# w-k-jones/tobac-flow

Measured on AMD Instinct MI355X. Metric: Mpix/s end-to-end flow+sobel+watershed, 5424^2 frames, higher is better.
Workload: dtype f32

## Files before the change

tobac_flow_amd/csrc/capi.hip:

```cpp
#include "tf_common.h"
#include <stdarg.h>
#include <algorithm>

static thread_local char g_err[512] = "";

void tf_set_error(const char *fmt, ...) {
    va_list ap;
    va_start(ap, fmt);
    vsnprintf(g_err, sizeof(g_err), fmt, ap);
    va_end(ap);
}

extern "C" int tf_version(void) { return 100; }
extern "C" const char *tf_last_error(void) { return g_err; }
extern "C" int tf_device_count(void) {
    int n = 0;
    hipError_t e = hipGetDeviceCount(&n);
    if (e != hipSuccess) { tf_set_error("hipGetDeviceCount: %s", hipGetErrorString(e)); return 0; }
    return n;
}

#include <vector>
#include <mutex>
bool g_tf_prof_on = false;
namespace {
struct Rec { int id; double bytes; hipEvent_t a, b; };
std::vector<Rec> g_recs;
std::vector<hipEvent_t> g_free;
std::mutex g_mu;
const char *g_names[TFK_COUNT] = {"to8bit_pair", "fb_gaussian_blur", "fb_resize", "fb_polyexp", "fb_update_matrices",
    "fb_blur_solve", "fb_iteration_fused", "smooth_flow", "convolve", "sobel", "ws_setup", "ws_relax_sweep", "ws_labels", "vr_prepare", "vr_system", "vr_sor", "binary_morph"};
hipEvent_t get_event() {
    if (!g_free.empty()) { hipEvent_t e = g_free.back(); g_free.pop_back(); return e; }
    hipEvent_t e; (void)hipEventCreate(&e); return e;
}
}
void tf_prof_record(int id, double bytes, hipStream_t s, bool start) {
    std::lock_guard<std::mutex> lk(g_mu);
    if (start) { Rec r{id, bytes, get_event(), get_event()}; (void)hipEventRecord(r.a, s); g_recs.push_back(r); }
    else {
        for (size_t i = g_recs.size(); i-- > 0;) if (g_recs[i].id == id) { (void)hipEventRecord(g_recs[i].b, s); break; }
    }
}
extern "C" int tf_profile_enable(int on) { g_tf_prof_on = on != 0; return TF_OK; }
extern "C" int tf_profile_kernel_count(void) { return TFK_COUNT; }
extern "C" const char *tf_profile_kernel_name(int id) { return (id >= 0 && id < TFK_COUNT) ? g_names[id] : ""; }
extern "C" int tf_profile_collect(int64_t *calls, double *ms, double *bytes) {
    std::lock_guard<std::mutex> lk(g_mu);
    for (int i = 0; i < TFK_COUNT; i++) { calls[i] = 0; ms[i] = 0; bytes[i] = 0; }
    for (auto &r : g_recs) {
        float t = 0;
        if (hipEventSynchronize(r.b) == hipSuccess && hipEventElapsedTime(&t, r.a, r.b) == hipSuccess) {
            calls[r.id]++; ms[r.id] += t; bytes[r.id] += r.bytes;
        }
        g_free.push_back(r.a); g_free.push_back(r.b);
    }
    g_recs.clear();
    return TF_OK;
}

void tf_ws_host_pool_release();
extern "C" int tf_shutdown(void) {
    tf_ws_host_pool_release();
    std::lock_guard<std::mutex> lk(g_mu);
    g_tf_prof_on = false;
    for (auto &r : g_recs) { (void)hipEventDestroy(r.a); (void)hipEventDestroy(r.b); }
    for (auto e : g_free) (void)hipEventDestroy(e);
    g_recs.clear(); g_free.clear();
    return TF_OK;
}

template <int UNROLL, bool NT>
__global__ void __launch_bounds__(256)
k_copy16(const uint4 *__restrict__ src, uint4 *__restrict__ dst, size_t n16)
{
    const size_t tile = (size_t)UNROLL * 256, n_tiles = n16 / tile;
    for (size_t t = blockIdx.x; t < n_tiles; t += gridDim.x) {
        const size_t base = t * tile + threadIdx.x;
        uint4 v[UNROLL];
#pragma unroll
        for (int k = 0; k < UNROLL; k++) {
            if (NT) { typedef unsigned int u4 __attribute__((ext_vector_type(4))); const u4 r = __builtin_nontemporal_load((const u4 *)(src + base + k * 256)); v[k] = make_uint4(r.x, r.y, r.z, r.w); }
            else v[k] = src[base + k * 256];
        }
#pragma unroll
        for (int k = 0; k < UNROLL; k++) {
            if (NT) { typedef unsigned int u4 __attribute__((ext_vector_type(4))); u4 r; r.x = v[k].x; r.y = v[k].y; r.z = v[k].z; r.w = v[k].w; __builtin_nontemporal_store(r, (u4 *)(dst + base + k * 256)); }
            else dst[base + k * 256] = v[k];
        }
    }
    for (size_t i = n_tiles * tile + (size_t)blockIdx.x * 256 + threadIdx.x; i < n16; i += (size_t)gridDim.x * 256) dst[i] = src[i];
}
extern "C" int tf_copy16_variant(const void *src, void *dst, size_t bytes, void *stream, int variant)
{
    TF_REQUIRE(src && dst && bytes >= 16 && bytes % 16 == 0 && ((uintptr_t)src & 15) == 0 && ((uintptr_t)dst & 15) == 0, "tf_copy16: 16-byte aligned buffers of a multiple of 16 bytes");
    const size_t n16 = bytes / 16;
    hipStream_t s = (hipStream_t)stream;
    const uint4 *a = (const uint4 *)src; uint4 *b = (uint4 *)dst;
    const unsigned g8 = (unsigned)std::min<size_t>((n16 + 255) / 256, 256 * 8), g16 = (unsigned)std::min<size_t>((n16 + 255) / 256, 256 * 16);
    switch (variant) {
    case 1: hipLaunchKernelGGL((k_copy16<4, false>), dim3(g16), dim3(256), 0, s, a, b, n16); break;
    case 2: hipLaunchKernelGGL((k_copy16<8, false>), dim3(g8), dim3(256), 0, s, a, b, n16); break;
    case 3: hipLaunchKernelGGL((k_copy16<4, true>), dim3(g8), dim3(256), 0, s, a, b, n16); break;
    case 4: hipLaunchKernelGGL((k_copy16<8, true>), dim3(g8), dim3(256), 0, s, a, b, n16); break;
    case 5: hipLaunchKernelGGL((k_copy16<2, false>), dim3(g8), dim3(256), 0, s, a, b, n16); break;
    case 6: hipLaunchKernelGGL((k_copy16<1, false>), dim3(g16), dim3(256), 0, s, a, b, n16); break;
    case 7: hipLaunchKernelGGL((k_copy16<4, false>), dim3(g8), dim3(256), 0, s, a, b, n16); break;
    default: hipLaunchKernelGGL((k_copy16<4, true>), dim3(g8), dim3(256), 0, s, a, b, n16); break;
    }
    TF_CHECK_LAUNCH();
    return TF_OK;
}
extern "C" int tf_copy16(const void *src, void *dst, size_t bytes, void *stream) { return tf_copy16_variant(src, dst, bytes, stream, 0); }
```

tobac_flow_amd/csrc/morph.hip:

```cpp
#include "tf_common.h"
#include <initializer_list>
#include <string.h>
#include <stdlib.h>

struct MorphTaps { int n; int8_t dt[27], dy[27], dx[27]; };

__global__ void __launch_bounds__(256)
k_binary_morph(const uint8_t *__restrict__ in, int64_t T, int H, int W, MorphTaps tp, int op, int border,
               uint8_t *__restrict__ out)
{
    const int x = blockIdx.x * 64 + threadIdx.x, y = blockIdx.y * 4 + threadIdx.y;
    const int64_t t = blockIdx.z;
    if (x >= W || y >= H) return;
    const int64_t plane = (int64_t)H * W;
    bool r = op == 0;
    for (int i = 0; i < tp.n; i++) {
        const int s = op == 0 ? 1 : -1;
        const int64_t tt = t + s * tp.dt[i];
        const int yy = y + s * tp.dy[i], xx = x + s * tp.dx[i];
        bool v;
        if (tt < 0 || tt >= T || yy < 0 || yy >= H || xx < 0 || xx >= W) v = border != 0;
        else v = in[tt * plane + (int64_t)yy * W + xx] != 0;
        if (op == 0) { if (!v) { r = false; break; } }
        else if (v) { r = true; break; }
    }
    out[t * plane + (int64_t)y * W + x] = r ? 1 : 0;
}

struct MorphRows { int n; int8_t dt[9], dy[9]; uint8_t dxmask[9]; };

__device__ __forceinline__ uint32_t morph_norm(uint32_t w) {
    w |= w >> 4; w |= w >> 2; w |= w >> 1;
    return w & 0x01010101u;
}

__global__ void __launch_bounds__(256)
k_binary_morph4(const uint32_t *__restrict__ in, int64_t T, int H, int W4, MorphRows rw, int op, int border,
                uint32_t *__restrict__ out)
{
    const int x4 = blockIdx.x * 64 + threadIdx.x, y = blockIdx.y * 4 + threadIdx.y;
    const int64_t t = blockIdx.z;
    if (x4 >= W4 || y >= H) return;
    const int64_t plane4 = (int64_t)H * W4;
    const uint32_t bw = border ? 0x01010101u : 0u, bb = border ? 1u : 0u;
    uint32_t r = op == 0 ? 0x01010101u : 0u;
    const int s = op == 0 ? 1 : -1;
    for (int i = 0; i < rw.n; i++) {
        const int64_t tt = t + s * rw.dt[i];
        const int yy = y + s * rw.dy[i];
        uint32_t c = bw, l = bb, rt = bb;
        if (tt >= 0 && tt < T && yy >= 0 && yy < H) {
            const uint32_t *row = in + tt * plane4 + (int64_t)yy * W4;
            c = morph_norm(row[x4]);
            if (rw.dxmask[i] & 5) {
                if (x4 > 0) l = morph_norm(row[x4 - 1]) >> 24;
                if (x4 + 1 < W4) rt = morph_norm(row[x4 + 1]) & 1u;
            }
        }
        const uint32_t m = rw.dxmask[i];
        const uint32_t left = (c << 8) | l, right = (c >> 8) | (rt << 24);
        const uint32_t lo = s == 1 ? left : right, hi = s == 1 ? right : left;
        if (op == 0) {
            if (m & 1) r &= lo;
            if (m & 2) r &= c;
            if (m & 4) r &= hi;
        } else {
            if (m & 1) r |= lo;
            if (m & 2) r |= c;
            if (m & 4) r |= hi;
        }
    }
    out[t * plane4 + (int64_t)y * W4 + x4] = r;
}

__global__ void __launch_bounds__(256)
k_binary_morph16(const uint4 *__restrict__ in, int64_t T, int H, int W16, MorphRows rw, int op, int border,
                 uint4 *__restrict__ out)
{
    const int tiles_x = (W16 + 63) / 64, tiles_y = (H + 7) / 8;
    const int64_t n_tiles = (int64_t)tiles_x * tiles_y, L = blockIdx.x;
    int64_t slot = L >> 3, tile = (slot / T) * 8 + (L & 7), t = slot % T;
    if (border & 2) {
        const int64_t padded = (n_tiles + 7) / 8 * 8;
        tile = L % padded; t = L / padded;
        border &= 1;
    }
    if (tile >= n_tiles) return;
    const int x16 = (int)(tile % tiles_x) * 64 + threadIdx.x;
    if (x16 >= W16) return;
    const int64_t plane16 = (int64_t)H * W16;
    const uint32_t bw = border ? 0x01010101u : 0u, bb = border ? 1u : 0u;
    const uint32_t init = op == 0 ? 0x01010101u : 0u;
    const int s = op == 0 ? 1 : -1;
    for (int half = 0; half < 2; half++) {
    const int y = (int)(tile / tiles_x) * 8 + threadIdx.y + 4 * half;
    if (y >= H) break;
    uint32_t r[4] = {init, init, init, init};
    for (int i = 0; i < rw.n; i++) {
        const int64_t tt = t + s * rw.dt[i];
        const int yy = y + s * rw.dy[i];
        uint32_t c[4] = {bw, bw, bw, bw}, l = bb, rt = bb;
        if (tt >= 0 && tt < T && yy >= 0 && yy < H) {
            const uint4 *row = in + tt * plane16 + (int64_t)yy * W16;
            const uint4 v = row[x16];
            c[0] = morph_norm(v.x); c[1] = morph_norm(v.y); c[2] = morph_norm(v.z); c[3] = morph_norm(v.w);
            if (rw.dxmask[i] & 5) {
                const uint32_t *words = (const uint32_t *)row;
                if (x16 > 0) l = morph_norm(words[4 * x16 - 1]) >> 24;
                if (x16 + 1 < W16) rt = morph_norm(words[4 * x16 + 4]) & 1u;
            }
        }
        const uint32_t m = rw.dxmask[i];
#pragma unroll
        for (int k = 0; k < 4; k++) {
            const uint32_t lb = k == 0 ? l : c[k - 1] >> 24, rb = k == 3 ? rt : c[k + 1] & 1u;
            const uint32_t left = (c[k] << 8) | lb, right = (c[k] >> 8) | (rb << 24);
            const uint32_t lo = s == 1 ? left : right, hi = s == 1 ? right : left;
            if (op == 0) {
                if (m & 1) r[k] &= lo;
                if (m & 2) r[k] &= c[k];
                if (m & 4) r[k] &= hi;
            } else {
                if (m & 1) r[k] |= lo;
                if (m & 2) r[k] |= c[k];
                if (m & 4) r[k] |= hi;
            }
        }
    }
    out[t * plane16 + (int64_t)y * W16 + x16] = make_uint4(r[0], r[1], r[2], r[3]);
    }
}

extern "C" int tf_binary_morph(const uint8_t *in, int64_t T, int64_t H, int64_t W, const uint8_t *structure_host,
                               int op, int iterations, int border_value, uint8_t *out, uint8_t *tmp, void *stream)
{
    TF_REQUIRE(in && out && structure_host, "tf_binary_morph: null pointer");
    TF_REQUIRE(T > 0 && H > 0 && W > 0 && T < 65536 && H < (1 << 15) && W < (1 << 15), "tf_binary_morph: bad shape");
    TF_REQUIRE(op == 0 || op == 1, "tf_binary_morph: op must be 0 (erosion) or 1 (dilation)");
    TF_REQUIRE(iterations >= 1, "tf_binary_morph: iterations must be >= 1");
    TF_REQUIRE(iterations == 1 || tmp, "tf_binary_morph: iterations > 1 needs a tmp buffer");
    TF_REQUIRE(out != in && tmp != in && (tmp != out || iterations == 1), "tf_binary_morph: buffers alias");
    MorphTaps tp; tp.n = 0;
    for (int p = 0; p < 3; p++) for (int r = 0; r < 3; r++) for (int c = 0; c < 3; c++)
        if (structure_host[p * 9 + r * 3 + c]) { tp.dt[tp.n] = (int8_t)(p - 1); tp.dy[tp.n] = (int8_t)(r - 1); tp.dx[tp.n] = (int8_t)(c - 1); tp.n++; }
    TF_REQUIRE(tp.n > 0, "tf_binary_morph: empty structure");
    hipStream_t s = (hipStream_t)stream;
    dim3 block(64, 4), grid((unsigned)((W + 63) / 64), (unsigned)((H + 3) / 4), (unsigned)T);
    MorphRows rw; rw.n = 0;
    for (int p = 0; p < 3; p++) for (int r = 0; r < 3; r++) {
        uint8_t m = 0;
        for (int c = 0; c < 3; c++) if (structure_host[p * 9 + r * 3 + c]) m |= (uint8_t)(1 << c);
        if (m) { rw.dt[rw.n] = (int8_t)(p - 1); rw.dy[rw.n] = (int8_t)(r - 1); rw.dxmask[rw.n] = m; rw.n++; }
    }
    const bool words = W % 4 == 0 && ((uintptr_t)in % 4 == 0) && ((uintptr_t)out % 4 == 0) && (!tmp || (uintptr_t)tmp % 4 == 0);
    const dim3 grid4((unsigned)((W / 4 + 63) / 64), (unsigned)((H + 3) / 4), (unsigned)T);
    const bool quads = W % 16 == 0 && ((uintptr_t)in % 16 == 0) && ((uintptr_t)out % 16 == 0) && (!tmp || (uintptr_t)tmp % 16 == 0);
    const int64_t tiles16 = (int64_t)((W / 16 + 63) / 64) * ((H + 7) / 8);
    TF_REQUIRE(!quads || ((tiles16 + 7) / 8) * 8 * T < (1ll << 31), "tf_binary_morph: volume too large for the 1-D grid");
    const dim3 grid16((unsigned)(((tiles16 + 7) / 8) * 8 * T), 1, 1);
    const uint8_t *src = in;
    for (int it = 0; it < iterations; it++) {
        uint8_t *dst = ((iterations - 1 - it) % 2 == 0) ? out : tmp;
        TfProfScope ps(TFK_MORPH, 2.0 * (double)T * H * W, s);
        static const bool plane_grid = getenv("TF_MORPH_GRID") && !strcmp(getenv("TF_MORPH_GRID"), "plane");
        if (quads) hipLaunchKernelGGL(k_binary_morph16, grid16, block, 0, s, (const uint4 *)src, T, (int)H, (int)(W / 16), rw, op, (border_value ? 1 : 0) | (plane_grid ? 2 : 0), (uint4 *)dst);
        else if (words) hipLaunchKernelGGL(k_binary_morph4, grid4, block, 0, s, (const uint32_t *)src, T, (int)H, (int)(W / 4), rw, op, border_value, (uint32_t *)dst);
        else hipLaunchKernelGGL(k_binary_morph, grid, block, 0, s, src, T, (int)H, (int)W, tp, op, border_value, dst);
        src = dst;
    }
    TF_CHECK_LAUNCH();
    return TF_OK;
}

__global__ void __launch_bounds__(256)
k_linearise(const float *__restrict__ f, int64_t n, float lo, float hi, int flip, float *__restrict__ out)
{
    const int64_t i = (int64_t)blockIdx.x * blockDim.x + threadIdx.x;
    if (i >= n) return;
    float v = (f[i] - lo) / (hi - lo);
    v = (v != v) ? v : fminf(v, 1.f);
    v = (v != v) ? v : fmaxf(v, 0.f);
    out[i] = flip ? 1.f - v : v;
}

static bool tf_vec4_ok(std::initializer_list<const void *> words, std::initializer_list<const void *> bytes)
{
    for (const void *p : words) if ((uintptr_t)p % 16) return false;
    for (const void *p : bytes) if ((uintptr_t)p % 4) return false;
    return true;
}

__global__ void __launch_bounds__(256)
k_linearise4(const float *__restrict__ f, int64_t n, float lo, float hi, int flip, float *__restrict__ out)
{
    const int64_t i = ((int64_t)blockIdx.x * blockDim.x + threadIdx.x) * 4;
    if (i >= n) return;
    auto one = [&](float x) {
        float v = (x - lo) / (hi - lo);
        v = (v != v) ? v : fminf(v, 1.f);
        v = (v != v) ? v : fmaxf(v, 0.f);
        return flip ? 1.f - v : v;
    };
    if (i + 3 < n) {
        const float4 x = *(const float4 *)(f + i);
        *(float4 *)(out + i) = make_float4(one(x.x), one(x.y), one(x.z), one(x.w));
    } else {
        for (int64_t j = i; j < n; j++) out[j] = one(f[j]);
    }
}

extern "C" int tf_linearise(const float *field, int64_t n, double lower, double upper, float *out, void *stream)
{
    TF_REQUIRE(field && out && n > 0, "tf_linearise: bad arguments");
    TF_REQUIRE(lower != upper, "tf_linearise: lower and upper thresholds must have different values");
    int flip = 0;
    if (lower > upper) { const double t = lower; lower = upper; upper = t; flip = 1; }
    if (tf_vec4_ok({field, out}, {}))
        hipLaunchKernelGGL(k_linearise4, dim3((unsigned)(((n + 3) / 4 + 255) / 256)), dim3(256), 0, (hipStream_t)stream, field, n,
                           (float)lower, (float)upper, flip, out);
    else
    hipLaunchKernelGGL(k_linearise, dim3((unsigned)((n + 255) / 256)), dim3(256), 0, (hipStream_t)stream, field, n,
                       (float)lower, (float)upper, flip, out);
    TF_CHECK_LAUNCH();
    return TF_OK;
}

__global__ void __launch_bounds__(256)
k_label_extent(const int32_t *__restrict__ labels, const uint8_t *__restrict__ mask, int64_t plane, int n_labels,
               int *__restrict__ tmin, int *__restrict__ tmax, uint8_t *__restrict__ hit)
{
    const int64_t i = (int64_t)blockIdx.x * blockDim.x + threadIdx.x;
    const int t = blockIdx.y;
    if (i >= plane) return;
    const int64_t p = (int64_t)t * plane + i;
    const int32_t l = labels[p];
    if (l <= 0 || l > n_labels) return;
    if (tmin[l] > t) atomicMin(&tmin[l], t);
    if (tmax[l] < t) atomicMax(&tmax[l], t);
    if (mask && mask[p] && !hit[l]) hit[l] = 1;
}

extern "C" int tf_label_extent(const int32_t *labels, const uint8_t *mask, int64_t T, int64_t H, int64_t W, int n_labels,
                               int *tmin, int *tmax, uint8_t *hit, void *stream)
{
    TF_REQUIRE(labels && tmin && tmax && hit && n_labels >= 0, "tf_label_extent: bad arguments");
    TF_REQUIRE(T > 0 && T < 65536 && H > 0 && W > 0, "tf_label_extent: bad shape");
    hipStream_t s = (hipStream_t)stream;
    TF_CHECK_HIP(hipMemsetAsync(tmin, 0x7f, (size_t)(n_labels + 1) * sizeof(int), s));
    TF_CHECK_HIP(hipMemsetAsync(tmax, 0xff, (size_t)(n_labels + 1) * sizeof(int), s));
    TF_CHECK_HIP(hipMemsetAsync(hit, 0, (size_t)(n_labels + 1), s));
    const int64_t plane = H * W;
    hipLaunchKernelGGL(k_label_extent, dim3((unsigned)((plane + 255) / 256), (unsigned)T), dim3(256), 0, s,
                       labels, mask, plane, n_labels, tmin, tmax, hit);
    TF_CHECK_LAUNCH();
    return TF_OK;
}

__global__ void __launch_bounds__(256)
k_apply_lut(const int32_t *__restrict__ labels, int64_t n, const int32_t *__restrict__ lut, int n_lut, int32_t *__restrict__ out)
{
    const int64_t i = (int64_t)blockIdx.x * blockDim.x + threadIdx.x;
    if (i >= n) return;
    const int32_t l = labels[i];
    out[i] = (l >= 0 && l < n_lut) ? lut[l] : 0;
}

extern "C" int tf_apply_lut(const int32_t *labels, int64_t n, const int32_t *lut, int n_lut, int32_t *out, void *stream)
{
    TF_REQUIRE(labels && lut && out && n > 0 && n_lut > 0, "tf_apply_lut: bad arguments");
    hipLaunchKernelGGL(k_apply_lut, dim3((unsigned)((n + 255) / 256)), dim3(256), 0, (hipStream_t)stream, labels, n, lut, n_lut, out);
    TF_CHECK_LAUNCH();
    return TF_OK;
}

__global__ void __launch_bounds__(256)
k_apply_lut_keep(const int32_t *__restrict__ labels, int64_t n, const int32_t *__restrict__ lut, int n_lut, int32_t *__restrict__ out)
{
    const int64_t i = (int64_t)blockIdx.x * blockDim.x + threadIdx.x;
    if (i >= n) return;
    const int32_t l = labels[i];
    out[i] = l <= 0 ? l : (l < n_lut ? lut[l] : 0);
}

__global__ void __launch_bounds__(256)
k_apply_lut_keep4(const int32_t *__restrict__ labels, int64_t n, const int32_t *__restrict__ lut, int n_lut, int32_t *__restrict__ out)
{
    const int64_t i = ((int64_t)blockIdx.x * blockDim.x + threadIdx.x) * 4;
    if (i >= n) return;
    auto one = [&](int32_t l) { return l <= 0 ? l : (l < n_lut ? lut[l] : 0); };
    if (i + 3 < n) {
        const int4 l = *(const int4 *)(labels + i);
        *(int4 *)(out + i) = make_int4(one(l.x), one(l.y), one(l.z), one(l.w));
    } else {
        for (int64_t j = i; j < n; j++) out[j] = one(labels[j]);
    }
}

extern "C" int tf_apply_lut_keep_nonpositive(const int32_t *labels, int64_t n, const int32_t *lut, int n_lut, int32_t *out, void *stream)
{
    TF_REQUIRE(labels && lut && out && n > 0 && n_lut > 0, "tf_apply_lut_keep_nonpositive: bad arguments");
    if (tf_vec4_ok({labels, out}, {}))
        hipLaunchKernelGGL(k_apply_lut_keep4, dim3((unsigned)(((n + 3) / 4 + 255) / 256)), dim3(256), 0, (hipStream_t)stream, labels, n, lut, n_lut, out);
    else
    hipLaunchKernelGGL(k_apply_lut_keep, dim3((unsigned)((n + 255) / 256)), dim3(256), 0, (hipStream_t)stream, labels, n, lut, n_lut, out);
    TF_CHECK_LAUNCH();
    return TF_OK;
}

__global__ void __launch_bounds__(256)
k_field_masks(const float *__restrict__ f, int64_t n, uint8_t *__restrict__ ge1, uint8_t *__restrict__ le0, uint8_t *__restrict__ isn)
{
    const int64_t i = (int64_t)blockIdx.x * blockDim.x + threadIdx.x;
    if (i >= n) return;
    const float v = f[i];
    const bool nan = v != v;
    ge1[i] = v >= 1.f; le0[i] = (v <= 0.f) || nan; isn[i] = nan;
}
__global__ void __launch_bounds__(256)
k_merge_seeds(const int32_t *__restrict__ comp, const uint8_t *__restrict__ bg, const uint8_t *__restrict__ isn, int64_t n,
              int32_t *__restrict__ seeds)
{
    const int64_t i = (int64_t)blockIdx.x * blockDim.x + threadIdx.x;
    if (i >= n) return;
    seeds[i] = (bg[i] | isn[i]) ? -1 : comp[i];
}
__global__ void __launch_bounds__(256)
k_field_masks4(const float *__restrict__ f, int64_t n, uint8_t *__restrict__ ge1, uint8_t *__restrict__ le0, uint8_t *__restrict__ isn)
{
    const int64_t i = ((int64_t)blockIdx.x * blockDim.x + threadIdx.x) * 4;
    if (i >= n) return;
    if (i + 3 < n) {
        const float4 x = *(const float4 *)(f + i);
        const float v[4] = {x.x, x.y, x.z, x.w};
        uint32_t a = 0, b = 0, c = 0;
#pragma unroll
        for (int k = 0; k < 4; k++) {
            const bool nan = v[k] != v[k];
            a |= (uint32_t)(v[k] >= 1.f) << (8 * k); b |= (uint32_t)((v[k] <= 0.f) || nan) << (8 * k); c |= (uint32_t)nan << (8 * k);
        }
        *(uint32_t *)(ge1 + i) = a; *(uint32_t *)(le0 + i) = b; *(uint32_t *)(isn + i) = c;
    } else {
        for (int64_t j = i; j < n; j++) {
            const float v = f[j];
            const bool nan = v != v;
            ge1[j] = v >= 1.f; le0[j] = (v <= 0.f) || nan; isn[j] = nan;
        }
    }
}
__global__ void __launch_bounds__(256)
k_merge_seeds4(const int32_t *__restrict__ comp, const uint8_t *__restrict__ bg, const uint8_t *__restrict__ isn, int64_t n,
               int32_t *__restrict__ seeds)
{
    const int64_t i = ((int64_t)blockIdx.x * blockDim.x + threadIdx.x) * 4;
    if (i >= n) return;
    if (i + 3 < n) {
        const int4 c = *(const int4 *)(comp + i);
        const uint32_t m = *(const uint32_t *)(bg + i) | *(const uint32_t *)(isn + i);
        *(int4 *)(seeds + i) = make_int4((m & 0xffu) ? -1 : c.x, (m & 0xff00u) ? -1 : c.y, (m & 0xff0000u) ? -1 : c.z, (m & 0xff000000u) ? -1 : c.w);
    } else {
        for (int64_t j = i; j < n; j++) seeds[j] = (bg[j] | isn[j]) ? -1 : comp[j];
    }
}
extern "C" int tf_field_masks(const float *field, int64_t n, uint8_t *ge1, uint8_t *le0_or_nan, uint8_t *isnan_out, void *stream)
{
    TF_REQUIRE(field && ge1 && le0_or_nan && isnan_out && n > 0, "tf_field_masks: bad arguments");
    if (tf_vec4_ok({field}, {ge1, le0_or_nan, isnan_out}))
        hipLaunchKernelGGL(k_field_masks4, dim3((unsigned)(((n + 3) / 4 + 255) / 256)), dim3(256), 0, (hipStream_t)stream, field, n, ge1, le0_or_nan, isnan_out);
    else
    hipLaunchKernelGGL(k_field_masks, dim3((unsigned)((n + 255) / 256)), dim3(256), 0, (hipStream_t)stream, field, n, ge1, le0_or_nan, isnan_out);
    TF_CHECK_LAUNCH();
    return TF_OK;
}
extern "C" int tf_merge_seeds(const int32_t *comp, const uint8_t *bg, const uint8_t *isnan_in, int64_t n, int32_t *seeds, void *stream)
{
    TF_REQUIRE(comp && bg && isnan_in && seeds && n > 0, "tf_merge_seeds: bad arguments");
    if (tf_vec4_ok({comp, seeds}, {bg, isnan_in}))
        hipLaunchKernelGGL(k_merge_seeds4, dim3((unsigned)(((n + 3) / 4 + 255) / 256)), dim3(256), 0, (hipStream_t)stream, comp, bg, isnan_in, n, seeds);
    else
    hipLaunchKernelGGL(k_merge_seeds, dim3((unsigned)((n + 255) / 256)), dim3(256), 0, (hipStream_t)stream, comp, bg, isnan_in, n, seeds);
    TF_CHECK_LAUNCH();
    return TF_OK;
}

#include "tf_prim.h"

__device__ __forceinline__ int ccl_find(int *__restrict__ parent, int p) {
    int q = parent[p];
    while (q != p) { p = q; q = parent[p]; }
    return p;
}

__device__ __forceinline__ void ccl_union(int *__restrict__ parent, int a, int b) {
    for (;;) {
        a = ccl_find(parent, a); b = ccl_find(parent, b);
        if (a == b) return;
        if (a < b) { const int t = a; a = b; b = t; }
        const int old = atomicMin(&parent[a], b);
        if (old == a) return;
        a = old;
    }
}

__global__ void __launch_bounds__(256)
k_ccl_init(const uint8_t *__restrict__ in, int64_t n, int *__restrict__ parent) {
    const int64_t i = (int64_t)blockIdx.x * blockDim.x + threadIdx.x;
    if (i < n) parent[i] = in[i] ? (int)i : -1;
}
__global__ void __launch_bounds__(256)
k_ccl_init4(const uint8_t *__restrict__ in, int64_t n, int *__restrict__ parent) {
    const int64_t i = ((int64_t)blockIdx.x * blockDim.x + threadIdx.x) * 4;
    if (i >= n) return;
    if (i + 3 < n) {
        const uint32_t m = *(const uint32_t *)(in + i);
        const int b = (int)i;
        *(int4 *)(parent + i) = make_int4((m & 0xffu) ? b : -1, (m & 0xff00u) ? b + 1 : -1, (m & 0xff0000u) ? b + 2 : -1, (m & 0xff000000u) ? b + 3 : -1);
    } else {
        for (int64_t j = i; j < n; j++) parent[j] = in[j] ? (int)j : -1;
    }
}

__global__ void __launch_bounds__(256)
k_ccl_init_runs(const uint8_t *__restrict__ in, int64_t T, int H, int W, int *__restrict__ parent)
{
    const int x = blockIdx.x * 64 + threadIdx.x, y = blockIdx.y * 4 + threadIdx.y;
    const int64_t t = blockIdx.z;
    const bool inside = x < W && y < H;
    const int64_t plane = (int64_t)H * W, p = t * plane + (int64_t)y * W + x;
    const bool on = inside && in[p] != 0;
    const unsigned long long m = __ballot(on);
    if (!inside) return;
    if (!on) { parent[p] = -1; return; }
    const int lane = threadIdx.x;
    const unsigned long long zeros_below = ~m & ((1ull << lane) - 1ull);
    const int head = zeros_below ? 64 - __clzll((long long)zeros_below) : 0;
    parent[p] = (int)(p - (lane - head));
}

template <bool RUNS>
__global__ void __launch_bounds__(256)
k_ccl_union(const uint8_t *__restrict__ in, int64_t T, int H, int W, MorphTaps tp, unsigned sibling, int *__restrict__ parent)
{
    const int x = blockIdx.x * 64 + threadIdx.x, y = blockIdx.y * 4 + threadIdx.y;
    const int64_t t = blockIdx.z;
    if (x >= W || y >= H) return;
    const int64_t plane = (int64_t)H * W, p = t * plane + (int64_t)y * W + x;
    if (!in[p]) return;
    const bool left = RUNS && x > 0 && in[p - 1] != 0;
    if (RUNS && left && threadIdx.x == 0) ccl_union(parent, (int)p, (int)(p - 1));
    for (int i = 0; i < tp.n; i++) {
        if (RUNS && tp.dt[i] == 0 && tp.dy[i] == 0) continue;
        const int64_t tt = t + tp.dt[i];
        const int yy = y + tp.dy[i], xx = x + tp.dx[i];
        if (tt < 0 || tt >= T || yy < 0 || yy >= H || xx < 0 || xx >= W) continue;
        const int64_t q = tt * plane + (int64_t)yy * W + xx;
        if (!in[q]) continue;
        if (RUNS && tp.dx[i] == 0 && left && in[q - 1]) continue;
        if (RUNS && tp.dx[i] != 0 && ((sibling >> i) & 1u) && in[q - tp.dx[i]]) continue;
        ccl_union(parent, (int)p, (int)q);
    }
}

__global__ void __launch_bounds__(256)
k_ccl_flatten(int64_t n, int *__restrict__ parent, uint8_t *__restrict__ isroot) {
    const int64_t i = (int64_t)blockIdx.x * blockDim.x + threadIdx.x;
    if (i >= n) return;
    const int p = parent[i];
    if (p < 0) { isroot[i] = 0; return; }
    const int r = ccl_find(parent, (int)i);
    parent[i] = r;
    isroot[i] = r == (int)i;
}

__global__ void __launch_bounds__(256)
k_ccl_count_roots(int64_t n, const uint8_t *__restrict__ isroot, int *__restrict__ block_count) {
    const int64_t b = (int64_t)blockIdx.x * 4 + (threadIdx.x >> 6), i0 = b * 256 + (threadIdx.x & 63) * 4;
    if (b * 256 >= n) return;
    const uint32_t w = i0 < n ? *(const uint32_t *)(isroot + i0) : 0u;
    int c = 0;
#pragma unroll
    for (int j = 0; j < 4; j++) c += __popcll(__ballot(i0 + j < n && ((w >> (8 * j)) & 0xffu) != 0));
    if ((threadIdx.x & 63) == 0) block_count[b] = c;
}
__global__ void __launch_bounds__(256)
k_ccl_rank_roots(int64_t n, const uint8_t *__restrict__ isroot, const int *__restrict__ block_base, int *__restrict__ rank) {
    const int lane = threadIdx.x & 63;
    const int64_t b = (int64_t)blockIdx.x * 4 + (threadIdx.x >> 6), i0 = b * 256 + lane * 4;
    if (b * 256 >= n) return;
    const uint32_t w = i0 < n ? *(const uint32_t *)(isroot + i0) : 0u;
    const unsigned long long below = (1ull << lane) - 1ull;
    bool f[4];
    int before = 0;
#pragma unroll
    for (int j = 0; j < 4; j++) { f[j] = i0 + j < n && ((w >> (8 * j)) & 0xffu) != 0; before += __popcll(__ballot(f[j]) & below); }
    if (!(f[0] || f[1] || f[2] || f[3])) return;
    int r = block_base[b] + before;
#pragma unroll
    for (int j = 0; j < 4; j++) if (f[j]) rank[i0 + j] = r++;
}

__global__ void __launch_bounds__(256)
k_ccl_number(int64_t n, const int *__restrict__ parent, const int *__restrict__ rank, int32_t *__restrict__ labels) {
    const int64_t i = (int64_t)blockIdx.x * blockDim.x + threadIdx.x;
    if (i >= n) return;
    const int r = parent[i];
    labels[i] = r < 0 ? 0 : rank[r] + 1;
}
__global__ void __launch_bounds__(256)
k_ccl_number4(int64_t n, const int *__restrict__ parent, const int *__restrict__ rank, int32_t *__restrict__ labels) {
    const int64_t i = ((int64_t)blockIdx.x * blockDim.x + threadIdx.x) * 4;
    if (i >= n) return;
    if (i + 3 < n) {
        const int4 r = *(const int4 *)(parent + i);
        const int a = rank[r.x < 0 ? 0 : r.x], b = rank[r.y < 0 ? 0 : r.y], c = rank[r.z < 0 ? 0 : r.z], d = rank[r.w < 0 ? 0 : r.w];
        *(int4 *)(labels + i) = make_int4(r.x < 0 ? 0 : a + 1, r.y < 0 ? 0 : b + 1, r.z < 0 ? 0 : c + 1, r.w < 0 ? 0 : d + 1);
    } else {
        for (int64_t j = i; j < n; j++) { const int r = parent[j]; labels[j] = r < 0 ? 0 : rank[r] + 1; }
    }
}

extern "C" size_t tf_label_workspace_bytes(int64_t T, int64_t H, int64_t W)
{
    if (T <= 0 || H <= 0 || W <= 0) return 0;
    const int64_t n = T * H * W;
    size_t scan = 0;
    const int64_t nblk = (n + 255) / 256;
    (void)tf_exclusive_sum(nullptr, scan, (const int *)nullptr, (int *)nullptr, (size_t)(nblk > 0x7fffffff ? 0x7fffffff : nblk));
    return tf_align_up((size_t)n * 4, 256) * 2 + tf_align_up((size_t)n, 256) + 2 * tf_align_up((size_t)nblk * 4, 256) + tf_align_up(scan, 256) + 4096;
}

extern "C" int tf_label(const uint8_t *in, int64_t T, int64_t H, int64_t W, const uint8_t *structure_host,
                        int32_t *labels, int *n_labels_host, void *ws, size_t ws_bytes, void *stream)
{
    TF_REQUIRE(in && labels && structure_host && ws, "tf_label: null pointer");
    TF_REQUIRE(T > 0 && H > 0 && W > 0 && T < 65536 && H < (1 << 15) && W < (1 << 15), "tf_label: bad shape");
    const int64_t n = T * H * W;
    TF_REQUIRE(n < 0x7fffffffll, "tf_label: volume too large for 32-bit parents (use time windows)");
    if (ws_bytes < tf_label_workspace_bytes(T, H, W)) { tf_set_error("tf_label: workspace too small"); return TF_ENOMEM; }
    MorphTaps tp; tp.n = 0;
    for (int p = 0; p < 3; p++) for (int r = 0; r < 3; r++) for (int c = 0; c < 3; c++) {
        const int i = p * 9 + r * 3 + c;
        TF_REQUIRE((structure_host[i] != 0) == (structure_host[26 - i] != 0), "tf_label: structuring element must be symmetric");
        if (structure_host[i] && i > 13) { tp.dt[tp.n] = (int8_t)(p - 1); tp.dy[tp.n] = (int8_t)(r - 1); tp.dx[tp.n] = (int8_t)(c - 1); tp.n++; }
    }
    hipStream_t s = (hipStream_t)stream;
    TfArena ar(ws, ws_bytes);
    int *parent = ar.take<int>(n), *rank = ar.take<int>(n);
    uint8_t *isroot = ar.take<uint8_t>(n);
    const int64_t nblk = (n + 255) / 256;
    int *block_count = ar.take<int>(nblk), *block_base = ar.take<int>(nblk);
    size_t scan_bytes = 0;
    (void)tf_exclusive_sum(nullptr, scan_bytes, (const int *)nullptr, (int *)nullptr, (size_t)nblk);
    char *scan_tmp = ar.take<char>(scan_bytes ? scan_bytes : 1);
    if (!ar.ok()) { tf_set_error("tf_label: workspace too small"); return TF_ENOMEM; }
    const unsigned nb = (unsigned)((n + 255) / 256);
    dim3 block(64, 4), grid((unsigned)((W + 63) / 64), (unsigned)((H + 3) / 4), (unsigned)T);
    bool runs = false;
    for (int i = 0; i < tp.n; i++) runs = runs || (tp.dt[i] == 0 && tp.dy[i] == 0 && tp.dx[i] == 1);
    static const bool no_runs_env = getenv("TF_CCL_NO_RUNS") != nullptr;
    if (no_runs_env) runs = false;
    if (runs) hipLaunchKernelGGL(k_ccl_init_runs, grid, block, 0, s, in, T, (int)H, (int)W, parent);
    else if (tf_vec4_ok({parent}, {in})) hipLaunchKernelGGL(k_ccl_init4, dim3((unsigned)(((n + 3) / 4 + 255) / 256)), dim3(256), 0, s, in, n, parent);
    else hipLaunchKernelGGL(k_ccl_init, dim3(nb), dim3(256), 0, s, in, n, parent);
    unsigned sibling = 0;
    for (int i = 0; i < tp.n; i++)
        for (int j = 0; j < tp.n && tp.dx[i] != 0; j++)
            if (tp.dx[j] == 0 && tp.dt[j] == tp.dt[i] && tp.dy[j] == tp.dy[i]) sibling |= 1u << i;
    if (tp.n && runs) hipLaunchKernelGGL(k_ccl_union<true>, grid, block, 0, s, in, T, (int)H, (int)W, tp, sibling, parent);
    else if (tp.n) hipLaunchKernelGGL(k_ccl_union<false>, grid, block, 0, s, in, T, (int)H, (int)W, tp, sibling, parent);
    hipLaunchKernelGGL(k_ccl_flatten, dim3(nb), dim3(256), 0, s, n, parent, isroot);
    TF_CHECK_LAUNCH();
    const unsigned nb4 = (unsigned)((nblk + 3) / 4);
    hipLaunchKernelGGL(k_ccl_count_roots, dim3(nb4), dim3(256), 0, s, n, (const uint8_t *)isroot, block_count);
    TF_CHECK_HIP(tf_exclusive_sum(scan_tmp, scan_bytes, (const int *)block_count, block_base, (size_t)nblk, s));
    hipLaunchKernelGGL(k_ccl_rank_roots, dim3(nb4), dim3(256), 0, s, n, (const uint8_t *)isroot, (const int *)block_base, rank);
    if (tf_vec4_ok({parent, labels}, {})) hipLaunchKernelGGL(k_ccl_number4, dim3((unsigned)(((n + 3) / 4 + 255) / 256)), dim3(256), 0, s, n, parent, rank, labels);
    else hipLaunchKernelGGL(k_ccl_number, dim3(nb), dim3(256), 0, s, n, parent, rank, labels);
    TF_CHECK_LAUNCH();
    int last_base = 0, last_count = 0;
    TF_CHECK_HIP(hipMemcpyAsync(&last_base, block_base + nblk - 1, sizeof(int), hipMemcpyDeviceToHost, s));
    TF_CHECK_HIP(hipMemcpyAsync(&last_count, block_count + nblk - 1, sizeof(int), hipMemcpyDeviceToHost, s));
    TF_CHECK_HIP(hipStreamSynchronize(s));
    if (n_labels_host) *n_labels_host = last_base + last_count;
    return TF_OK;
}

#define TF_C1D_MAX_RADIUS 64
struct Corr1dW { double w[TF_C1D_MAX_RADIUS + 1]; int r; };

__device__ __forceinline__ int64_t tf_reflect_index(int64_t i, int64_t n)
{
    if (n == 1) return 0;
    const int64_t p = 2 * n;
    i %= p;
    if (i < 0) i += p;
    return i < n ? i : p - 1 - i;
}

template <typename TS>
__global__ void __launch_bounds__(256)
k_correlate1d_sym(const TS *__restrict__ in, int64_t T, int H, int W, int axis, Corr1dW kw, TS *__restrict__ out)
{
    const int x = blockIdx.x * 64 + threadIdx.x, y = blockIdx.y * 4 + threadIdx.y;
    const int64_t t = blockIdx.z;
    if (x >= W || y >= H) return;
    const int64_t plane = (int64_t)H * W;
    const int64_t o = t * plane + (int64_t)y * W + x;
    const int64_t n = axis == 0 ? T : (axis == 1 ? H : W);
    const int64_t c = axis == 0 ? t : (axis == 1 ? y : x);
    const int64_t stride = axis == 0 ? plane : (axis == 1 ? W : 1);
    const TS *line = in + (o - c * stride);
    double tmp = (double)line[c * stride] * kw.w[0];
    for (int j = kw.r; j >= 1; j--) {
        const double a = (double)line[tf_reflect_index(c - j, n) * stride];
        const double b = (double)line[tf_reflect_index(c + j, n) * stride];
        tmp += (a + b) * kw.w[j];
    }
    out[o] = (TS)tmp;
}

extern "C" int tf_correlate1d_sym(const void *in, int type, int64_t T, int64_t H, int64_t W, int axis,
                                  const double *weights_host, int radius, void *out, void *stream)
{
    TF_REQUIRE(in && out && weights_host, "tf_correlate1d_sym: null pointer");
    TF_REQUIRE(in != out, "tf_correlate1d_sym: in-place operation is not supported");
    TF_REQUIRE(T > 0 && H > 0 && W > 0 && H < (1 << 30) && W < (1 << 30) && T < 65536, "tf_correlate1d_sym: bad shape");
    TF_REQUIRE(axis >= 0 && axis <= 2, "tf_correlate1d_sym: axis must be 0, 1 or 2");
    TF_REQUIRE(radius >= 0 && radius <= TF_C1D_MAX_RADIUS, "tf_correlate1d_sym: radius out of range");
    TF_REQUIRE(type == TF_F32 || type == TF_F64, "tf_correlate1d_sym: type must be TF_F32 or TF_F64");
    Corr1dW kw; kw.r = radius;
    for (int j = 0; j <= radius; j++) {
        TF_REQUIRE(weights_host[radius - j] == weights_host[radius + j], "tf_correlate1d_sym: kernel is not symmetric");
        kw.w[j] = weights_host[radius + j];
    }
    hipStream_t s = (hipStream_t)stream;
    const dim3 block(64, 4, 1), grid((unsigned)((W + 63) / 64), (unsigned)((H + 3) / 4), (unsigned)T);
    if (type == TF_F32) hipLaunchKernelGGL(k_correlate1d_sym<float>, grid, block, 0, s, (const float *)in, T, (int)H, (int)W, axis, kw, (float *)out);
    else hipLaunchKernelGGL(k_correlate1d_sym<double>, grid, block, 0, s, (const double *)in, T, (int)H, (int)W, axis, kw, (double *)out);
    TF_CHECK_LAUNCH();
    return TF_OK;
}

template <typename TS>
__global__ void __launch_bounds__(256)
k_grey_morph(const TS *__restrict__ in, int64_t T, int H, int W, MorphTaps tp, int op, TS *__restrict__ out)
{
    const int x = blockIdx.x * 64 + threadIdx.x, y = blockIdx.y * 4 + threadIdx.y;
    const int64_t t = blockIdx.z;
    if (x >= W || y >= H) return;
    const int64_t plane = (int64_t)H * W;
    TS tmp = 0;
    for (int i = 0; i < tp.n; i++) {
        const int64_t tt = tf_reflect_index(t + tp.dt[i], T);
        const int64_t yy = tf_reflect_index(y + tp.dy[i], H), xx = tf_reflect_index(x + tp.dx[i], W);
        const TS v = in[tt * plane + yy * W + xx];
        if (i == 0) tmp = v;
        else if (op == 0) { if (v < tmp) tmp = v; }
        else { if (v > tmp) tmp = v; }
    }
    out[t * plane + (int64_t)y * W + x] = tmp;
}

extern "C" int tf_grey_morph(const void *in, int type, int64_t T, int64_t H, int64_t W, const uint8_t *footprint_host,
                             int op, void *out, void *stream)
{
    TF_REQUIRE(in && out && footprint_host, "tf_grey_morph: null pointer");
    TF_REQUIRE(in != out, "tf_grey_morph: in-place operation is not supported");
    TF_REQUIRE(T > 0 && H > 0 && W > 0 && H < (1 << 30) && W < (1 << 30) && T < 65536, "tf_grey_morph: bad shape");
    TF_REQUIRE(op == 0 || op == 1, "tf_grey_morph: op must be 0 (erosion) or 1 (dilation)");
    TF_REQUIRE(type == TF_F32 || type == TF_F64, "tf_grey_morph: type must be TF_F32 or TF_F64");
    MorphTaps tp; tp.n = 0;
    for (int i = 0; i < 27; i++) {
        TF_REQUIRE((footprint_host[i] != 0) == (footprint_host[26 - i] != 0), "tf_grey_morph: footprint must be point-symmetric");
        if (footprint_host[i]) { tp.dt[tp.n] = (int8_t)(i / 9 - 1); tp.dy[tp.n] = (int8_t)((i / 3) % 3 - 1); tp.dx[tp.n] = (int8_t)(i % 3 - 1); tp.n++; }
    }
    TF_REQUIRE(tp.n > 0, "tf_grey_morph: empty footprint");
    hipStream_t s = (hipStream_t)stream;
    const dim3 block(64, 4, 1), grid((unsigned)((W + 63) / 64), (unsigned)((H + 3) / 4), (unsigned)T);
    if (type == TF_F32) hipLaunchKernelGGL(k_grey_morph<float>, grid, block, 0, s, (const float *)in, T, (int)H, (int)W, tp, op, (float *)out);
    else hipLaunchKernelGGL(k_grey_morph<double>, grid, block, 0, s, (const double *)in, T, (int)H, (int)W, tp, op, (double *)out);
    TF_CHECK_LAUNCH();
    return TF_OK;
}
```

tobac_flow_amd/csrc/tf_common.h:

```cpp
#pragma once
#include <hip/hip_runtime.h>
#include <stdint.h>
#include <stdio.h>
#include "../../include/tobac_flow_hip.h"

void tf_set_error(const char *fmt, ...);

#define TF_CHECK_HIP(expr)                                                              \
    do {                                                                                \
        hipError_t _e = (expr);                                                         \
        if (_e != hipSuccess) {                                                         \
            tf_set_error("%s failed: %s (%s:%d)", #expr, hipGetErrorString(_e), __FILE__, __LINE__); \
            return TF_EHIP;                                                             \
        }                                                                               \
    } while (0)

#define TF_CHECK_LAUNCH()                                                               \
    do {                                                                                \
        hipError_t _e = hipGetLastError();                                              \
        if (_e != hipSuccess) {                                                         \
            tf_set_error("kernel launch failed: %s (%s:%d)", hipGetErrorString(_e), __FILE__, __LINE__); \
            return TF_EHIP;                                                             \
        }                                                                               \
    } while (0)

#define TF_REQUIRE(cond, msg)                                                           \
    do {                                                                                \
        if (!(cond)) { tf_set_error("%s", msg); return TF_EINVAL; }                     \
    } while (0)

static inline size_t tf_align_up(size_t v, size_t a) { return (v + a - 1) / a * a; }

struct TfArena {
    char *base; size_t size, used;
    TfArena(void *p, size_t n) : base((char *)p), size(n), used(0) {}
    template <typename T> T *take(size_t count) {
        size_t off = tf_align_up(used, 256);
        size_t end = off + count * sizeof(T);
        if (end > size || base == nullptr) { used = size + 1; return nullptr; }
        used = end;
        return (T *)(base + off);
    }
    bool ok() const { return used <= size; }
};

#include <mutex>
#define TF_MAX_DEVICES 64
struct TfDeviceOnce {
    std::mutex mu; bool done_[TF_MAX_DEVICES] = {};
    struct Guard {
        TfDeviceOnce &o; std::unique_lock<std::mutex> lk; int dev; bool first;
        explicit Guard(TfDeviceOnce &o_) : o(o_), lk(o_.mu), dev(0), first(false) {
            if (hipGetDevice(&dev) != hipSuccess || dev < 0 || dev >= TF_MAX_DEVICES) dev = 0;
            first = !o.done_[dev];
        }
        void done() { o.done_[dev] = true; }
    };
};

__device__ __forceinline__ int tf_cvround(float v) { return __float2int_rn(v); }
__device__ __forceinline__ int tf_cvfloor(float v) { return __float2int_rd(v); }
__device__ __forceinline__ int tf_sat_short(int v) { return v < -32768 ? -32768 : (v > 32767 ? 32767 : v); }
__device__ __forceinline__ int tf_clampi(int v, int lo, int hi) { return v < lo ? lo : (v > hi ? hi : v); }

enum TfKernelId {
    TFK_TO8BIT = 0, TFK_FB_BLUR, TFK_FB_RESIZE, TFK_FB_POLYEXP, TFK_FB_MATRICES, TFK_FB_BLUR_SOLVE, TFK_FB_ITER,
    TFK_SMOOTH, TFK_CONVOLVE, TFK_SOBEL, TFK_WS_SETUP, TFK_WS_RELAX, TFK_WS_LABELS, TFK_VR_PREPARE, TFK_VR_SYSTEM, TFK_VR_SOR,
    TFK_MORPH,
    TFK_COUNT
};
extern bool g_tf_prof_on;
void tf_prof_record(int id, double bytes, hipStream_t s, bool start);
struct TfProfScope {
    int id; double bytes; hipStream_t s; bool on;
    TfProfScope(int id_, double bytes_, hipStream_t s_) : id(id_), bytes(bytes_), s(s_), on(g_tf_prof_on) { if (on) tf_prof_record(id, bytes, s, true); }
    ~TfProfScope() { if (on) tf_prof_record(id, bytes, s, false); }
};
```

tobac_flow_amd/csrc/watershed.hip:

```cpp
#include "tf_common.h"
#include <string.h>
#include <time.h>
#include <stdio.h>
#include <stdlib.h>
#include "tf_prim.h"
#include <new>

typedef unsigned long long u64;
#define WS_INF 0xFFFFFFFFFFFFFFFFull
#define WS_MARKER_BIT 0x8000000000000000ull
#define WS_MAX_NBR 26
#define WS_MAX_DEPTH TF_WS_MAX_DEPTH
#define WS_BATCH 32
#define WS_K2(c, i) ((c).KM[2 * (int64_t)(i)])
#define WS_M1(c, i) ((c).KM[2 * (int64_t)(i) + 1])

struct WsGeom {
    int64_t T; int H, W; int64_t plane;
    int n_nbr;
    int8_t dt[WS_MAX_NBR], dy[WS_MAX_NBR], dx[WS_MAX_NBR];
    int n_tx;
};

#ifndef WS_TILE
#define WS_TILE 16
#endif
__device__ __forceinline__ int64_t ws_vpos(const WsGeom &g, int64_t t, int y, int x) {
    const int64_t tile = (int64_t)(y / WS_TILE) * g.n_tx + x / WS_TILE;
    return ((tile * g.T + t) * WS_TILE + (y % WS_TILE)) * WS_TILE + (x % WS_TILE);
}
static int64_t ws_virtual_voxels(int64_t T, int64_t H, int64_t W) {
    return T * ((H + WS_TILE - 1) / WS_TILE * WS_TILE) * ((W + WS_TILE - 1) / WS_TILE * WS_TILE);
}

struct WsC {
    int64_t R; int n_nbr;
    const u64 *pix; const unsigned *val; const int *nbr;
    u64 *KM;
    u64 *C[WS_MAX_DEPTH], *Rt;
    int *Llo, *Lhi;
    const u64 *emask;
};

__device__ __forceinline__ unsigned ws_ordkey(float v) {
    v = v + 0.0f;
    unsigned u = __float_as_uint(v);
    return (u & 0x80000000u) ? ~u : (u | 0x80000000u);
}
__device__ __forceinline__ u64 ws_load(const u64 *p) {
    return __hip_atomic_load(p, __ATOMIC_RELAXED, __HIP_MEMORY_SCOPE_AGENT);
}
__device__ __forceinline__ int ws_after(int was) { asm volatile("" : "+v"(was)); return was >> 2; }
__device__ __forceinline__ int ws_round_flow(float f) {
    return (f == f) ? __float2int_rn(f) : 0;
}

__device__ __forceinline__ int64_t ws_neighbour(const WsGeom &g, int64_t t, int y, int x, int fx, int fy, int bx, int by, int i) {
    const int dt = g.dt[i];
    int yy = y + g.dy[i], xx = x + g.dx[i];
    if (dt == 1) { xx += fx; yy += fy; }
    else if (dt == -1) { xx += bx; yy += by; }
    const int64_t tt = t + dt;
    if (tt < 0 || tt >= g.T || (unsigned)yy >= (unsigned)g.H || (unsigned)xx >= (unsigned)g.W) return -1;
    return tt * g.plane + (int64_t)yy * g.W + xx;
}

__global__ void __launch_bounds__(256)
k_ws_classify(const int32_t *__restrict__ markers, const int8_t *__restrict__ mask, int64_t n, uint8_t *__restrict__ cls)
{
    const int64_t i = (int64_t)blockIdx.x * blockDim.x + threadIdx.x;
    if (i >= n) return;
    const int32_t m = markers[i];
    cls[i] = m != 0 ? 2 : ((mask ? mask[i] != 0 : true) ? 1 : 0);
}
__global__ void __launch_bounds__(256)
k_ws_classify4(const int32_t *__restrict__ markers, const int8_t *__restrict__ mask, int64_t n, uint8_t *__restrict__ cls)
{
    const int64_t i = ((int64_t)blockIdx.x * blockDim.x + threadIdx.x) * 4;
    if (i >= n) return;
    if (i + 3 < n) {
        const int4 m = *(const int4 *)(markers + i);
        const uint32_t k = mask ? *(const uint32_t *)(mask + i) : 0xffffffffu;
        const int mm[4] = {m.x, m.y, m.z, m.w};
        uint32_t out = 0;
#pragma unroll
        for (int j = 0; j < 4; j++) out |= (uint32_t)(mm[j] != 0 ? 2 : (((k >> (8 * j)) & 0xffu) ? 1 : 0)) << (8 * j);
        *(uint32_t *)(cls + i) = out;
    } else {
        for (int64_t j = i; j < n; j++) cls[j] = markers[j] != 0 ? 2 : ((mask ? mask[j] != 0 : true) ? 1 : 0);
    }
}

template <int NN>
__global__ void __launch_bounds__(256)
k_ws_relevant(const uint8_t *__restrict__ cls, const float *__restrict__ fwd, const float *__restrict__ bwd, WsGeom g,
              uint8_t *__restrict__ flag)
{
    const int x = blockIdx.x * 64 + threadIdx.x, y = blockIdx.y * 4 + threadIdx.y;
    const int64_t t = blockIdx.z;
    if (x >= g.W || y >= g.H) return;
    const int64_t p = t * g.plane + (int64_t)y * g.W + x;
    const uint8_t c = cls[p];
    uint8_t f = c == 1;
    if (c == 2) {
        const float2 fw = ((const float2 *)fwd)[p], bw = ((const float2 *)bwd)[p];
        const int fx = ws_round_flow(fw.x), fy = ws_round_flow(fw.y), bx = ws_round_flow(bw.x), by = ws_round_flow(bw.y);
        if (NN > 0) {
            uint8_t v[NN > 0 ? NN : 1];
#pragma unroll
            for (int j = 0; j < NN; j++) {
                const int64_t n = ws_neighbour(g, t, y, x, fx, fy, bx, by, j);
                const uint8_t vn = cls[n >= 0 ? n : p];
                v[j] = n >= 0 ? vn : 0;
            }
#pragma unroll
            for (int j = 0; j < NN; j++) f |= v[j] == 1;
        } else {
            for (int i0 = 0; i0 < g.n_nbr && !f; i0 += 8) {
                uint8_t v[8];
#pragma unroll
                for (int j = 0; j < 8; j++) {
                    const int64_t n = i0 + j < g.n_nbr ? ws_neighbour(g, t, y, x, fx, fy, bx, by, i0 + j) : -1;
                    v[j] = n >= 0 ? cls[n] : 0;
                }
#pragma unroll
                for (int j = 0; j < 8; j++) f |= v[j] == 1;
            }
        }
    }
    flag[ws_vpos(g, t, y, x)] = f;
}

__global__ void __launch_bounds__(256)
k_ws_relevant6x4(const uint8_t *__restrict__ cls, const float *__restrict__ fwd, const float *__restrict__ bwd, WsGeom g,
                 uint8_t *__restrict__ flag)
{
    const int x0 = (blockIdx.x * 64 + threadIdx.x) * 4, y = blockIdx.y * 4 + threadIdx.y;
    const int64_t t = blockIdx.z;
    if (x0 >= g.W || y >= g.H) return;
    const int64_t p0 = t * g.plane + (int64_t)y * g.W + x0;
    const uint32_t c = *(const uint32_t *)(cls + p0);
    const uint32_t is1 = c & 0x01010101u & ~((c >> 1) & 0x01010101u);
    const uint32_t is2 = (c >> 1) & 0x01010101u;
    uint32_t rel = is1;
    if (is2) {
        const uint32_t up = y > 0 ? *(const uint32_t *)(cls + p0 - g.W) : 0u, dn = y + 1 < g.H ? *(const uint32_t *)(cls + p0 + g.W) : 0u;
        const uint32_t lb = x0 > 0 ? cls[p0 - 1] : 0u, rb = x0 + 4 < g.W ? cls[p0 + 4] : 0u;
        const uint32_t one = 0x01010101u;
        auto ones = [&](uint32_t w) { return w & one & ~((w >> 1) & one); };
        uint32_t hit = ones(up) | ones(dn) | ones((c << 8) | lb) | ones((c >> 8) | (rb << 24));
        uint32_t need = is2 & ~hit;
        rel |= is2 & hit;
        if (need) {
            const float4 fa = *(const float4 *)(fwd + 2 * p0), fb = *(const float4 *)(fwd + 2 * p0 + 4);
            const float4 ba = *(const float4 *)(bwd + 2 * p0), bb = *(const float4 *)(bwd + 2 * p0 + 4);
            const float fx[4] = {fa.x, fa.z, fb.x, fb.z}, fy[4] = {fa.y, fa.w, fb.y, fb.w};
            const float bx[4] = {ba.x, ba.z, bb.x, bb.z}, by[4] = {ba.y, ba.w, bb.y, bb.w};
            uint8_t vn[4], vp[4];
#pragma unroll
            for (int j = 0; j < 4; j++) {
                const bool want = (need >> (8 * j)) & 1u;
                const int xn = x0 + j + ws_round_flow(fx[j]), yn = y + ws_round_flow(fy[j]);
                const int xp = x0 + j + ws_round_flow(bx[j]), yp = y + ws_round_flow(by[j]);
                const bool okn = want && t + 1 < g.T && (unsigned)xn < (unsigned)g.W && (unsigned)yn < (unsigned)g.H;
                const bool okp = want && t > 0 && (unsigned)xp < (unsigned)g.W && (unsigned)yp < (unsigned)g.H;
                const uint8_t a = cls[okn ? (t + 1) * g.plane + (int64_t)yn * g.W + xn : p0 + j];
                const uint8_t b = cls[okp ? (t - 1) * g.plane + (int64_t)yp * g.W + xp : p0 + j];
                vn[j] = okn ? a : 0; vp[j] = okp ? b : 0;
            }
#pragma unroll
            for (int j = 0; j < 4; j++) rel |= (uint32_t)(vn[j] == 1 || vp[j] == 1) << (8 * j);
        }
    }
    *(uint32_t *)(flag + ws_vpos(g, t, y, x0)) = rel;
}

__global__ void __launch_bounds__(256)
k_ws_cid_tiled(const uint8_t *__restrict__ cls, const uint8_t *__restrict__ flag, const int *__restrict__ scan, WsGeom g,
               int *__restrict__ cid)
{
    const int x = blockIdx.x * 64 + threadIdx.x, y = blockIdx.y * 4 + threadIdx.y;
    const int64_t t = blockIdx.z;
    if (x >= g.W || y >= g.H) return;
    const int64_t p = t * g.plane + (int64_t)y * g.W + x, k = ws_vpos(g, t, y, x);
    int c = -1;
    if (flag[k]) c = cls[p] == 1 ? scan[k] : -2 - scan[k];
    cid[p] = c;
}

__global__ void __launch_bounds__(256)
k_ws_count_tiles(const uint8_t *__restrict__ flag, int64_t n_tiles, long long *__restrict__ count)
{
    const int64_t b = (int64_t)blockIdx.x * 4 + (threadIdx.x >> 6);
    if (b >= n_tiles) return;
    const int lane = threadIdx.x & 63;
    const uint32_t w = *(const uint32_t *)(flag + b * 256 + lane * 4);
    int c = 0;
#pragma unroll
    for (int j = 0; j < 4; j++) c += __popcll(__ballot(((w >> (8 * j)) & 0xffu) != 0));
    if (lane == 0) count[b] = c;
}
__global__ void __launch_bounds__(256)
k_ws_cid_tiles(const uint8_t *__restrict__ cls, const uint8_t *__restrict__ flag, const long long *__restrict__ base, int64_t n_tiles,
               WsGeom g, int *__restrict__ cid)
{
    const int64_t b = (int64_t)blockIdx.x * 4 + (threadIdx.x >> 6);
    if (b >= n_tiles) return;
    const int lane = threadIdx.x & 63;
    const int64_t tile = b / g.T, t = b - tile * g.T;
    const int ty = (int)(tile / g.n_tx), tx = (int)(tile - (int64_t)ty * g.n_tx);
    const int y = ty * WS_TILE + lane / 4, x0 = tx * WS_TILE + (lane & 3) * 4;
    const uint32_t w = *(const uint32_t *)(flag + b * 256 + lane * 4);
    const unsigned long long below = (1ull << lane) - 1ull;
    bool f[4]; unsigned long long m[4];
    int before = 0;
#pragma unroll
    for (int j = 0; j < 4; j++) { f[j] = ((w >> (8 * j)) & 0xffu) != 0; m[j] = __ballot(f[j]); before += __popcll(m[j] & below); }
    if (y >= g.H || x0 >= g.W) return;
    const int64_t p0 = t * g.plane + (int64_t)y * g.W + x0;
    const int id0 = (int)base[b] + before;
    int c[4], run = 0;
#pragma unroll
    for (int j = 0; j < 4; j++) {
        c[j] = -1;
        if (f[j]) { const int id = id0 + run; c[j] = cls[p0 + j] == 1 ? id : -2 - id; run++; }
    }
    if (x0 + 3 < g.W && (((uintptr_t)(cid + p0)) & 15) == 0) *(int4 *)(cid + p0) = make_int4(c[0], c[1], c[2], c[3]);
    else {
#pragma unroll
        for (int j = 0; j < 4; j++) if (x0 + j < g.W) cid[p0 + j] = c[j];
    }
}
static_assert(WS_TILE * WS_TILE == 256, "one scan block = one tile of one frame");

__global__ void __launch_bounds__(256)
k_ws_cid(const uint8_t *__restrict__ cls, const uint8_t *__restrict__ flag, const int *__restrict__ scan, int64_t n,
         int *__restrict__ cid)
{
    const int64_t i = (int64_t)blockIdx.x * blockDim.x + threadIdx.x;
    if (i >= n) return;
    int c = -1;
    if (flag[i]) c = cls[i] == 1 ? scan[i] : -2 - scan[i];
    cid[i] = c;
}

template <int NN>
__global__ void __launch_bounds__(256)
k_ws_compact(const float *__restrict__ field, const float *__restrict__ fwd, const float *__restrict__ bwd,
             const int *__restrict__ cid, WsGeom g, u64 *__restrict__ pix, unsigned *__restrict__ val,
             int *__restrict__ nbr, u64 *__restrict__ KM, int *__restrict__ nan_flag)
{
    const int x = blockIdx.x * 64 + threadIdx.x, y = blockIdx.y * 4 + threadIdx.y;
    const int64_t t = blockIdx.z;
    if (x >= g.W || y >= g.H) return;
    const int64_t p = t * g.plane + (int64_t)y * g.W + x;
    const int c = cid[p];
    if (c == -1) return;
    const bool marker = c < 0;
    const int64_t id = marker ? -2 - c : c;
    const float2 fw = ((const float2 *)fwd)[p], bw = ((const float2 *)bwd)[p];
    const int fx = ws_round_flow(fw.x), fy = ws_round_flow(fw.y), bx = ws_round_flow(bw.x), by = ws_round_flow(bw.y);
    const float fv = field[p];
    if (fv != fv) *nan_flag = 1;
    const unsigned v = ws_ordkey(fv);
    pix[id] = (u64)p | (marker ? WS_MARKER_BIT : 0ull);
    val[id] = v;
    if (NN > 0) {
        int cn[NN > 0 ? NN : 1];
#pragma unroll
        for (int i = 0; i < NN; i++) {
            const int64_t n = ws_neighbour(g, t, y, x, fx, fy, bx, by, i);
            const int cv = cid[n >= 0 ? n : p];
            cn[i] = n >= 0 ? cv : -1;
        }
#pragma unroll
        for (int i = 0; i < NN; i++) nbr[id * NN + i] = cn[i] < 0 ? -1 : cn[i];
    } else {
        for (int i = 0; i < g.n_nbr; i++) {
            const int64_t n = ws_neighbour(g, t, y, x, fx, fy, bx, by, i);
            int cn = -1;
            if (n >= 0) { cn = cid[n]; if (cn < 0) cn = -1; }
            nbr[id * g.n_nbr + i] = cn;
        }
    }
    *(ulonglong2 *)&KM[2 * id] = make_ulonglong2(marker ? ((u64)v << 32) : WS_INF, WS_INF);
}

struct WsRavel {
    int64_t n; int n_nbr;
    int64_t structure[WS_MAX_NBR]; int32_t floc[WS_MAX_NBR], bloc[WS_MAX_NBR];
    const int32_t *foff, *boff;
};
__device__ __forceinline__ int64_t wsr_neighbour(const WsRavel &g, int64_t p, int fo, int bo, int i) {
    const int64_t n = p + g.structure[i] + (int64_t)g.floc[i] * fo + (int64_t)g.bloc[i] * bo;
    return (n >= 0 && n < g.n) ? n : -1;
}

__global__ void __launch_bounds__(256)
k_wsr_seeds(const int64_t *__restrict__ locs, int64_t n_locs, int64_t n, uint8_t *__restrict__ seed, int *__restrict__ bad)
{
    const int64_t i = (int64_t)blockIdx.x * blockDim.x + threadIdx.x;
    if (i >= n_locs) return;
    const int64_t p = locs[i];
    if (p < 0 || p >= n || (i > 0 && locs[i - 1] >= p)) { *bad = 1; return; }
    seed[p] = 1;
}

__global__ void __launch_bounds__(256)
k_wsr_classify(const uint8_t *__restrict__ seed, const int32_t *__restrict__ output, const int8_t *__restrict__ mask, int64_t n,
               uint8_t *__restrict__ cls, int *__restrict__ bad)
{
    const int64_t i = (int64_t)blockIdx.x * blockDim.x + threadIdx.x;
    if (i >= n) return;
    const bool sd = seed[i] != 0;
    if (sd && output[i] == 0) *bad = 2;
    cls[i] = sd ? 2 : ((mask[i] != 0 && output[i] == 0) ? 1 : 0);
}

__global__ void __launch_bounds__(256)
k_wsr_relevant(const uint8_t *__restrict__ cls, WsRavel g, uint8_t *__restrict__ flag)
{
    const int64_t p = (int64_t)blockIdx.x * blockDim.x + threadIdx.x;
    if (p >= g.n) return;
    const uint8_t c = cls[p];
    uint8_t f = c == 1;
    if (c == 2) {
        const int fo = g.foff[p], bo = g.boff[p];
        for (int i = 0; i < g.n_nbr && !f; i++) { const int64_t n = wsr_neighbour(g, p, fo, bo, i); f |= n >= 0 && cls[n] == 1; }
    }
    flag[p] = f;
}

__global__ void __launch_bounds__(256)
k_wsr_compact(const float *__restrict__ image, const int *__restrict__ cid, WsRavel g, u64 *__restrict__ pix,
              unsigned *__restrict__ val, int *__restrict__ nbr, u64 *__restrict__ KM, int *__restrict__ nan_flag)
{
    const int64_t p = (int64_t)blockIdx.x * blockDim.x + threadIdx.x;
    if (p >= g.n) return;
    const int c = cid[p];
    if (c == -1) return;
    const bool marker = c < 0;
    const int64_t id = marker ? -2 - c : c;
    const int fo = g.foff[p], bo = g.boff[p];
    const float fv = image[p];
    if (fv != fv) *nan_flag = 1;
    const unsigned v = ws_ordkey(fv);
    pix[id] = (u64)p | (marker ? WS_MARKER_BIT : 0ull);
    val[id] = v;
    for (int i = 0; i < g.n_nbr; i++) {
        const int64_t n = wsr_neighbour(g, p, fo, bo, i);
        int cn = -1;
        if (n >= 0) { cn = cid[n]; if (cn < 0) cn = -1; }
        nbr[id * g.n_nbr + i] = cn;
    }
    *(ulonglong2 *)&KM[2 * id] = make_ulonglong2(marker ? ((u64)v << 32) : WS_INF, WS_INF);
}

__global__ void __launch_bounds__(256)
k_wsr_labels(const int *__restrict__ cid, const u64 *__restrict__ Rt, const u64 *__restrict__ pix, int ranked, int32_t *output, int64_t n)
{
    const int64_t i = (int64_t)blockIdx.x * blockDim.x + threadIdx.x;
    if (i >= n) return;
    const int c = cid[i];
    if (c >= 0 && output[i] == 0) { const u64 r = Rt[c]; if (r != WS_INF) output[i] = output[ranked ? (pix[r & 0xFFFFFFFFull] & ~WS_MARKER_BIT) : r]; }
}

__global__ void __launch_bounds__(256)
k_ws_init_level(const u64 *__restrict__ pix, u64 *__restrict__ dst, int64_t R, int is_root, const int *__restrict__ rank)
{
    const int64_t i = (int64_t)blockIdx.x * blockDim.x + threadIdx.x;
    if (i >= R) return;
    const u64 px = pix[i];
    const bool marker = (px & WS_MARKER_BIT) != 0ull;
    const u64 root = rank ? (((u64)(unsigned)rank[i] << 32) | (u64)(unsigned)i) : (px & ~WS_MARKER_BIT);
    dst[i] = marker ? (is_root ? root : 0ull) : WS_INF;
}

__global__ void __launch_bounds__(256)
k_ws_init_labelset(const u64 *__restrict__ pix, const int32_t *__restrict__ markers, int *__restrict__ lo,
                   int *__restrict__ hi, int64_t R)
{
    const int64_t i = (int64_t)blockIdx.x * blockDim.x + threadIdx.x;
    if (i >= R) return;
    const u64 px = pix[i];
    const bool marker = (px & WS_MARKER_BIT) != 0ull;
    const int32_t l = marker ? markers[px & ~WS_MARKER_BIT] : 0;
    lo[i] = marker ? l : 0x7fffffff;
    hi[i] = marker ? l : (int)0x80000000;
}

#ifndef WS_LDS_CAP
#define WS_LDS_CAP 4096
#endif
struct WsStage { int cnt[2]; int base; int buf[2][WS_LDS_CAP]; };

__device__ __forceinline__ void ws_stage(WsStage &st, int w, bool enq, int n, int *__restrict__ qout, int *__restrict__ cnt_out, int qcap) {
    if (enq) {
        const int pos = atomicAdd(&st.cnt[w], 1);
        if (pos < WS_LDS_CAP) st.buf[w][pos] = n;
        else { const int g = atomicAdd(cnt_out, 1); if (g < qcap) qout[g] = n; }
    }
}
__device__ __forceinline__ void ws_flush(WsStage &st, int w, int *__restrict__ qout, int *__restrict__ cnt_out, int qcap) {
    __syncthreads();
    const int n = min(st.cnt[w], WS_LDS_CAP);
    if (n > 0) {
        if (threadIdx.x == 0) st.base = atomicAdd(cnt_out, n);
        __syncthreads();
        const int base = st.base;
        for (int i = threadIdx.x; i < n; i += blockDim.x) { const int pos = base + i; if (pos < qcap) qout[pos] = st.buf[w][i]; }
        __syncthreads();
        if (threadIdx.x == 0) st.cnt[w] = 0;
    }
    __syncthreads();
}

#define WS_NB 8

template <int NN>
__device__ __forceinline__ void ws_entry_a(const WsC &c, WsStage &st, int w, bool act, int p, int *__restrict__ inq,
                                           int *__restrict__ qout, int *__restrict__ cnt_out, int qcap)
{
    constexpr int NB = NN ? NN : WS_NB;
    const int n_nbr = NN ? NN : c.n_nbr;
    const int *np = c.nbr + (int64_t)p * n_nbr;
    u64 kp = WS_INF;
    for (int s0 = 0; s0 < n_nbr; s0 += NB) {
        int n[NB];
#pragma unroll
        for (int j = 0; j < NB; j++) n[j] = (act && s0 + j < n_nbr) ? np[s0 + j] : -1;
        if (s0 == 0 && act) {
            const int dep = inq ? ws_after(atomicExch(&inq[p], 0)) : 0;
            kp = ws_load(&WS_K2(c, p) + 2 * dep);
        }
        const u64 lp = kp >> 32;
        u64 vn[NB], m1[NB], k2[NB];
#pragma unroll
        for (int j = 0; j < NB; j++) {
            const int q = n[j] >= 0 ? n[j] : 0;
            vn[j] = c.val[q];
            const ulonglong2 km = *(const ulonglong2 *)&WS_K2(c, q);
            k2[j] = km.x; m1[j] = km.y;
        }
        u64 cand[NB], old[NB];
#pragma unroll
        for (int j = 0; j < NB; j++) {
            cand[j] = vn[j] > lp ? ((vn[j] << 32) | 1ull) : (vn[j] == lp ? kp + 1ull : kp);
            old[j] = 0ull;
            if (n[j] >= 0) {
                if (kp < m1[j]) atomicMin(&WS_M1(c, n[j]), kp);
                if (cand[j] < k2[j]) old[j] = atomicMin(&WS_K2(c, n[j]), cand[j]);
            }
        }
        int was_q[NB];
#pragma unroll
        for (int j = 0; j < NB; j++) {
            was_q[j] = 1;
            if (n[j] >= 0 && cand[j] < old[j]) was_q[j] = inq ? atomicExch(&inq[n[j]], 1) : 0;
        }
#pragma unroll
        for (int j = 0; j < NB; j++) ws_stage(st, w, was_q[j] == 0, n[j], qout, cnt_out, qcap);
    }
}

template <int NN>
__global__ void __launch_bounds__(256)
k_ws_sweep_a(WsC c, const int *__restrict__ qin, const int *__restrict__ cnt_in, int *__restrict__ qout,
             int *__restrict__ cnt_out, int *__restrict__ inq, int qcap, int rounds)
{
    __shared__ WsStage st;
    if (threadIdx.x == 0) { st.cnt[0] = 0; st.cnt[1] = 0; }
    __syncthreads();
    const int64_t n_in = qin ? (int64_t)min(*cnt_in, qcap) : c.R;
    const int64_t n_pad = (n_in + 255) & ~255ll;
    for (int64_t i0 = (int64_t)blockIdx.x * 256; i0 < n_pad; i0 += (int64_t)gridDim.x * 256) {
        const int64_t i = i0 + threadIdx.x;
        const bool act = i < n_in;
        const int p = act ? (qin ? qin[i] : (int)i) : 0;
        int w = 0;
        ws_entry_a<NN>(c, st, w, act, p, inq, qout, cnt_out, qcap);
        for (int r = 0; r < rounds; r++) {
            __syncthreads();
            const int n = min(st.cnt[w], WS_LDS_CAP);
            if (n == 0) break;
            for (int j0 = 0; j0 < n; j0 += 256) {
                const int j = j0 + threadIdx.x;
                const bool a2 = j < n;
                ws_entry_a<NN>(c, st, w ^ 1, a2, a2 ? st.buf[w][j] : 0, inq, qout, cnt_out, qcap);
            }
            __syncthreads();
            if (threadIdx.x == 0) st.cnt[w] = 0;
            w ^= 1;
        }
        ws_flush(st, w, qout, cnt_out, qcap);
    }
}

__global__ void __launch_bounds__(256)
k_ws_edge_masks(WsC c, u64 *__restrict__ emask)
{
    const int64_t p = (int64_t)blockIdx.x * blockDim.x + threadIdx.x;
    if (p >= c.R) return;
    const u64 kp = WS_K2(c, p);
    u64 m = 0ull;
    if (kp != WS_INF) {
        const int *np = c.nbr + p * c.n_nbr;
        for (int i0 = 0; i0 < c.n_nbr; i0 += WS_NB) {
            int n[WS_NB]; u64 m1[WS_NB], kn[WS_NB]; unsigned vn[WS_NB];
#pragma unroll
            for (int j = 0; j < WS_NB; j++) n[j] = i0 + j < c.n_nbr ? np[i0 + j] : -1;
#pragma unroll
            for (int j = 0; j < WS_NB; j++) {
                const int q = n[j] >= 0 ? n[j] : 0;
                const ulonglong2 km = *(const ulonglong2 *)&WS_K2(c, q);
                kn[j] = km.x; m1[j] = km.y; vn[j] = c.val[q];
            }
#pragma unroll
            for (int j = 0; j < WS_NB; j++)
                if (n[j] >= 0 && m1[j] == kp) {
                    m |= 1ull << (i0 + j);
                    if ((kn[j] >> 32) == (u64)vn[j] && (kn[j] & 0xFFFFFFFFull) == 1ull) m |= 1ull << (32 + i0 + j);
                }
        }
    }
    emask[p] = m;
}

__device__ __forceinline__ int ws_load_i(const int *p) {
    return __hip_atomic_load(p, __ATOMIC_RELAXED, __HIP_MEMORY_SCOPE_AGENT);
}

template <int NN>
__device__ __forceinline__ void ws_entry_chain(const WsC &c, int k, int depth, u64 *__restrict__ dst, WsStage &st, int w,
                                               bool act0, int p, int *__restrict__ inq,
                                               int *__restrict__ qout, int *__restrict__ cnt_out, int qcap)
{
    constexpr int NB = NN ? NN : WS_NB;
    const int n_nbr = NN ? NN : c.n_nbr;
    const int *np = c.nbr + (int64_t)p * n_nbr;
    const bool root = k == depth;
    u64 kp = WS_INF, own = WS_INF, em = 0ull;
    int own_lo = 0x7fffffff, own_hi = (int)0x80000000;
    u64 cp[WS_MAX_DEPTH];
    for (int s0 = 0; s0 < n_nbr; s0 += NB) {
        if (s0 == 0 && act0) {
            const int dep = inq ? ws_after(atomicExch(&inq[p], 0)) : 0;
            em = c.emask[p];
            kp = WS_K2(c, p);
            own = ws_load(&dst[p] + dep);
            if (root) { own_lo = ws_load_i(&c.Llo[p] + dep); own_hi = ws_load_i(&c.Lhi[p] + dep); }
            for (int j = 1; j < k; j++) cp[j] = c.C[j][p];
        }
        int n[NB];
#pragma unroll
        for (int j = 0; j < NB; j++) n[j] = (s0 + j < n_nbr && ((em >> (s0 + j)) & 1ull)) ? np[s0 + j] : -1;
        u64 dn[NB];
        int lon[NB], hin[NB];
#pragma unroll
        for (int j = 0; j < NB; j++) {
            dn[j] = WS_INF; lon[j] = 0; hin[j] = 0;
            if (n[j] >= 0) { dn[j] = dst[n[j]]; if (root) { lon[j] = c.Llo[n[j]]; hin[j] = c.Lhi[n[j]]; } }
        }
        u64 offered[NB], old[NB];
        int olo[NB], ohi[NB];
#pragma unroll
        for (int j = 0; j < NB; j++) {
            offered[j] = WS_INF; old[j] = 0ull; olo[j] = (int)0x80000000; ohi[j] = 0x7fffffff;
            if (n[j] >= 0) {
                const bool entry = ((em >> (32 + s0 + j)) & 1ull) != 0ull;
                bool match = true;
                for (int l = 1; l < k && match; l++) {
                    const u64 offered_l = entry ? (l == 1 ? kp : cp[l - 1]) : cp[l];
                    match = offered_l == c.C[l][n[j]];
                }
                if (match) {
                    if (root) offered[j] = own;
                    else offered[j] = entry ? (k == 1 ? kp : cp[k - 1]) : own;
                    if (offered[j] != WS_INF && offered[j] < dn[j]) old[j] = atomicMin(&dst[n[j]], offered[j]);
                    if (root) {
                        if (own_lo < lon[j]) olo[j] = atomicMin(&c.Llo[n[j]], own_lo);
                        if (own_hi > hin[j]) ohi[j] = atomicMax(&c.Lhi[n[j]], own_hi);
                    }
                }
            }
        }
        int was_q[NB];
#pragma unroll
        for (int j = 0; j < NB; j++) {
            was_q[j] = 1;
            const bool improved = offered[j] < old[j] || (root && (own_lo < olo[j] || own_hi > ohi[j]));
            if (improved) was_q[j] = inq ? atomicExch(&inq[n[j]], 1) : 0;
        }
#pragma unroll
        for (int j = 0; j < NB; j++) ws_stage(st, w, was_q[j] == 0, n[j], qout, cnt_out, qcap);
    }
}

template <int NN>
__global__ void __launch_bounds__(256)
k_ws_sweep_chain(WsC c, int k, int depth, const int *__restrict__ qin, const int *__restrict__ cnt_in,
                 int *__restrict__ qout, int *__restrict__ cnt_out, int *__restrict__ inq, int qcap, int rounds)
{
    __shared__ WsStage st;
    if (threadIdx.x == 0) { st.cnt[0] = 0; st.cnt[1] = 0; }
    __syncthreads();
    const int64_t n_in = qin ? (int64_t)min(*cnt_in, qcap) : c.R;
    const int64_t n_pad = (n_in + 255) & ~255ll;
    u64 *dst = k == depth ? c.Rt : c.C[k];
    for (int64_t i0 = (int64_t)blockIdx.x * 256; i0 < n_pad; i0 += (int64_t)gridDim.x * 256) {
        const int64_t i = i0 + threadIdx.x;
        const bool act0 = i < n_in;
        const int p = act0 ? (qin ? qin[i] : (int)i) : 0;
        int w = 0;
        ws_entry_chain<NN>(c, k, depth, dst, st, w, act0, p, inq, qout, cnt_out, qcap);
        for (int r = 0; r < rounds; r++) {
            __syncthreads();
            const int n = min(st.cnt[w], WS_LDS_CAP);
            if (n == 0) break;
            for (int j0 = 0; j0 < n; j0 += 256) {
                const int j = j0 + threadIdx.x;
                const bool a2 = j < n;
                ws_entry_chain<NN>(c, k, depth, dst, st, w ^ 1, a2, a2 ? st.buf[w][j] : 0, inq, qout, cnt_out, qcap);
            }
            __syncthreads();
            if (threadIdx.x == 0) st.cnt[w] = 0;
            w ^= 1;
        }
        ws_flush(st, w, qout, cnt_out, qcap);
    }
}

__global__ void __launch_bounds__(256)
k_ws_origins(WsC c, int depth, int *__restrict__ org)
{
    const int64_t p = (int64_t)blockIdx.x * blockDim.x + threadIdx.x;
    if (p >= c.R) return;
    const u64 kp = WS_K2(c, p);
    if (kp == WS_INF || c.Rt[p] == WS_INF) return;
    const int lo = c.Llo[p], hi = c.Lhi[p];
    u64 cp[WS_MAX_DEPTH];
    for (int j = 1; j < depth; j++) cp[j] = c.C[j][p];
    const u64 em = c.emask[p];
    for (int i = 0; i < c.n_nbr; i++) {
        if (!((em >> i) & 1ull)) continue;
        const int n = c.nbr[p * c.n_nbr + i];
        const bool entry = ((em >> (32 + i)) & 1ull) != 0ull;
        bool match = true;
        for (int l = 1; l < depth && match; l++) {
            const u64 offered_l = entry ? (l == 1 ? kp : cp[l - 1]) : cp[l];
            match = offered_l == c.C[l][n];
        }
        if (!match) continue;
        if (c.Llo[n] != lo || c.Lhi[n] != hi) {
            const bool complete = depth >= 2 && (c.C[depth - 1][n] & 0xFFFFFFFFull) == 0ull;
            atomicOr(&org[n], complete ? 1 : 2);
        }
    }
}

__global__ void __launch_bounds__(256)
k_ws_count_ambiguous(WsC c, const int *__restrict__ org, unsigned long long *__restrict__ cnt)
{
    const int64_t i = (int64_t)blockIdx.x * blockDim.x + threadIdx.x;
    int a = 0, t = 0, e = 0;
    if (i < c.R && c.Rt[i] != WS_INF && !(c.pix[i] & WS_MARKER_BIT)) {
        a = c.Llo[i] != c.Lhi[i];
        const int o = org[i];
        t = o & 1; e = (o >> 1) & 1;
    }
    const unsigned long long ma = __ballot(a), mt = __ballot(t), me = __ballot(e);
    if ((threadIdx.x & 63) == 0) {
        if (ma) atomicAdd(&cnt[0], (unsigned long long)__popcll(ma));
        if (mt) atomicAdd(&cnt[1], (unsigned long long)__popcll(mt));
        if (me) atomicAdd(&cnt[2], (unsigned long long)__popcll(me));
    }
}

__global__ void __launch_bounds__(256)
k_ws_labels(const int32_t *__restrict__ markers, const int *__restrict__ cid, const u64 *__restrict__ Rt,
            const u64 *__restrict__ pix, int ranked, const int *__restrict__ lo, const int *__restrict__ hi, const int *__restrict__ org,
            int32_t *__restrict__ labels, uint8_t *__restrict__ amb, int64_t n)
{
    const int64_t i = (int64_t)blockIdx.x * blockDim.x + threadIdx.x;
    if (i >= n) return;
    int32_t l = markers[i];
    const int c = cid[i];
    uint8_t a = 0;
    if (l == 0 && c >= 0) {
        const u64 r = Rt[c];
        if (r != WS_INF) {
            l = markers[ranked ? (pix[r & 0xFFFFFFFFull] & ~WS_MARKER_BIT) : r];
            if (amb) a = (uint8_t)((lo[c] != hi[c] ? 1 : 0) | ((org[c] & 3) << 1));
        }
    }
    labels[i] = l;
    if (amb) amb[i] = a;
}

__global__ void __launch_bounds__(256)
k_ws_seed_counts(const uint8_t *__restrict__ cls, const float *__restrict__ field, int64_t n, unsigned vmax,
                 int *__restrict__ n_seed, int *__restrict__ n_small, int *__restrict__ any_below)
{
    __shared__ int part[2][4];
    const int64_t i = (int64_t)blockIdx.x * 256 + threadIdx.x;
    const bool sd = i < n && cls[i] == 2;
    const unsigned key = sd ? ws_ordkey(field[i]) : 0u;
    const bool sm = sd && key <= vmax;
    if (sm && key < vmax) *any_below = 1;
    const unsigned long long ms = __ballot(sd), mm = __ballot(sm);
    if ((threadIdx.x & 63) == 0) { part[0][threadIdx.x >> 6] = __popcll(ms); part[1][threadIdx.x >> 6] = __popcll(mm); }
    __syncthreads();
    if (threadIdx.x == 0) {
        n_seed[blockIdx.x] = part[0][0] + part[0][1] + part[0][2] + part[0][3];
        n_small[blockIdx.x] = part[1][0] + part[1][1] + part[1][2] + part[1][3];
    }
}
__global__ void __launch_bounds__(256)
k_ws_small_list(const uint8_t *__restrict__ cls, const int *__restrict__ cid, const float *__restrict__ field, int64_t n, unsigned vmax,
                const long long *__restrict__ base_seed, const long long *__restrict__ base_small, const int *__restrict__ subid,
                long long *__restrict__ out_k, unsigned *__restrict__ out_val, int *__restrict__ out_id)
{
    __shared__ int part[2][4];
    const int64_t i = (int64_t)blockIdx.x * 256 + threadIdx.x;
    unsigned key = 0;
    const bool sd = i < n && cls[i] == 2;
    bool sm = false;
    if (sd) { key = ws_ordkey(field[i]); sm = key <= vmax; }
    const unsigned long long ms = __ballot(sd), mm = __ballot(sm);
    const int lane = threadIdx.x & 63, wave = threadIdx.x >> 6;
    if (lane == 0) { part[0][wave] = __popcll(ms); part[1][wave] = __popcll(mm); }
    __syncthreads();
    if (!sm) return;
    const unsigned long long below = (1ull << lane) - 1ull;
    long long k = base_seed[blockIdx.x] + __popcll(ms & below), slot = base_small[blockIdx.x] + __popcll(mm & below);
    for (int w = 0; w < wave; w++) { k += part[0][w]; slot += part[1][w]; }
    const int c = cid[i];
    const int id = c <= -2 ? -2 - c : -1;
    out_k[slot] = k; out_val[slot] = key; out_id[slot] = (id >= 0 && subid) ? subid[id] : id;
}
__global__ void __launch_bounds__(256)
k_ws_seed_list(const uint8_t *__restrict__ cls, const int *__restrict__ cid, const float *__restrict__ field, int64_t n,
               const long long *__restrict__ base_seed, int64_t c0, int64_t cap, const int *__restrict__ subid, unsigned vmax,
               u64 *__restrict__ out_entry)
{
    __shared__ int part[4];
    const long long b0 = base_seed[blockIdx.x];
    if (b0 >= c0 + cap || b0 + 256 <= c0) return;
    const int64_t i = (int64_t)blockIdx.x * 256 + threadIdx.x;
    const bool sd = i < n && cls[i] == 2;
    const unsigned long long ms = __ballot(sd);
    const int lane = threadIdx.x & 63, wave = threadIdx.x >> 6;
    if (lane == 0) part[wave] = __popcll(ms);
    __syncthreads();
    if (!sd) return;
    long long k = b0 + __popcll(ms & ((1ull << lane) - 1ull));
    for (int w = 0; w < wave; w++) k += part[w];
    k -= c0;
    if (k < 0 || k >= cap) return;
    const int c = cid[i];
    int id = c <= -2 ? -2 - c : -1;
    const unsigned v = ws_ordkey(field[i]);
    if (id >= 0 && subid && v <= vmax) id = subid[id];
    out_entry[k] = v > vmax ? WS_INF : (((u64)v << 32) | 0x80000000ull | (u64)(unsigned)(id + 1));
}
__global__ void __launch_bounds__(256)
k_ws_entry_sample(const uint8_t *__restrict__ cls, const int *__restrict__ cid, const float *__restrict__ field, int64_t n, unsigned vmax,
                  u64 *__restrict__ out)
{
    const int64_t step = n / 256 > 0 ? n / 256 : 1;
    int64_t i = (int64_t)threadIdx.x * step;
    u64 e = 0ull;
    for (int j = 0; j < 512 && i < n; j++, i++) {
        if (cls[i] != 2 || cid[i] != -1) continue;
        const unsigned v = ws_ordkey(field[i]);
        if (v <= vmax) { e = ((u64)v << 32) | 0x80000000ull; break; }
    }
    out[threadIdx.x] = e;
}
struct WsSeedCode { bool seed, d, l, x; unsigned key; int id; };
__device__ __forceinline__ WsSeedCode ws_seed_code(const uint8_t *cls, const int *cid, const float *field, int64_t i, int64_t n, unsigned vmax, u64 D) {
    WsSeedCode r; r.seed = i < n && cls[i] == 2; r.d = r.l = r.x = false; r.key = 0; r.id = -1;
    if (r.seed) {
        r.key = ws_ordkey(field[i]);
        const int c = cid[i];
        r.id = c <= -2 ? -2 - c : -1;
        r.l = r.key > vmax;
        r.d = !r.l && r.id < 0 && D != 0ull && r.key == (unsigned)(D >> 32);
        r.x = !r.l && !r.d;
    }
    return r;
}
__global__ void __launch_bounds__(256)
k_ws_code_counts(const uint8_t *__restrict__ cls, const int *__restrict__ cid, const float *__restrict__ field, int64_t n, unsigned vmax, u64 D,
                 int *__restrict__ n_exc)
{
    __shared__ int part[4];
    const WsSeedCode r = ws_seed_code(cls, cid, field, (int64_t)blockIdx.x * 256 + threadIdx.x, n, vmax, D);
    const unsigned long long m = __ballot(r.x);
    if ((threadIdx.x & 63) == 0) part[threadIdx.x >> 6] = __popcll(m);
    __syncthreads();
    if (threadIdx.x == 0) n_exc[blockIdx.x] = part[0] + part[1] + part[2] + part[3];
}
__global__ void __launch_bounds__(256)
k_ws_seed_codes(const uint8_t *__restrict__ cls, const int *__restrict__ cid, const float *__restrict__ field, int64_t n, unsigned vmax, u64 D,
                const long long *__restrict__ base_seed, const long long *__restrict__ base_exc, const int *__restrict__ subid,
                int write_bits, unsigned *__restrict__ bits_d, unsigned *__restrict__ bits_l, int64_t c0, int64_t cap, u64 *__restrict__ exc)
{
    __shared__ int part_s[4], part_x[4];
    __shared__ unsigned lb_d[9], lb_l[9];
    if (!write_bits) { const long long b0 = base_exc[blockIdx.x]; if (b0 >= c0 + cap || b0 + 256 <= c0) return; }
    if (threadIdx.x < 9) { lb_d[threadIdx.x] = 0u; lb_l[threadIdx.x] = 0u; }
    const WsSeedCode r = ws_seed_code(cls, cid, field, (int64_t)blockIdx.x * 256 + threadIdx.x, n, vmax, D);
    const unsigned long long ms = __ballot(r.seed), mx = __ballot(r.x);
    const int lane = threadIdx.x & 63, wave = threadIdx.x >> 6;
    if (lane == 0) { part_s[wave] = __popcll(ms); part_x[wave] = __popcll(mx); }
    __syncthreads();
    const unsigned long long below = (1ull << lane) - 1ull;
    int sl = __popcll(ms & below), xl = __popcll(mx & below);
    for (int w = 0; w < wave; w++) { sl += part_s[w]; xl += part_x[w]; }
    if (write_bits) {
        if (r.d) atomicOr(&lb_d[sl >> 5], 1u << (sl & 31));
        if (r.l) atomicOr(&lb_l[sl >> 5], 1u << (sl & 31));
        __syncthreads();
        if (threadIdx.x < 18) {
            const int t = threadIdx.x % 9;
            const unsigned *lb = threadIdx.x < 9 ? lb_d : lb_l;
            unsigned *bits = threadIdx.x < 9 ? bits_d : bits_l;
            const long long kb = base_seed[blockIdx.x];
            const int sh = (int)(kb & 31);
            const unsigned lo = t < 8 ? lb[t] : 0u, hi = t > 0 ? lb[t - 1] : 0u;
            const unsigned word = sh ? ((lo << sh) | (hi >> (32 - sh))) : lo;
            if (word) atomicOr(&bits[(kb >> 5) + t], word);
        }
    }
    if (r.x) {
        const long long slot = base_exc[blockIdx.x] + xl - c0;
        if (slot >= 0 && slot < cap) {
            int id = r.id;
            if (id >= 0 && subid) id = subid[id];
            exc[slot] = ((u64)r.key << 32) | 0x80000000ull | (u64)(unsigned)(id + 1);
        }
    }
}
__device__ __forceinline__ bool ws_poppable(const WsC &c, int64_t i, unsigned vmax) {
    const unsigned v = c.val[i];
    return (c.pix[i] & WS_MARKER_BIT) ? v <= vmax : v < vmax;
}
__global__ void __launch_bounds__(256)
k_ws_sub_mark(WsC c, unsigned vmax, uint8_t *__restrict__ in_q, int *__restrict__ any_flooded_small)
{
    const int64_t i = (int64_t)blockIdx.x * blockDim.x + threadIdx.x;
    if (i >= c.R || !ws_poppable(c, i, vmax)) return;
    in_q[i] = 1;
    if (!(c.pix[i] & WS_MARKER_BIT)) *any_flooded_small = 1;
    const int *np = c.nbr + i * c.n_nbr;
    for (int j = 0; j < c.n_nbr; j++) { const int n = np[j]; if (n >= 0) in_q[n] = 1; }
}
__global__ void __launch_bounds__(256)
k_ws_sub_export(WsC c, unsigned vmax, const uint8_t *__restrict__ in_q, const int *__restrict__ subid,
                unsigned *__restrict__ out_val, int *__restrict__ out_nbr)
{
    const int64_t i = (int64_t)blockIdx.x * blockDim.x + threadIdx.x;
    if (i >= c.R || !in_q[i]) return;
    const int64_t q = subid[i];
    out_val[q] = c.val[i];
    const bool pop = ws_poppable(c, i, vmax);
    const int *np = c.nbr + i * c.n_nbr;
    for (int j = 0; j < c.n_nbr; j++) { const int n = pop ? np[j] : -1; out_nbr[q * c.n_nbr + j] = n >= 0 ? subid[n] : -1; }
}
struct WsTie { const long long *k; const int *sid; int S; long long M; long long *pos; int *tj, *c0, *c1, *size, *pre; int *n_nodes; };
__device__ __forceinline__ int ws_tie_lower_bound(const long long *k, int lo, int hi, long long a) {
    while (lo < hi) { const int mid = lo + ((hi - lo) >> 1); if (k[mid] < a) lo = mid + 1; else hi = mid; }
    return lo;
}
__global__ void __launch_bounds__(256)
k_ws_tie_level(WsTie t, int lo, int hi)
{
    const int n = lo + (int)(blockIdx.x * blockDim.x + threadIdx.x);
    if (n >= hi) return;
    const long long p = t.pos[n];
    const int j = t.tj[n];
    const long long kprev = t.k[j];
#pragma unroll
    for (int side = 0; side < 2; side++) {
        const long long v = 2 * p + 1 + side;
        int jj = -1;
        for (int sh = 0; sh < 62; sh++) {
            const long long lo_l = ((v + 1) << sh) - 1;
            if (lo_l >= t.M) break;
            const long long hi_l = lo_l + (1ll << sh) - 1;
            if (hi_l <= kprev) continue;
            const long long a = lo_l > kprev + 1 ? lo_l : kprev + 1;
            const int idx = ws_tie_lower_bound(t.k, j + 1, t.S, a);
            if (idx < t.S && t.k[idx] <= hi_l) { jj = idx; break; }
        }
        int m = -1;
        if (jj >= 0) { m = atomicAdd(t.n_nodes, 1); if (m < t.S) { t.pos[m] = v; t.tj[m] = jj; } else m = -1; }
        if (side == 0) t.c0[n] = m; else t.c1[n] = m;
    }
}
__global__ void __launch_bounds__(256)
k_ws_tie_sizes(WsTie t, int lo, int hi)
{
    const int n = lo + (int)(blockIdx.x * blockDim.x + threadIdx.x);
    if (n >= hi) return;
    const int a = t.c0[n], b = t.c1[n];
    t.size[n] = 1 + (a >= 0 ? t.size[a] : 0) + (b >= 0 ? t.size[b] : 0);
}
__global__ void __launch_bounds__(256)
k_ws_tie_pre(WsTie t, int lo, int hi)
{
    const int n = lo + (int)(blockIdx.x * blockDim.x + threadIdx.x);
    if (n >= hi) return;
    const int a = t.c0[n], b = t.c1[n], p = t.pre[n];
    if (a >= 0) t.pre[a] = p + 1;
    if (b >= 0) t.pre[b] = p + 1 + (a >= 0 ? t.size[a] : 0);
}
__global__ void __launch_bounds__(256)
k_ws_tie_default_ranks(int64_t R, int S, int *__restrict__ rank)
{
    const int64_t i = (int64_t)blockIdx.x * blockDim.x + threadIdx.x;
    if (i < R) rank[i] = (int)(S + i);
}
__global__ void __launch_bounds__(256)
k_ws_tie_scatter(WsTie t, int *__restrict__ rank)
{
    const int n = (int)(blockIdx.x * blockDim.x + threadIdx.x);
    if (n >= t.S) return;
    const int id = t.sid[t.tj[n]];
    if (id >= 0) rank[id] = t.pre[n];
}

__global__ void __launch_bounds__(256)
k_ws_scatter_ranks(const uint8_t *__restrict__ in_q, const int *__restrict__ subid, const int *__restrict__ rank_q, int n_ranked,
                   int64_t R, int *__restrict__ rank)
{
    const int64_t i = (int64_t)blockIdx.x * blockDim.x + threadIdx.x;
    if (i >= R) return;
    int r = -1;
    if (!in_q) r = rank_q[i];
    else if (in_q[i]) r = rank_q[subid[i]];
    rank[i] = r >= 0 ? r : (int)(n_ranked + i);
}
__global__ void __launch_bounds__(256)
k_ws_tie_value_max(WsC c, const int *__restrict__ org, const float *__restrict__ field, int ranked, unsigned *__restrict__ vmax)
{
    const int64_t i = (int64_t)blockIdx.x * blockDim.x + threadIdx.x;
    if (i >= c.R || !(org[i] & 1)) return;
    const u64 r = c.Rt[i];
    if (r != WS_INF) atomicMax(vmax, ws_ordkey(field[ranked ? (c.pix[r & 0xFFFFFFFFull] & ~WS_MARKER_BIT) : r]));
}

struct WsU8ToInt { __host__ __device__ __forceinline__ int operator()(uint8_t v) const { return (int)v; } };
typedef rocprim::transform_iterator<const uint8_t *, WsU8ToInt, int> WsFlagIter;

#define WS_SCAN_CHUNK (1ll << 30)
struct WsIntToLL { __host__ __device__ __forceinline__ long long operator()(int v) const { return (long long)v; } };
typedef rocprim::transform_iterator<const int *, WsIntToLL, long long> WsCountIter;
static size_t ws_scan_temp_bytes(int64_t n) {
    size_t bytes = 0, b2 = 0, b3 = 0;
    WsFlagIter it((const uint8_t *)nullptr, WsU8ToInt());
    (void)tf_exclusive_sum_from(nullptr, bytes, it, (int *)nullptr, 0, (size_t)(n > WS_SCAN_CHUNK ? WS_SCAN_CHUNK : n));
    const int64_t nb = (n + 255) / 256 < 0x7fffffffll ? (n + 255) / 256 : 0x7ffffffell;
    (void)tf_exclusive_sum(nullptr, b2, (const long long *)nullptr, (long long *)nullptr, (size_t)nb);
    (void)tf_exclusive_sum(nullptr, b3, WsCountIter((const int *)nullptr, WsIntToLL()), (long long *)nullptr, (size_t)nb);
    if (b2 > bytes) bytes = b2;
    if (b3 > bytes) bytes = b3;
    return bytes;
}

static int ws_scan_flags(const uint8_t *flag, int *scan, int64_t N, void *tmp, size_t tmp_bytes, hipStream_t s, int64_t *total)
{
    int64_t carry = 0;
    for (int64_t off = 0; off < N; off += WS_SCAN_CHUNK) {
        const int64_t n = N - off < WS_SCAN_CHUNK ? N - off : WS_SCAN_CHUNK;
        size_t tb = tmp_bytes;
        WsFlagIter it(flag + off, WsU8ToInt());
        TF_CHECK_HIP(tf_exclusive_sum_from(tmp, tb, it, scan + off, (int)carry, (size_t)n, s));
        int last_scan = 0; uint8_t last_flag = 0;
        TF_CHECK_HIP(hipMemcpyAsync(&last_scan, scan + off + n - 1, sizeof(int), hipMemcpyDeviceToHost, s));
        TF_CHECK_HIP(hipMemcpyAsync(&last_flag, flag + off + n - 1, 1, hipMemcpyDeviceToHost, s));
        TF_CHECK_HIP(hipStreamSynchronize(s));
        carry = (int64_t)last_scan + last_flag;
        TF_REQUIRE(carry <= 0x3fffff00ll, "tf_watershed: more than 2^30 relevant pixels in one call (use time windows)");
    }
    *total = carry;
    return TF_OK;
}

static size_t ws_full_bytes(int64_t N, int64_t NV) {
    return tf_align_up((size_t)N, 256) + tf_align_up((size_t)NV, 256) + tf_align_up((size_t)N * 4, 256) + tf_align_up((size_t)NV * 4, 256)
         + tf_align_up(ws_scan_temp_bytes(NV), 256) + tf_align_up((size_t)((N + 255) / 256) * 24 + 64, 256) + 4096;
}
static size_t ws_compact_bytes(int64_t R, int n_nbr, int depth) {
    return tf_align_up((size_t)R * 8, 256) + tf_align_up((size_t)R * 4, 256) + tf_align_up((size_t)R * 4 * n_nbr, 256)
         + (size_t)(depth + 2) * tf_align_up((size_t)R * 8, 256)
         + 2 * tf_align_up((size_t)R * 8 + 256, 256) + tf_align_up((size_t)R * 4, 256)
         + 5 * tf_align_up((size_t)R * 4, 256) + tf_align_up((size_t)R * 8, 256) + 4096;
}

extern "C" size_t tf_watershed_workspace_bytes(int64_t T, int64_t H, int64_t W, int n_nbr, int chain_depth, int64_t max_relevant)
{
    if (T <= 0 || H <= 0 || W <= 0 || chain_depth < 1 || chain_depth > WS_MAX_DEPTH || n_nbr < 1 || n_nbr > WS_MAX_NBR) return 0;
    const int64_t N = T * H * W;
    if (max_relevant <= 0 || max_relevant > N) max_relevant = N;
    return ws_full_bytes(N, ws_virtual_voxels(T, H, W)) + ws_compact_bytes(max_relevant, n_nbr, chain_depth);
}

struct WsQueues { int *q[2]; int *cnt; int *inq; int qcap; int *h_cnt; int64_t *processed; };

static int ws_run_phase(const WsC &c, int phase_k, int depth, const WsQueues &Q, hipStream_t s, int64_t max_sweeps,
                        int64_t *sweeps_out, double alg_bytes = 0.0)
{
    const unsigned nbR = (unsigned)((c.R + 255) / 256);
    const unsigned nb = nbR < 2048u ? nbR : 2048u;
    static const int rounds = getenv("TF_WS_LOCAL_ROUNDS") ? atoi(getenv("TF_WS_LOCAL_ROUNDS")) : 4;
    static const bool dedupe = getenv("TF_WS_DEDUPE") != nullptr;
    int *inq = dedupe ? Q.inq : nullptr;
    TF_CHECK_HIP(hipMemsetAsync(Q.cnt, 0, (WS_BATCH + 1) * sizeof(int), s));
    if (dedupe) TF_CHECK_HIP(hipMemsetAsync(Q.inq, 0, (size_t)c.R * sizeof(int), s));
    int64_t sweeps = 0;
    int parity = 0;
    bool first = true;
    unsigned grid_hint = nb;
    for (;;) {
        const bool scan_batch = first;
        {
            TfProfScope ps(TFK_WS_RELAX, alg_bytes, s);
            alg_bytes = 0.0;
            for (int b = 0; b < WS_BATCH; b++) {
                const int *qin = first ? nullptr : Q.q[parity];
                const unsigned blocks = first ? nbR : grid_hint;
                if (phase_k == 0) {
                    if (c.n_nbr == 6) hipLaunchKernelGGL(k_ws_sweep_a<6>, dim3(blocks), dim3(256), 0, s, c, qin, Q.cnt + b, Q.q[parity ^ 1], Q.cnt + b + 1, inq, Q.qcap, rounds);
                    else hipLaunchKernelGGL(k_ws_sweep_a<0>, dim3(blocks), dim3(256), 0, s, c, qin, Q.cnt + b, Q.q[parity ^ 1], Q.cnt + b + 1, inq, Q.qcap, rounds);
                } else {
                    if (c.n_nbr == 6) hipLaunchKernelGGL(k_ws_sweep_chain<6>, dim3(blocks), dim3(256), 0, s, c, phase_k, depth, qin, Q.cnt + b, Q.q[parity ^ 1], Q.cnt + b + 1, inq, Q.qcap, rounds);
                    else hipLaunchKernelGGL(k_ws_sweep_chain<0>, dim3(blocks), dim3(256), 0, s, c, phase_k, depth, qin, Q.cnt + b, Q.q[parity ^ 1], Q.cnt + b + 1, inq, Q.qcap, rounds);
                }
                parity ^= 1;
                first = false;
            }
        }
        TF_CHECK_LAUNCH();
        TF_CHECK_HIP(hipMemcpyAsync(Q.h_cnt, Q.cnt, (WS_BATCH + 1) * sizeof(int), hipMemcpyDeviceToHost, s));
        TF_CHECK_HIP(hipStreamSynchronize(s));
        bool done = false, overflow = false;
        static const bool trace = getenv("TF_WS_TRACE") != nullptr;
        if (trace) {
            fprintf(stderr, "ws_trace phase %d sweeps %lld:", phase_k, (long long)sweeps);
            for (int b = 0; b <= WS_BATCH; b++) fprintf(stderr, " %d", Q.h_cnt[b]);
            fprintf(stderr, "\n");
        }
        for (int b = (scan_batch ? 1 : 0); b <= WS_BATCH; b++) overflow = overflow || Q.h_cnt[b] > Q.qcap;
        if (overflow && dedupe) { tf_set_error("tf_watershed: frontier queue overflow"); return TF_EHIP; }
        for (int b = (scan_batch ? 1 : 0); b <= WS_BATCH && !overflow; b++) {
            if (Q.h_cnt[b] == 0) { done = true; break; }
            if (b < WS_BATCH) *Q.processed += Q.h_cnt[b];
        }
        sweeps += WS_BATCH;
        {
            const int64_t last = Q.h_cnt[WS_BATCH];
            int64_t gb = (last * 4 + 255) / 256;
            if (gb < 64) gb = 64;
            if (gb > (int64_t)nb) gb = nb;
            grid_hint = (unsigned)gb;
        }
        if (done) break;
        if (sweeps > max_sweeps) { tf_set_error("tf_watershed: phase %d did not converge in %lld sweeps", phase_k, (long long)sweeps); return TF_ENOCONV; }
        if (overflow) {
            first = true;
            TF_CHECK_HIP(hipMemsetAsync(Q.cnt, 0, (WS_BATCH + 1) * sizeof(int), s));
            continue;
        }
        TF_CHECK_HIP(hipMemcpyAsync(Q.cnt, Q.cnt + WS_BATCH, sizeof(int), hipMemcpyDeviceToDevice, s));
        TF_CHECK_HIP(hipMemsetAsync(Q.cnt + 1, 0, WS_BATCH * sizeof(int), s));
    }
    *sweeps_out = sweeps;
    return TF_OK;
}

#include <vector>
namespace {
struct WsHostBuf { void *p; size_t bytes; bool pinned; };
std::mutex g_ws_host_mu;
std::vector<WsHostBuf> g_ws_host_free, g_ws_host_lent;
}
static WsHostBuf ws_host_take(size_t bytes, bool pinned)
{
    if (bytes == 0) bytes = 64;
    {
        std::lock_guard<std::mutex> lk(g_ws_host_mu);
        int best = -1;
        for (size_t i = 0; i < g_ws_host_free.size(); i++) {
            const WsHostBuf &b = g_ws_host_free[i];
            if (b.pinned == pinned && b.bytes >= bytes && (best < 0 || b.bytes < g_ws_host_free[best].bytes)) best = (int)i;
        }
        if (best >= 0) { WsHostBuf b = g_ws_host_free[best]; g_ws_host_free.erase(g_ws_host_free.begin() + best); return b; }
    }
    WsHostBuf b{nullptr, bytes + bytes / 8, pinned};
    if (pinned) { if (hipHostMalloc(&b.p, b.bytes, hipHostMallocDefault) != hipSuccess) { (void)hipGetLastError(); b.p = nullptr; } }
    else b.p = malloc(b.bytes);
    if (!b.p) b.bytes = 0;
    return b;
}
static void ws_host_give(WsHostBuf &b)
{
    if (!b.p) return;
    std::lock_guard<std::mutex> lk(g_ws_host_mu);
    g_ws_host_free.push_back(b);
    b.p = nullptr; b.bytes = 0;
}
static void *ws_pool_alloc(size_t bytes)
{
    WsHostBuf b = ws_host_take(bytes, false);
    if (!b.p) return nullptr;
    std::lock_guard<std::mutex> lk(g_ws_host_mu);
    g_ws_host_lent.push_back(b);
    return b.p;
}
static void ws_pool_free(void *p)
{
    if (!p) return;
    std::lock_guard<std::mutex> lk(g_ws_host_mu);
    for (size_t i = 0; i < g_ws_host_lent.size(); i++)
        if (g_ws_host_lent[i].p == p) { g_ws_host_free.push_back(g_ws_host_lent[i]); g_ws_host_lent.erase(g_ws_host_lent.begin() + i); return; }
}
void tf_ws_host_pool_release()
{
    std::lock_guard<std::mutex> lk(g_ws_host_mu);
    for (auto &b : g_ws_host_free) { if (b.pinned) (void)hipHostFree(b.p); else free(b.p); }
    g_ws_host_free.clear();
}
#define WSR_ALLOC(bytes) ws_pool_alloc(bytes)
#define WSR_FREE(p) ws_pool_free(p)
#include "ws_replay.h"

struct tf_ws_job {
    const float *field; const int32_t *markers; const int8_t *mask;
    int64_t T, H, W, N, NV, R;
    int n_nbr, depth0, depth_max, flags;
    hipStream_t s;
    bool raveled;
    WsGeom g;
    uint8_t *cls, *flag; int *scan, *cid; char *scan_tmp; size_t scan_bytes;
    int *d_flags; unsigned long long *d_cnt; char *seed_blocks;
    WsC c; WsQueues Q; int *org, *rank_dev;
    int h_cnt[WS_BATCH + 8];
    int depth; int64_t max_sweeps;
    unsigned long long h_amb[4];
    int64_t st[TF_WS_NSTATS];
    bool need_replay, replay_done, applied, sparse, plain, identity, coded;
    bool speculative;
    bool root_pending;
    bool sweeps_pending;
    bool speculate_fast; int levels_done;
    unsigned true_vmax; bool has_tie, spec_hit; int *subid;
    bool ranked, late_export; double ms_detour;
    bool device_ranks;
    u64 code_d; int64_t code_words, n_exc;
    int64_t M, S, nQ; unsigned vmax;
    WsHostBuf hb_val, hb_nbr, hb_rank, hb_sk, hb_sval, hb_sid;
    int64_t popped; int n_ranked; int replay_rc;
    double ms_export, ms_replay;
};

static double ws_now_ms() { timespec ts; clock_gettime(CLOCK_MONOTONIC, &ts); return ts.tv_sec * 1e3 + ts.tv_nsec * 1e-6; }
static bool ws_env(const char *name) { return getenv(name) != nullptr; }

static void ws_job_free(tf_ws_job *j)
{
    if (!j) return;
    ws_host_give(j->hb_val); ws_host_give(j->hb_nbr); ws_host_give(j->hb_rank);
    ws_host_give(j->hb_sk); ws_host_give(j->hb_sval); ws_host_give(j->hb_sid);
    delete j;
}

static int ws_to_host(void *dst, const void *src, size_t bytes, hipStream_t s)
{
    if (bytes == 0) return TF_OK;
    TF_CHECK_HIP(hipMemcpyAsync(dst, src, bytes, hipMemcpyDeviceToHost, s));
    return TF_OK;
}

static int ws_job_export(tf_ws_job *j)
{
    const double t_enter = ws_now_ms();
    j->device_ranks = false;
    hipStream_t s = j->s;
    const WsC &c = j->c;
    const int64_t R = j->R, N = j->N;
    const int nn = j->n_nbr;
    const unsigned nbr_blocks = (unsigned)((R + 255) / 256);
    static const bool ref_debug = ws_env("TF_WS_REF_DEBUG");
    const char *dense_env = getenv("TF_WS_REFERENCE_DENSE");
    const bool force_dense = dense_env != nullptr;
    j->plain = dense_env && atoi(dense_env) == 2;
    const unsigned h_vmax = j->vmax;
    const int64_t nb256 = (N + 255) / 256;
    TF_REQUIRE(nb256 < 0x7fffffffll, "tf_watershed: too many voxels for the seed numbering");
    int *n_seed = (int *)j->seed_blocks, *n_small = n_seed + nb256;
    long long *base_seed = (long long *)(((uintptr_t)(n_small + nb256) + 15) & ~(uintptr_t)15), *base_small = base_seed + nb256;
    size_t need = 0;
    (void)tf_exclusive_sum(nullptr, need, WsCountIter((const int *)nullptr, WsIntToLL()), (long long *)nullptr, (size_t)nb256);
    TF_REQUIRE(need <= j->scan_bytes, "tf_watershed: scan scratch too small for the seed numbering");
    int *d_any = j->d_flags + WS_BATCH + 6;
    TF_CHECK_HIP(hipMemsetAsync(d_any, 0, 2 * sizeof(int), s));
    hipLaunchKernelGGL(k_ws_seed_counts, dim3((unsigned)nb256), dim3(256), 0, s, (const uint8_t *)j->cls, j->field, N, h_vmax, n_seed, n_small, d_any);
    TF_CHECK_LAUNCH();
    size_t tb = j->scan_bytes;
    TF_CHECK_HIP(tf_exclusive_sum(j->scan_tmp, tb, WsCountIter(n_seed, WsIntToLL()), base_seed, (size_t)nb256, s));
    tb = j->scan_bytes;
    TF_CHECK_HIP(tf_exclusive_sum(j->scan_tmp, tb, WsCountIter(n_small, WsIntToLL()), base_small, (size_t)nb256, s));
    long long h_last[4] = {0, 0, 0, 0}; int h_lastc[2] = {0, 0};
    TF_CHECK_HIP(hipMemcpyAsync(&h_last[0], base_seed + nb256 - 1, sizeof(long long), hipMemcpyDeviceToHost, s));
    TF_CHECK_HIP(hipMemcpyAsync(&h_last[1], base_small + nb256 - 1, sizeof(long long), hipMemcpyDeviceToHost, s));
    TF_CHECK_HIP(hipMemcpyAsync(&h_lastc[0], n_seed + nb256 - 1, sizeof(int), hipMemcpyDeviceToHost, s));
    TF_CHECK_HIP(hipMemcpyAsync(&h_lastc[1], n_small + nb256 - 1, sizeof(int), hipMemcpyDeviceToHost, s));
    uint8_t *in_q = (uint8_t *)j->scan;
    int *subid = j->subid;
    TF_CHECK_HIP(hipMemsetAsync(in_q, 0, (size_t)R, s));
    hipLaunchKernelGGL(k_ws_sub_mark, dim3(nbr_blocks), dim3(256), 0, s, c, h_vmax, in_q, d_any + 1);
    TF_CHECK_LAUNCH();
    int h_any[2] = {0, 0};
    TF_CHECK_HIP(hipMemcpyAsync(h_any, d_any, 2 * sizeof(int), hipMemcpyDeviceToHost, s));
    int64_t nQ = 0;
    {
        const int rc = ws_scan_flags(in_q, subid, R, j->scan_tmp, j->scan_bytes, s, &nQ);
        if (rc) return rc;
    }
    j->M = h_last[0] + h_lastc[0]; j->S = h_last[1] + h_lastc[1];
    {
        const bool force_host = ws_env("TF_WS_REFERENCE_HOST");
        const int64_t S = j->S;
        char *tie_base = (char *)j->scan + tf_align_up((size_t)R, 256);
        const size_t tie_room = (size_t)j->NV * 4 > tf_align_up((size_t)R, 256) ? (size_t)j->NV * 4 - tf_align_up((size_t)R, 256) : 0;
        const size_t tie_need = tf_align_up((size_t)S * 8, 256) + 5 * tf_align_up((size_t)S * 4, 256) + 256;
        if (ref_debug)
            fprintf(stderr, "reference order: closed form? seed below the tie value %d, floodable pixel below it %d, S %lld, R %lld, room %zu of %zu\n",
                    h_any[0], h_any[1], (long long)S, (long long)R, tie_room, tie_need);
        if (!force_host && !force_dense && !h_any[0] && !h_any[1] && S > 0 && S <= R && S < 0x3fffffffll && tie_need <= tie_room) {
            long long *stg_k = (long long *)c.Rt; unsigned *stg_val = (unsigned *)c.Llo; int *stg_id = c.Lhi;
            hipLaunchKernelGGL(k_ws_small_list, dim3((unsigned)nb256), dim3(256), 0, s, (const uint8_t *)j->cls, (const int *)j->cid, j->field, N, h_vmax,
                               (const long long *)base_seed, (const long long *)base_small, (const int *)nullptr, stg_k, stg_val, stg_id);
            TF_CHECK_LAUNCH();
            long long k_max = 0;
            TF_CHECK_HIP(hipMemcpyAsync(&k_max, stg_k + S - 1, sizeof(long long), hipMemcpyDeviceToHost, s));
            TF_CHECK_HIP(hipStreamSynchronize(s));
            if (ref_debug && k_max >= j->M - S) fprintf(stderr, "reference order: closed form refused: small seed at heap position %lld of %lld\n", k_max, (long long)j->M);
            if (k_max < j->M - S) {
                TfArena ta(tie_base, tie_room);
                WsTie t;
                t.k = stg_k; t.sid = stg_id; t.S = (int)S; t.M = j->M;
                t.pos = ta.take<long long>(S); t.tj = ta.take<int>(S); t.c0 = ta.take<int>(S); t.c1 = ta.take<int>(S);
                t.size = ta.take<int>(S); t.pre = ta.take<int>(S); t.n_nodes = ta.take<int>(4);
                if (ta.ok()) {
                    const long long h_pos0 = 0; const int h_init[2] = {1, 0};
                    TF_CHECK_HIP(hipMemcpyAsync(t.pos, &h_pos0, sizeof(long long), hipMemcpyHostToDevice, s));
                    TF_CHECK_HIP(hipMemsetAsync(t.tj, 0, sizeof(int), s));
                    TF_CHECK_HIP(hipMemsetAsync(t.pre, 0, sizeof(int), s));
                    TF_CHECK_HIP(hipMemcpyAsync(t.n_nodes, h_init, sizeof(int), hipMemcpyHostToDevice, s));
                    int offs[80]; int n_lev = 0, lo = 0, hi = 1;
                    offs[0] = 0;
                    while (hi > lo && n_lev < 78) {
                        hipLaunchKernelGGL(k_ws_tie_level, dim3((unsigned)((hi - lo + 255) / 256)), dim3(256), 0, s, t, lo, hi);
                        TF_CHECK_LAUNCH();
                        int h_n = 0;
                        TF_CHECK_HIP(hipMemcpyAsync(&h_n, t.n_nodes, sizeof(int), hipMemcpyDeviceToHost, s));
                        TF_CHECK_HIP(hipStreamSynchronize(s));
                        offs[++n_lev] = hi;
                        lo = hi; hi = h_n < (int)S ? h_n : (int)S;
                        if (h_n > (int)S) { lo = hi = -1; break; }
                    }
                    if (hi == (int)S && lo == hi) {
                        for (int l = n_lev - 1; l >= 0; l--)
                            hipLaunchKernelGGL(k_ws_tie_sizes, dim3((unsigned)((offs[l + 1] - offs[l] + 255) / 256)), dim3(256), 0, s, t, offs[l], offs[l + 1]);
                        for (int l = 0; l < n_lev; l++)
                            hipLaunchKernelGGL(k_ws_tie_pre, dim3((unsigned)((offs[l + 1] - offs[l] + 255) / 256)), dim3(256), 0, s, t, offs[l], offs[l + 1]);
                        hipLaunchKernelGGL(k_ws_tie_default_ranks, dim3(nbr_blocks), dim3(256), 0, s, R, (int)S, j->rank_dev);
                        hipLaunchKernelGGL(k_ws_tie_scatter, dim3((unsigned)((S + 255) / 256)), dim3(256), 0, s, t, j->rank_dev);
                        TF_CHECK_LAUNCH();
                        TF_CHECK_HIP(hipStreamSynchronize(s));
                        j->device_ranks = true;
                        j->need_replay = false;
                        j->popped = S; j->n_ranked = (int)S;
                        j->ms_export = ws_now_ms() - t_enter;
                        if (ref_debug)
                            fprintf(stderr, "reference order: %lld seeds, %lld at the tie value (key %u) and nothing below it: pop ranks on the device "
                                    "(tree of %d levels), %.1f ms\n", (long long)j->M, (long long)S, h_vmax, n_lev, j->ms_export);
                        return TF_OK;
                    }
                }
            }
        }
    }
    j->identity = nQ * nn > 2 * R + 64;
    if (j->identity) nQ = R;
    j->nQ = nQ;
    j->sparse = !force_dense && j->S <= R;
    const double t_numbered = ws_now_ms();
    j->hb_val = ws_host_take((size_t)nQ * sizeof(unsigned), true);
    j->hb_nbr = ws_host_take((size_t)nQ * nn * sizeof(int), true);
    j->hb_rank = ws_host_take((size_t)nQ * sizeof(int), true);
    if (j->sparse) {
        j->hb_sk = ws_host_take((size_t)j->S * sizeof(long long), true);
        j->hb_sval = ws_host_take((size_t)j->S * sizeof(unsigned), true); j->hb_sid = ws_host_take((size_t)j->S * sizeof(int), true);
    }
    if (!j->hb_val.p || !j->hb_nbr.p || !j->hb_rank.p || (j->sparse && (!j->hb_sk.p || !j->hb_sval.p || !j->hb_sid.p))) {
        tf_set_error("tf_watershed: out of host memory for the reference-order replay");
        return TF_ENOMEM;
    }
    if (j->identity) {
        if (ws_to_host(j->hb_val.p, c.val, (size_t)R * sizeof(unsigned), s) || ws_to_host(j->hb_nbr.p, c.nbr, (size_t)R * nn * sizeof(int), s)) return TF_EHIP;
    } else {
        unsigned *stg_val = (unsigned *)j->Q.q[0]; int *stg_nbr = j->Q.q[1];
        hipLaunchKernelGGL(k_ws_sub_export, dim3(nbr_blocks), dim3(256), 0, s, c, h_vmax, (const uint8_t *)in_q, (const int *)subid, stg_val, stg_nbr);
        TF_CHECK_LAUNCH();
        if (ws_to_host(j->hb_val.p, stg_val, (size_t)nQ * sizeof(unsigned), s) || ws_to_host(j->hb_nbr.p, stg_nbr, (size_t)nQ * nn * sizeof(int), s)) return TF_EHIP;
    }
    const int *subid_or_null = j->identity ? nullptr : subid;
    if (j->sparse) {
        long long *stg_k = (long long *)c.Rt; unsigned *stg_val = (unsigned *)c.Llo; int *stg_id = c.Lhi;
        hipLaunchKernelGGL(k_ws_small_list, dim3((unsigned)nb256), dim3(256), 0, s, (const uint8_t *)j->cls, (const int *)j->cid, j->field, N, h_vmax,
                           (const long long *)base_seed, (const long long *)base_small, subid_or_null, stg_k, stg_val, stg_id);
        TF_CHECK_LAUNCH();
        if (ws_to_host(j->hb_sk.p, stg_k, (size_t)j->S * sizeof(long long), s) || ws_to_host(j->hb_sval.p, stg_val, (size_t)j->S * sizeof(unsigned), s) ||
            ws_to_host(j->hb_sid.p, stg_id, (size_t)j->S * sizeof(int), s)) return TF_EHIP;
        TF_CHECK_HIP(hipStreamSynchronize(s));
    } else {
        TF_CHECK_HIP(hipStreamSynchronize(s));
        const int64_t W = (j->M + 31) / 32 + 8;
        j->coded = 2 * W <= 2 * R + 64 && !ws_env("TF_WS_REFERENCE_NO_CODES");
        if (j->coded) {
            u64 *d_sample = (u64 *)j->Q.q[1];
            hipLaunchKernelGGL(k_ws_entry_sample, dim3(1), dim3(256), 0, s, (const uint8_t *)j->cls, (const int *)j->cid, j->field, N, h_vmax, d_sample);
            TF_CHECK_LAUNCH();
            u64 h_sample[256];
            TF_CHECK_HIP(hipMemcpyAsync(h_sample, d_sample, sizeof(h_sample), hipMemcpyDeviceToHost, s));
            TF_CHECK_HIP(hipStreamSynchronize(s));
            u64 D = 0ull; int best = 0;
            for (int a = 0; a < 256; a++) {
                if (!h_sample[a]) continue;
                int cnt = 0;
                for (int b = 0; b < 256; b++) cnt += h_sample[b] == h_sample[a];
                if (cnt > best) { best = cnt; D = h_sample[a]; }
            }
            j->code_d = D;
            int *n_exc = n_small; long long *base_exc = base_small;
            hipLaunchKernelGGL(k_ws_code_counts, dim3((unsigned)nb256), dim3(256), 0, s, (const uint8_t *)j->cls, (const int *)j->cid, j->field, N, h_vmax, D, n_exc);
            TF_CHECK_LAUNCH();
            tb = j->scan_bytes;
            TF_CHECK_HIP(tf_exclusive_sum(j->scan_tmp, tb, WsCountIter(n_exc, WsIntToLL()), base_exc, (size_t)nb256, s));
            long long h_e = 0; int h_ec = 0;
            TF_CHECK_HIP(hipMemcpyAsync(&h_e, base_exc + nb256 - 1, sizeof(long long), hipMemcpyDeviceToHost, s));
            TF_CHECK_HIP(hipMemcpyAsync(&h_ec, n_exc + nb256 - 1, sizeof(int), hipMemcpyDeviceToHost, s));
            TF_CHECK_HIP(hipStreamSynchronize(s));
            const int64_t E = h_e + h_ec;
            j->code_words = W; j->n_exc = E;
            j->hb_sval = ws_host_take((size_t)2 * W * sizeof(unsigned), true);
            j->hb_sid = ws_host_take((size_t)(E > 0 ? E : 1) * sizeof(u64), true);
            j->hb_sk = ws_host_take((size_t)(j->M + nQ + 1) * sizeof(u64), false);
            if (!j->hb_sval.p || !j->hb_sid.p || !j->hb_sk.p) { tf_set_error("tf_watershed: out of host memory for the reference-order replay"); return TF_ENOMEM; }
            unsigned *d_bits = (unsigned *)j->Q.q[0];
            TF_CHECK_HIP(hipMemsetAsync(d_bits, 0, (size_t)2 * W * sizeof(unsigned), s));
            const int64_t cap = R + 32;
            bool first = true;
            for (int64_t c0 = 0; first || c0 < E; c0 += cap, first = false) {
                const int64_t cnt = E - c0 < cap ? E - c0 : cap;
                u64 *stg = (u64 *)j->Q.q[1];
                hipLaunchKernelGGL(k_ws_seed_codes, dim3((unsigned)nb256), dim3(256), 0, s, (const uint8_t *)j->cls, (const int *)j->cid, j->field, N, h_vmax, D,
                                   (const long long *)base_seed, (const long long *)base_exc, subid_or_null, first ? 1 : 0, d_bits, d_bits + W, c0, cap, stg);
                TF_CHECK_LAUNCH();
                if (cnt > 0 && ws_to_host((u64 *)j->hb_sid.p + c0, stg, (size_t)cnt * sizeof(u64), s)) return TF_EHIP;
                if (first && ws_to_host(j->hb_sval.p, d_bits, (size_t)2 * W * sizeof(unsigned), s)) return TF_EHIP;
                TF_CHECK_HIP(hipStreamSynchronize(s));
            }
        } else {
            j->hb_sk = ws_host_take((size_t)(j->M + nQ + 1) * sizeof(u64), true);
            if (!j->hb_sk.p) { tf_set_error("tf_watershed: out of host memory for the reference-order replay"); return TF_ENOMEM; }
            const int64_t cap = R + 32;
            int turn = 0;
            for (int64_t c0 = 0; c0 < j->M; c0 += cap, turn ^= 1) {
                const int64_t cnt = j->M - c0 < cap ? j->M - c0 : cap;
                u64 *stg = (u64 *)j->Q.q[turn];
                hipLaunchKernelGGL(k_ws_seed_list, dim3((unsigned)nb256), dim3(256), 0, s, (const uint8_t *)j->cls, (const int *)j->cid, j->field, N,
                                   (const long long *)base_seed, c0, cap, subid_or_null, h_vmax, stg);
                TF_CHECK_LAUNCH();
                if (ws_to_host((u64 *)j->hb_sk.p + c0, stg, (size_t)cnt * sizeof(u64), s)) return TF_EHIP;
                if (turn) TF_CHECK_HIP(hipStreamSynchronize(s));
            }
            TF_CHECK_HIP(hipStreamSynchronize(s));
        }
    }
    j->need_replay = true;
    j->ms_export = ws_now_ms() - t_enter;
    if (ref_debug)
        fprintf(stderr, "reference order: %lld seeds, %lld at or below the tie value (key %u), %lld relevant pixels, sub-graph %lld%s, %s form; "
                "tie value + numbering %.1f ms, export %.1f ms\n", (long long)j->M, (long long)j->S, h_vmax, (long long)R, (long long)nQ,
                j->identity ? " (whole compact set)" : "", j->sparse ? "sparse" : (j->coded ? "dense (2 bits per seed + exceptions)" : "dense"), t_numbered - t_enter, ws_now_ms() - t_numbered);
    if (ref_debug && !j->sparse && j->coded)
        fprintf(stderr, "reference order: modal ballast entry %016llx, %lld exceptions\n", (unsigned long long)j->code_d, (long long)j->n_exc);
    return TF_OK;
}

static int ws_chain_levels(tf_ws_job *j)
{
    const unsigned nbr_blocks = (unsigned)((j->R + 255) / 256);
    for (int k = j->levels_done + 1; k < j->depth; k++) {
        hipLaunchKernelGGL(k_ws_init_level, dim3(nbr_blocks), dim3(256), 0, j->s, j->c.pix, j->c.C[k], j->R, 0, (const int *)nullptr);
        TF_CHECK_LAUNCH();
        int64_t sw = 0;
        const int rc = ws_run_phase(j->c, k, j->depth_max + 1, j->Q, j->s, j->max_sweeps, &sw);
        if (rc) return rc;
        j->st[2 + (k < 3 ? k - 1 : 2)] += sw;
        j->levels_done = k;
    }
    return TF_OK;
}

static int ws_root_and_check(tf_ws_job *j, bool ranked)
{
    hipStream_t s = j->s;
    const WsC &c = j->c;
    const int64_t R = j->R;
    const unsigned nbr_blocks = (unsigned)((R + 255) / 256);
    hipLaunchKernelGGL(k_ws_init_level, dim3(nbr_blocks), dim3(256), 0, s, c.pix, c.Rt, R, 1, ranked ? (const int *)j->rank_dev : (const int *)nullptr);
    hipLaunchKernelGGL(k_ws_init_labelset, dim3(nbr_blocks), dim3(256), 0, s, c.pix, j->markers, c.Llo, c.Lhi, R);
    TF_CHECK_LAUNCH();
    int64_t sw = 0;
    const int rc = ws_run_phase(c, j->depth, j->depth, j->Q, s, j->max_sweeps, &sw);
    if (rc) return rc;
    if (j->speculate_fast && j->depth == 1) j->st[1] = sw; else j->st[2 + (j->depth < 3 ? j->depth - 1 : 2)] += sw;
    j->st[12] += 1;
    TF_CHECK_HIP(hipMemsetAsync(j->org, 0, (size_t)R * sizeof(int), s));
    TF_CHECK_HIP(hipMemsetAsync(j->d_cnt, 0, 4 * sizeof(unsigned long long), s));
    hipLaunchKernelGGL(k_ws_origins, dim3(nbr_blocks), dim3(256), 0, s, c, j->depth, j->org);
    hipLaunchKernelGGL(k_ws_count_ambiguous, dim3(nbr_blocks), dim3(256), 0, s, c, j->org, j->d_cnt);
    TF_CHECK_LAUNCH();
    TF_CHECK_HIP(hipMemcpyAsync(j->h_amb, j->d_cnt, 4 * sizeof(unsigned long long), hipMemcpyDeviceToHost, s));
    TF_CHECK_HIP(hipStreamSynchronize(s));
    return TF_OK;
}

static int ws_job_sweeps(tf_ws_job *j)
{
    if (!j->sweeps_pending) return TF_OK;
    j->sweeps_pending = false;
    int64_t *st = j->st;
    const WsC &c = j->c;
    hipStream_t s = j->s;
    const unsigned nbr_blocks = (unsigned)((j->R + 255) / 256);
    int rc = ws_run_phase(c, 0, j->depth_max, j->Q, s, j->max_sweeps, &st[0], 29.0 * (double)j->N);
    if (rc) return rc;
    {
        TfProfScope ps(TFK_WS_SETUP, 0.0, s);
        hipLaunchKernelGGL(k_ws_edge_masks, dim3(nbr_blocks), dim3(256), 0, s, c, (u64 *)c.emask);
    }
    TF_CHECK_LAUNCH();
    j->speculate_fast = !((j->flags & TF_WS_SKIP_FAST_PATH) && j->depth0 > 1);
    st[5] = j->speculate_fast ? 0 : -1;
    j->depth = j->depth0;
    j->root_pending = true;
    if (j->speculate_fast) {
        j->depth = 1;
        rc = ws_root_and_check(j, false);
        if (rc) return rc;
        st[5] = j->h_amb[2] != 0;
        if (j->h_amb[2] == 0 || j->depth_max <= 1) j->root_pending = false;
        else j->depth = j->depth0;
    }
    if (j->root_pending) {
        rc = ws_chain_levels(j);
        if (rc) return rc;
    }
    st[8] = j->depth; st[9] = (int64_t)j->h_amb[0]; st[10] = (int64_t)j->h_amb[1]; st[11] = (int64_t)j->h_amb[2];
    return TF_OK;
}

static int ws_job_begin(tf_ws_job *j, const float *field, const int32_t *markers, const int8_t *mask,
                        const float *fwd, const float *bwd, int64_t T, int64_t H, int64_t W,
                        const int8_t *nbr_host, int n_nbr, int depth0, int depth_max, int flags,
                        void *ws, size_t ws_bytes, void *stream,
                        const WsRavel *rv = nullptr, const int64_t *rv_locs = nullptr, int64_t rv_n_locs = 0, int64_t spec_key = -1)
{
    int64_t *st = j->st;
    for (int i = 0; i < TF_WS_NSTATS; i++) st[i] = 0;
    TF_REQUIRE((flags & ~(TF_WS_SKIP_FAST_PATH | TF_WS_REFERENCE_ORDER | TF_WS_DEFER_SWEEPS)) == 0, "tf_watershed: unknown flag");
    TF_REQUIRE(field && markers && ws, "tf_watershed: null pointer");
    if (!rv) {
        TF_REQUIRE(fwd && bwd && nbr_host, "tf_watershed: null pointer");
        TF_REQUIRE(T > 0 && H > 0 && W > 0 && H < (1 << 15) && W < (1 << 15) && T < 65536, "tf_watershed: bad shape");
    }
    TF_REQUIRE(n_nbr > 0 && n_nbr <= WS_MAX_NBR, "tf_watershed: bad neighbour count");
    TF_REQUIRE(depth0 >= 1 && depth0 <= depth_max && depth_max <= WS_MAX_DEPTH, "tf_watershed: bad chain_depth");
    const int64_t N = rv ? rv->n : T * H * W;
    TF_REQUIRE(N > 0 && (rv ? N <= 0x7fffffffll : N <= (1ll << 36)), "tf_watershed: too many voxels per call (use time windows)");
    const int64_t NV = rv ? N : ws_virtual_voxels(T, H, W);
    if (ws_bytes < ws_full_bytes(N, NV) + ws_compact_bytes(1, n_nbr, depth_max)) { tf_set_error("tf_watershed: workspace too small"); return TF_ENOMEM; }
    hipStream_t s = (hipStream_t)stream;
    WsGeom &g = j->g;
    g.T = T; g.H = (int)H; g.W = (int)W; g.plane = H * W; g.n_nbr = n_nbr; g.n_tx = (int)((W + WS_TILE - 1) / WS_TILE);
    for (int i = 0; i < n_nbr && !rv; i++) {
        g.dt[i] = nbr_host[i * 3]; g.dy[i] = nbr_host[i * 3 + 1]; g.dx[i] = nbr_host[i * 3 + 2];
        TF_REQUIRE(abs(g.dt[i]) <= 1 && abs(g.dy[i]) <= 1 && abs(g.dx[i]) <= 1, "tf_watershed: neighbour offset out of range");
    }
    j->field = field; j->markers = markers; j->mask = mask; j->T = T; j->H = H; j->W = W; j->N = N; j->NV = NV;
    j->n_nbr = n_nbr; j->depth0 = depth0; j->depth_max = depth_max; j->flags = flags; j->s = s; j->raveled = rv != nullptr;
    TfArena ar(ws, ws_bytes);
    uint8_t *cls = ar.take<uint8_t>(N), *flag = ar.take<uint8_t>(NV);
    int *scan = ar.take<int>(NV), *cid = ar.take<int>(N);
    const size_t scan_bytes = ws_scan_temp_bytes(NV);
    char *scan_tmp = ar.take<char>(scan_bytes ? scan_bytes : 1);
    int *d_flags = ar.take<int>(WS_BATCH + 8);
    unsigned long long *d_cnt = ar.take<unsigned long long>(4);
    j->seed_blocks = ar.take<char>((size_t)((N + 255) / 256) * 24 + 64);
    if (!ar.ok()) { tf_set_error("tf_watershed: workspace too small"); return TF_ENOMEM; }
    j->cls = cls; j->flag = flag; j->scan = scan; j->cid = cid; j->scan_tmp = scan_tmp; j->scan_bytes = scan_bytes;
    j->d_flags = d_flags; j->d_cnt = d_cnt;

    dim3 block(64, 4, 1), grid(rv ? 1 : (g.W + 63) / 64, rv ? 1 : (g.H + 3) / 4, rv ? 1 : (unsigned)T);
    const unsigned nb1 = (unsigned)((N + 255) / 256);
    int64_t R = 0;
    bool tiles = false;
    {
        TfProfScope ps(TFK_WS_SETUP, 29.0 * (double)N, s);
        if (rv) {
            int *d_bad = d_flags + WS_BATCH + 5;
            TF_CHECK_HIP(hipMemsetAsync(d_bad, 0, sizeof(int), s));
            TF_CHECK_HIP(hipMemsetAsync(flag, 0, (size_t)N, s));
            if (rv_n_locs > 0)
                hipLaunchKernelGGL(k_wsr_seeds, dim3((unsigned)((rv_n_locs + 255) / 256)), dim3(256), 0, s, rv_locs, rv_n_locs, N, flag, d_bad);
            hipLaunchKernelGGL(k_wsr_classify, dim3(nb1), dim3(256), 0, s, (const uint8_t *)flag, markers, mask, N, cls, d_bad);
            TF_CHECK_LAUNCH();
            int h_bad = 0;
            TF_CHECK_HIP(hipMemcpyAsync(&h_bad, d_bad, sizeof(int), hipMemcpyDeviceToHost, s));
            TF_CHECK_HIP(hipStreamSynchronize(s));
            TF_REQUIRE(h_bad != 1, "tf_watershed_raveled: marker_locations must be strictly ascending indices into the arrays (np.flatnonzero order)");
            TF_REQUIRE(h_bad != 2, "tf_watershed_raveled: output must be non-zero at every marker location (_watershed.pyx:241-244)");
            hipLaunchKernelGGL(k_wsr_relevant, dim3(nb1), dim3(256), 0, s, (const uint8_t *)cls, *rv, flag);
        } else {
            if ((uintptr_t)markers % 16 == 0 && (uintptr_t)cls % 4 == 0 && (!mask || (uintptr_t)mask % 4 == 0))
                hipLaunchKernelGGL(k_ws_classify4, dim3((unsigned)(((N + 3) / 4 + 255) / 256)), dim3(256), 0, s, markers, mask, N, cls);
            else hipLaunchKernelGGL(k_ws_classify, dim3(nb1), dim3(256), 0, s, markers, mask, N, cls);
            if (NV > N) TF_CHECK_HIP(hipMemsetAsync(flag, 0, (size_t)NV, s));
            bool faces = n_nbr == 6;
            for (int i = 0; faces && i < 6; i++) faces = abs(g.dt[i]) + abs(g.dy[i]) + abs(g.dx[i]) == 1;
            for (int i = 0; faces && i < 6; i++) for (int k = 0; k < i; k++) faces = faces && !(g.dt[i] == g.dt[k] && g.dy[i] == g.dy[k] && g.dx[i] == g.dx[k]);
            if (faces && W % 4 == 0 && (uintptr_t)cls % 4 == 0 && (uintptr_t)flag % 4 == 0 && (uintptr_t)fwd % 16 == 0 && (uintptr_t)bwd % 16 == 0)
                hipLaunchKernelGGL(k_ws_relevant6x4, dim3((unsigned)((W / 4 + 63) / 64), (unsigned)((H + 3) / 4), (unsigned)T), block, 0, s,
                                   (const uint8_t *)cls, fwd, bwd, g, flag);
            else if (n_nbr == 6) hipLaunchKernelGGL(k_ws_relevant<6>, grid, block, 0, s, cls, fwd, bwd, g, flag);
            else if (n_nbr == 18) hipLaunchKernelGGL(k_ws_relevant<18>, grid, block, 0, s, cls, fwd, bwd, g, flag);
            else if (n_nbr == 26) hipLaunchKernelGGL(k_ws_relevant<26>, grid, block, 0, s, cls, fwd, bwd, g, flag);
            else hipLaunchKernelGGL(k_ws_relevant<0>, grid, block, 0, s, cls, fwd, bwd, g, flag);
        }
        TF_CHECK_LAUNCH();
        const int64_t n_tiles = NV / 256;
        size_t tile_scan_bytes = 0;
        if (!rv) (void)tf_exclusive_sum(nullptr, tile_scan_bytes, (const long long *)nullptr, (long long *)nullptr, (size_t)n_tiles);
        tiles = !rv && NV % 256 == 0 && n_tiles > 0 && n_tiles < 0x7fffffffll && tile_scan_bytes <= scan_bytes;
        if (tiles) {
            long long *t_count = (long long *)scan, *t_base = t_count + n_tiles;
            hipLaunchKernelGGL(k_ws_count_tiles, dim3((unsigned)((n_tiles + 3) / 4)), dim3(256), 0, s, (const uint8_t *)flag, n_tiles, t_count);
            size_t tb = scan_bytes;
            TF_CHECK_HIP(tf_exclusive_sum(scan_tmp, tb, (const long long *)t_count, t_base, (size_t)n_tiles, s));
            long long h_last[2] = {0, 0};
            TF_CHECK_HIP(hipMemcpyAsync(&h_last[0], t_base + n_tiles - 1, sizeof(long long), hipMemcpyDeviceToHost, s));
            TF_CHECK_HIP(hipMemcpyAsync(&h_last[1], t_count + n_tiles - 1, sizeof(long long), hipMemcpyDeviceToHost, s));
            TF_CHECK_HIP(hipStreamSynchronize(s));
            R = h_last[0] + h_last[1];
            TF_REQUIRE(R <= 0x3fffff00ll, "tf_watershed: more than 2^30 relevant pixels in one call (use time windows)");
        } else {
            const int rc_scan = ws_scan_flags(flag, scan, NV, scan_tmp, scan_bytes, s, &R);
            if (rc_scan) return rc_scan;
        }
    }
    st[6] = R;
    j->R = R;
    if (ws_bytes < ws_full_bytes(N, NV) + ws_compact_bytes(R > 0 ? R : 1, n_nbr, depth_max)) {
        tf_set_error("tf_watershed: workspace too small for %lld relevant pixels", (long long)R);
        return TF_ENOMEM;
    }
    if (rv) hipLaunchKernelGGL(k_ws_cid, dim3(nb1), dim3(256), 0, s, cls, flag, scan, N, cid);
    else if (tiles) hipLaunchKernelGGL(k_ws_cid_tiles, dim3((unsigned)((NV / 256 + 3) / 4)), dim3(256), 0, s, (const uint8_t *)cls, (const uint8_t *)flag,
                                       (const long long *)((long long *)scan + NV / 256), NV / 256, g, cid);
    else hipLaunchKernelGGL(k_ws_cid_tiled, grid, block, 0, s, (const uint8_t *)cls, (const uint8_t *)flag, (const int *)scan, g, cid);
    TF_CHECK_LAUNCH();
    WsC &c = j->c; memset(&c, 0, sizeof(c));
    c.R = R; c.n_nbr = n_nbr;
    j->org = nullptr; j->rank_dev = nullptr;
    j->depth = 0;
    if (R > 0) {
        u64 *pix = ar.take<u64>(R); unsigned *val = ar.take<unsigned>(R); int *nbr = ar.take<int>(R * n_nbr);
        c.pix = pix; c.val = val; c.nbr = nbr;
        c.KM = ar.take<u64>(2 * R);
        for (int k = 1; k < depth_max; k++) c.C[k] = ar.take<u64>(R);
        c.Rt = ar.take<u64>(R);
        c.Llo = ar.take<int>(R); c.Lhi = ar.take<int>(R); j->org = ar.take<int>(R);
        j->rank_dev = ar.take<int>(R);
        u64 *emask = ar.take<u64>(R);
        c.emask = emask;
        WsQueues &Q = j->Q;
        Q.qcap = (int)(2 * R < 0x7fffff00ll ? 2 * R : 0x7fffff00ll);
        Q.q[0] = ar.take<int>(2 * R + 64); Q.q[1] = ar.take<int>(2 * R + 64); Q.inq = ar.take<int>(R);
        j->subid = ar.take<int>(R);
        Q.cnt = d_flags; Q.h_cnt = j->h_cnt; Q.processed = &st[7];
        if (!ar.ok()) { tf_set_error("tf_watershed: workspace too small"); return TF_ENOMEM; }
        int *d_nan = d_flags + WS_BATCH + 4;
        TF_CHECK_HIP(hipMemsetAsync(d_nan, 0, sizeof(int), s));
        {
            TfProfScope ps(TFK_WS_SETUP, 0.0, s);
            if (rv) hipLaunchKernelGGL(k_wsr_compact, dim3(nb1), dim3(256), 0, s, field, (const int *)cid, *rv, pix, val, nbr, c.KM, d_nan);
            else if (n_nbr == 6) hipLaunchKernelGGL(k_ws_compact<6>, grid, block, 0, s, field, fwd, bwd, cid, g, pix, val, nbr, c.KM, d_nan);
            else if (n_nbr == 18) hipLaunchKernelGGL(k_ws_compact<18>, grid, block, 0, s, field, fwd, bwd, cid, g, pix, val, nbr, c.KM, d_nan);
            else if (n_nbr == 26) hipLaunchKernelGGL(k_ws_compact<26>, grid, block, 0, s, field, fwd, bwd, cid, g, pix, val, nbr, c.KM, d_nan);
            else hipLaunchKernelGGL(k_ws_compact<0>, grid, block, 0, s, field, fwd, bwd, cid, g, pix, val, nbr, c.KM, d_nan);
        }
        TF_CHECK_LAUNCH();
        {
            int h_nan = 0;
            TF_CHECK_HIP(hipMemcpyAsync(&h_nan, d_nan, sizeof(int), hipMemcpyDeviceToHost, s));
            TF_CHECK_HIP(hipStreamSynchronize(s));
            if (h_nan) {
                tf_set_error("tf_watershed: the field is NaN at a floodable pixel or at a seed next to one; the pop order of the "
                             "reference's heap is undefined for NaN keys (detection.get_combined_edge_field maps NaN to +inf)");
                return TF_EINVAL;
            }
        }
        const unsigned nbr_blocks = (unsigned)((R + 255) / 256);
        const int64_t max_sweeps = rv ? 4096 + 2 * R : 4096 + 512 * (T + H + W);
        j->max_sweeps = max_sweeps;
        if ((flags & TF_WS_REFERENCE_ORDER) && spec_key >= 0) {
            j->vmax = (unsigned)spec_key;
            j->speculative = true;
            const int rc_x = ws_job_export(j);
            if (rc_x) return rc_x;
        }
        (void)nbr_blocks;
        j->sweeps_pending = true;
        if (flags & TF_WS_DEFER_SWEEPS) return TF_OK;
        return ws_job_sweeps(j);
    }
    st[8] = j->depth; st[9] = (int64_t)j->h_amb[0]; st[10] = (int64_t)j->h_amb[1]; st[11] = (int64_t)j->h_amb[2];
    return TF_OK;
}

static int ws_job_replay(tf_ws_job *j)
{
    if (!j->need_replay || j->replay_done) return j->replay_rc;
    const double t0 = ws_now_ms();
    int n_ranked = 0;
    double phase[2] = {0.0, 0.0};
    if (j->sparse)
        j->popped = ws_reference_ranks_sparse(j->M, j->S, (const long long *)j->hb_sk.p, (const unsigned *)j->hb_sval.p, (const int *)j->hb_sid.p,
                                              j->nQ, (const unsigned *)j->hb_val.p, (const int *)j->hb_nbr.p, j->n_nbr, j->vmax, (int *)j->hb_rank.p, &n_ranked, phase);
    else {
        const WsSeedCodes codes{(const uint32_t *)j->hb_sval.p, (const uint32_t *)j->hb_sval.p + (j->coded ? j->code_words : 0), j->code_d, (const u64 *)j->hb_sid.p};
        if (j->plain) {
            if (j->coded) wsr_expand(j->M, codes, (u64 *)j->hb_sk.p);
            j->popped = ws_reference_ranks_plain(j->M, (const u64 *)j->hb_sk.p, nullptr, j->nQ, (const unsigned *)j->hb_val.p,
                                                 (const int *)j->hb_nbr.p, j->n_nbr, j->vmax, (int *)j->hb_rank.p, &n_ranked);
        } else
            j->popped = ws_reference_ranks_dense(j->M, (u64 *)j->hb_sk.p, j->nQ, (const unsigned *)j->hb_val.p, (const int *)j->hb_nbr.p,
                                                 j->n_nbr, j->vmax, (int *)j->hb_rank.p, &n_ranked, phase, j->coded ? &codes : nullptr);
    }
    j->n_ranked = n_ranked;
    j->replay_done = true;
    j->ms_replay = ws_now_ms() - t0;
    if (j->popped < 0) { tf_set_error("tf_watershed: out of host memory for the reference-order replay"); j->replay_rc = TF_ENOMEM; }
    static const bool ref_debug = ws_env("TF_WS_REF_DEBUG");
    if (ref_debug) fprintf(stderr, "reference order: %s%s replay %.1f ms (%lld pops, %d markers ranked; heap build %.1f ms, pops %.1f ms)\n", j->speculative ? "speculative " : "",
                           j->sparse ? "sparse" : (j->plain ? "plain" : "dense"), j->ms_replay, (long long)j->popped, n_ranked, phase[0], phase[1]);
    return j->replay_rc;
}

static int ws_upload_ranks(tf_ws_job *j)
{
    hipStream_t s = j->s;
    const unsigned nbr_blocks = (unsigned)((j->R + 255) / 256);
    int *stg_rank = j->Q.q[0];
    TF_CHECK_HIP(hipMemcpyAsync(stg_rank, j->hb_rank.p, (size_t)j->nQ * sizeof(int), hipMemcpyHostToDevice, s));
    hipLaunchKernelGGL(k_ws_scatter_ranks, dim3(nbr_blocks), dim3(256), 0, s, j->identity ? (const uint8_t *)nullptr : (const uint8_t *)j->scan,
                       (const int *)j->subid, (const int *)stg_rank, j->n_ranked, j->R, j->rank_dev);
    TF_CHECK_LAUNCH();
    TF_CHECK_HIP(hipStreamSynchronize(s));
    return TF_OK;
}

static int ws_job_finish(tf_ws_job *j, int32_t *labels, uint8_t *amb_out)
{
    TF_REQUIRE(labels, "tf_watershed: null pointer");
    hipStream_t s = j->s;
    int64_t *st = j->st;
    const WsC &c = j->c;
    const int64_t R = j->R, N = j->N;
    const unsigned nb1 = (unsigned)((N + 255) / 256);
    static const bool ref_debug = ws_env("TF_WS_REF_DEBUG");
    bool ranked = j->ranked;
    if (R > 0 && j->sweeps_pending) {
        const int rc_s = ws_job_sweeps(j);
        if (rc_s) return rc_s;
    }
    if (R > 0 && j->late_export) {
        j->late_export = false;
        int rc = ws_job_replay(j);
        if (rc) return rc;
        const double t0 = ws_now_ms();
        rc = ws_upload_ranks(j);
        if (rc) return rc;
        ranked = j->ranked = true;
        rc = ws_root_and_check(j, true);
        if (rc) return rc;
        j->applied = true;
        j->ms_detour += j->ms_export + j->ms_replay + (ws_now_ms() - t0);
        st[13] = j->popped; st[14] = j->sparse ? j->S : j->M;
        st[15] = (int64_t)(j->ms_detour * 1000.0);
    } else if (R > 0 && j->root_pending) {
        j->root_pending = false;
        const unsigned nbr_blocks = (unsigned)((R + 255) / 256);
        int rc;
        double &ms_detour = j->ms_detour;
        if (j->need_replay) {
            rc = ws_job_replay(j);
            if (rc) return rc;
            const double t0 = ws_now_ms();
            rc = ws_upload_ranks(j);
            if (rc) return rc;
            ranked = j->ranked = true;
            ms_detour = j->ms_export + j->ms_replay + (ws_now_ms() - t0);
        } else if (j->device_ranks) {
            ranked = j->ranked = true;
            ms_detour = j->ms_export;
        }
        for (;;) {
            rc = ws_root_and_check(j, ranked);
            if (rc) return rc;
            if (j->h_amb[2] == 0 || j->depth >= j->depth_max) break;
            j->depth += 1;
            rc = ws_chain_levels(j);
            if (rc) return rc;
        }
        if ((j->flags & TF_WS_REFERENCE_ORDER) && j->h_amb[1] > 0 && j->h_amb[2] == 0) {
            unsigned *d_vmax = (unsigned *)(j->d_cnt + 3);
            TF_CHECK_HIP(hipMemsetAsync(d_vmax, 0, sizeof(unsigned), s));
            hipLaunchKernelGGL(k_ws_tie_value_max, dim3(nbr_blocks), dim3(256), 0, s, c, (const int *)j->org, j->field, ranked ? 1 : 0, d_vmax);
            TF_CHECK_LAUNCH();
            unsigned h_vmax = 0;
            TF_CHECK_HIP(hipMemcpyAsync(&h_vmax, d_vmax, sizeof(unsigned), hipMemcpyDeviceToHost, s));
            TF_CHECK_HIP(hipStreamSynchronize(s));
            j->true_vmax = h_vmax; j->has_tie = true;
            if (ranked && h_vmax <= j->vmax) {
                j->applied = true;
                j->spec_hit = true;
            } else {
                if (ref_debug && ranked) fprintf(stderr, "reference order: the guessed tie value (key %u) was too low (true key %u): export again\n", j->vmax, h_vmax);
                ws_host_give(j->hb_val); ws_host_give(j->hb_nbr); ws_host_give(j->hb_rank);
                ws_host_give(j->hb_sk); ws_host_give(j->hb_sval); ws_host_give(j->hb_sid);
                j->need_replay = false; j->replay_done = false; j->speculative = false; j->replay_rc = TF_OK;
                j->vmax = h_vmax;
                rc = ws_job_export(j);
                if (rc) return rc;
                if (j->device_ranks) {
                    ranked = j->ranked = true;
                    rc = ws_root_and_check(j, true);
                    if (rc) return rc;
                    j->applied = true;
                    ms_detour += j->ms_export;
                    st[13] = j->popped; st[14] = j->S; st[15] = (int64_t)(ms_detour * 1000.0);
                    goto labels_out;
                }
                j->late_export = true;
                st[8] = j->depth; st[9] = (int64_t)j->h_amb[0]; st[10] = (int64_t)j->h_amb[1]; st[11] = (int64_t)j->h_amb[2];
                return TF_WS_REPLAY_PENDING;
            }
        }
        if (j->need_replay && j->replay_done) {
            st[13] = j->popped; st[14] = j->sparse ? j->S : j->M;
            st[15] = (int64_t)(ms_detour * 1000.0);
        } else if (j->device_ranks) {
            st[13] = j->popped; st[14] = j->S; st[15] = (int64_t)(ms_detour * 1000.0);
        }
    }
labels_out:
    st[8] = j->depth; st[9] = (int64_t)j->h_amb[0]; st[10] = (int64_t)j->h_amb[1]; st[11] = (int64_t)j->h_amb[2];
    {
        TfProfScope ps(TFK_WS_LABELS, 12.0 * (double)N, s);
        if (j->raveled) { if (R > 0) hipLaunchKernelGGL(k_wsr_labels, dim3(nb1), dim3(256), 0, s, (const int *)j->cid, (const u64 *)c.Rt, c.pix, ranked ? 1 : 0, labels, N); }
        else hipLaunchKernelGGL(k_ws_labels, dim3(nb1), dim3(256), 0, s, j->markers, j->cid, c.Rt, c.pix, ranked ? 1 : 0, c.Llo, c.Lhi, j->org, labels,
                                R > 0 ? amb_out : nullptr, N);
    }
    TF_CHECK_LAUNCH();
    if (R == 0 && amb_out) TF_CHECK_HIP(hipMemsetAsync(amb_out, 0, (size_t)N, s));
    TF_CHECK_HIP(hipStreamSynchronize(s));
    if (st[11] > 0) {
        tf_set_error("tf_watershed: %lld pixel(s) still tie at chain depth %d (the compared chains are cut off); "
                     "labels written, but they may differ from the reference there: raise max_depth",
                     (long long)st[11], j->depth);
        return TF_EDEPTH;
    }
    return (st[9] > 0 && !j->applied) ? TF_WS_AMBIGUOUS : TF_OK;
}

static tf_ws_job *ws_job_new()
{
    tf_ws_job *j = new (std::nothrow) tf_ws_job;
    if (!j) return nullptr;
    memset((void *)j, 0, sizeof(*j));
    return j;
}

static int ws_run(const float *field, const int32_t *markers, const int8_t *mask,
                  const float *fwd, const float *bwd, int64_t T, int64_t H, int64_t W,
                  const int8_t *nbr_host, int n_nbr, int depth0, int depth_max, int flags, int32_t *labels,
                  uint8_t *amb_out, void *ws, size_t ws_bytes, int64_t *st, void *stream,
                  const WsRavel *rv = nullptr, const int64_t *rv_locs = nullptr, int64_t rv_n_locs = 0)
{
    TF_REQUIRE(!(flags & TF_WS_DEFER_SWEEPS), "tf_watershed: unknown flag (TF_WS_DEFER_SWEEPS is tf_watershed_begin's)");
    for (int i = 0; i < TF_WS_NSTATS; i++) st[i] = 0;
    TF_REQUIRE(labels, "tf_watershed: null pointer");
    tf_ws_job *j = ws_job_new();
    if (!j) { tf_set_error("tf_watershed: out of host memory"); return TF_ENOMEM; }
    int rc = ws_job_begin(j, field, markers, mask, fwd, bwd, T, H, W, nbr_host, n_nbr, depth0, depth_max, flags, ws, ws_bytes, stream, rv, rv_locs, rv_n_locs);
    if (rc == TF_OK) {
        rc = ws_job_finish(j, labels, amb_out);
        if (rc == TF_WS_REPLAY_PENDING) rc = ws_job_finish(j, labels, amb_out);
    }
    for (int i = 0; i < TF_WS_NSTATS; i++) st[i] = j->st[i];
    ws_job_free(j);
    return rc;
}

extern "C" int tf_watershed_begin(const float *field, const int32_t *markers, const int8_t *mask,
                                  const float *fwd, const float *bwd, int64_t T, int64_t H, int64_t W,
                                  const int8_t *nbr_host, int n_nbr, int chain_depth, int max_depth, int flags,
                                  int64_t guessed_tie_key, void *ws, size_t ws_bytes, int64_t *stats_host, void *stream, void **job_out)
{
    TF_REQUIRE(job_out, "tf_watershed_begin: null pointer");
    *job_out = nullptr;
    TF_REQUIRE(guessed_tie_key >= -1 && guessed_tie_key <= 0xFFFFFFFFll, "tf_watershed_begin: guessed_tie_key must be -1 or a 32-bit ordered key");
    tf_ws_job *j = ws_job_new();
    if (!j) { tf_set_error("tf_watershed: out of host memory"); return TF_ENOMEM; }
    const int rc = ws_job_begin(j, field, markers, mask, fwd, bwd, T, H, W, nbr_host, n_nbr, chain_depth, max_depth, flags, ws, ws_bytes, stream,
                                nullptr, nullptr, 0, guessed_tie_key);
    if (stats_host) for (int i = 0; i < TF_WS_NSTATS; i++) stats_host[i] = j->st[i];
    if (rc != TF_OK) { ws_job_free(j); return rc; }
    *job_out = j;
    return TF_OK;
}
extern "C" int tf_watershed_needs_replay(const void *job) { return job && ((const tf_ws_job *)job)->need_replay ? 1 : 0; }
extern "C" int tf_watershed_sweeps(void *job, int64_t *stats_host)
{
    TF_REQUIRE(job, "tf_watershed_sweeps: null job");
    tf_ws_job *j = (tf_ws_job *)job;
    const int rc = j->R > 0 ? ws_job_sweeps(j) : TF_OK;
    if (stats_host) for (int i = 0; i < TF_WS_NSTATS; i++) stats_host[i] = j->st[i];
    return rc;
}
extern "C" int tf_watershed_replay(void *job)
{
    TF_REQUIRE(job, "tf_watershed_replay: null job");
    return ws_job_replay((tf_ws_job *)job);
}
extern "C" int tf_watershed_job_info(const void *job, int64_t *info);
extern "C" int tf_watershed_finish(void *job, int32_t *labels, uint8_t *ambiguous, int64_t *stats_host, int64_t *info_host)
{
    TF_REQUIRE(job, "tf_watershed_finish: null job");
    tf_ws_job *j = (tf_ws_job *)job;
    const int rc = ws_job_finish(j, labels, ambiguous);
    if (stats_host) for (int i = 0; i < TF_WS_NSTATS; i++) stats_host[i] = j->st[i];
    if (info_host) (void)tf_watershed_job_info(j, info_host);
    if (rc == TF_WS_REPLAY_PENDING) return rc;
    ws_job_free(j);
    return rc;
}
extern "C" void tf_watershed_abandon(void *job) { ws_job_free((tf_ws_job *)job); }
extern "C" int tf_watershed_set_stream(void *job, void *stream)
{
    TF_REQUIRE(job, "tf_watershed_set_stream: null job");
    ((tf_ws_job *)job)->s = (hipStream_t)stream;
    return TF_OK;
}
extern "C" int tf_watershed_job_info(const void *job, int64_t *info)
{
    TF_REQUIRE(job && info, "tf_watershed_job_info: null pointer");
    const tf_ws_job *j = (const tf_ws_job *)job;
    info[0] = j->need_replay ? (j->sparse ? 1 : 2) : (j->device_ranks ? 3 : 0);
    info[1] = j->M; info[2] = j->S; info[3] = j->nQ; info[4] = j->R;
    info[5] = (int64_t)(j->ms_export * 1000.0); info[6] = j->replay_done ? (int64_t)(j->ms_replay * 1000.0) : -1;
    info[7] = j->has_tie ? (int64_t)j->true_vmax : -1;
    info[8] = j->speculative ? 1 : 0; info[9] = j->spec_hit ? 1 : 0; info[10] = (j->need_replay || j->device_ranks) ? (int64_t)j->vmax : -1; info[11] = j->device_ranks ? 1 : 0;
    return TF_OK;
}

extern "C" int tf_watershed_ex2(const float *field, const int32_t *markers, const int8_t *mask,
                                const float *fwd, const float *bwd, int64_t T, int64_t H, int64_t W,
                                const int8_t *nbr_host, int n_nbr, int chain_depth, int max_depth, int flags,
                                int32_t *labels, uint8_t *ambiguous, void *ws, size_t ws_bytes,
                                int64_t *stats_host, void *stream)
{
    int64_t st[TF_WS_NSTATS];
    const int rc = ws_run(field, markers, mask, fwd, bwd, T, H, W, nbr_host, n_nbr, chain_depth, max_depth, flags, labels,
                          ambiguous, ws, ws_bytes, st, stream);
    if (stats_host) for (int i = 0; i < TF_WS_NSTATS; i++) stats_host[i] = st[i];
    return rc;
}

extern "C" int tf_watershed_ex(const float *field, const int32_t *markers, const int8_t *mask,
                               const float *fwd, const float *bwd, int64_t T, int64_t H, int64_t W,
                               const int8_t *nbr_host, int n_nbr, int chain_depth, int flags, int32_t *labels,
                               void *ws, size_t ws_bytes, int64_t *stats_host, void *stream)
{
    int64_t st[TF_WS_NSTATS];
    const int rc = ws_run(field, markers, mask, fwd, bwd, T, H, W, nbr_host, n_nbr, chain_depth, chain_depth, flags, labels,
                          nullptr, ws, ws_bytes, st, stream);
    if (stats_host) for (int i = 0; i < 8; i++) stats_host[i] = st[i];
    return rc;
}

extern "C" int tf_watershed(const float *field, const int32_t *markers, const int8_t *mask,
                            const float *fwd, const float *bwd, int64_t T, int64_t H, int64_t W,
                            const int8_t *nbr_host, int n_nbr, int chain_depth, int32_t *labels,
                            void *ws, size_t ws_bytes, int64_t *stats_host, void *stream)
{
    return tf_watershed_ex(field, markers, mask, fwd, bwd, T, H, W, nbr_host, n_nbr, chain_depth, 0, labels,
                           ws, ws_bytes, stats_host, stream);
}

extern "C" size_t tf_watershed_raveled_workspace_bytes(int64_t n, int n_structure, int max_depth, int64_t max_relevant)
{
    if (n <= 0 || n > 0x7fffffffll || max_depth < 1 || max_depth > WS_MAX_DEPTH || n_structure < 1 || n_structure > WS_MAX_NBR) return 0;
    if (max_relevant <= 0 || max_relevant > n) max_relevant = n;
    return ws_full_bytes(n, n) + ws_compact_bytes(max_relevant, n_structure, max_depth);
}

extern "C" int tf_watershed_raveled_ex(const float *image, int64_t n, const int64_t *marker_locations, int64_t n_markers,
                                       const int64_t *structure_host, int n_structure,
                                       const int32_t *forward_offset, const int32_t *backward_offset,
                                       const int32_t *forward_offset_locations_host, const int32_t *backward_offset_locations_host,
                                       const int8_t *mask, const int32_t *strides_host, int n_strides, double compactness,
                                       int32_t *output, int wsl, int max_depth, int flags, void *ws, size_t ws_bytes,
                                       int64_t *stats_host, void *stream)
{
    TF_REQUIRE((flags & ~TF_WS_REFERENCE_ORDER) == 0, "tf_watershed_raveled_ex: unknown flag");
    TF_REQUIRE(image && structure_host && forward_offset && backward_offset && forward_offset_locations_host &&
               backward_offset_locations_host && mask && output && ws && (marker_locations || n_markers == 0),
               "tf_watershed_raveled: null pointer");
    (void)strides_host; (void)n_strides;
    TF_REQUIRE(compactness == 0.0 && !wsl, "tf_watershed_raveled: compactness > 0 and watershed lines are the dead branches of the "
               "reference's call path (watershed.py:151-164 passes 0 and False) and are not built");
    TF_REQUIRE(n_structure > 0 && n_structure <= WS_MAX_NBR, "tf_watershed_raveled: bad neighbour count");
    WsRavel rv; rv.n = n; rv.n_nbr = n_structure; rv.foff = forward_offset; rv.boff = backward_offset;
    for (int i = 0; i < n_structure; i++) {
        rv.structure[i] = structure_host[i]; rv.floc[i] = forward_offset_locations_host[i]; rv.bloc[i] = backward_offset_locations_host[i];
    }
    int64_t st[TF_WS_NSTATS];
    const int d0 = max_depth < 3 ? max_depth : 3;
    const int rc = ws_run(image, output, mask, nullptr, nullptr, 0, 0, 0, nullptr, n_structure, d0, max_depth, flags, output,
                          nullptr, ws, ws_bytes, st, stream, &rv, marker_locations, n_markers);
    if (stats_host) for (int i = 0; i < TF_WS_NSTATS; i++) stats_host[i] = st[i];
    return rc;
}

extern "C" int tf_watershed_raveled(const float *image, int64_t n, const int64_t *marker_locations, int64_t n_markers,
                                    const int64_t *structure_host, int n_structure,
                                    const int32_t *forward_offset, const int32_t *backward_offset,
                                    const int32_t *forward_offset_locations_host, const int32_t *backward_offset_locations_host,
                                    const int8_t *mask, const int32_t *strides_host, int n_strides, double compactness,
                                    int32_t *output, int wsl, int max_depth, void *ws, size_t ws_bytes,
                                    int64_t *stats_host, void *stream)
{
    return tf_watershed_raveled_ex(image, n, marker_locations, n_markers, structure_host, n_structure, forward_offset,
                                   backward_offset, forward_offset_locations_host, backward_offset_locations_host, mask,
                                   strides_host, n_strides, compactness, output, wsl, max_depth, 0, ws, ws_bytes, stats_host, stream);
}
```

Before: 1023.

## Compact watershed setup over relevant pixels and skip background work in CCL

The cid kernels now write the compact pixel list directly, so the compact kernels iterate only over the R relevant pixels instead of scanning the whole volume. The CCL init kernel no longer writes parent for background pixels. Flatten and number kernels read the input mask instead, and a vectorised flatten4 kernel is added. The seed/export kernels gain 16-wide variants with tail handling, and profiling scopes are added for the new categories. The risks are scattered writes into pix and extra mask reads in CCL.

```diff
diff --git a/tobac_flow_amd/csrc/capi.hip b/tobac_flow_amd/csrc/capi.hip
--- a/tobac_flow_amd/csrc/capi.hip
+++ b/tobac_flow_amd/csrc/capi.hip
@@ -29,7 +29,8 @@
 std::vector<hipEvent_t> g_free;
 std::mutex g_mu;
 const char *g_names[TFK_COUNT] = {"to8bit_pair", "fb_gaussian_blur", "fb_resize", "fb_polyexp", "fb_update_matrices",
-    "fb_blur_solve", "fb_iteration_fused", "smooth_flow", "convolve", "sobel", "ws_setup", "ws_relax_sweep", "ws_labels", "vr_prepare", "vr_system", "vr_sor", "binary_morph"};
+    "fb_blur_solve", "fb_iteration_fused", "smooth_flow", "convolve", "sobel", "ws_setup", "ws_relax_sweep", "ws_labels", "vr_prepare", "vr_system", "vr_sor", "binary_morph",
+    "ws_export", "label_ccl", "seeds_glue"};
 hipEvent_t get_event() {
     if (!g_free.empty()) { hipEvent_t e = g_free.back(); g_free.pop_back(); return e; }
     hipEvent_t e; (void)hipEventCreate(&e); return e;
diff --git a/tobac_flow_amd/csrc/morph.hip b/tobac_flow_amd/csrc/morph.hip
--- a/tobac_flow_amd/csrc/morph.hip
+++ b/tobac_flow_amd/csrc/morph.hip
@@ -215,6 +215,7 @@
     TF_REQUIRE(lower != upper, "tf_linearise: lower and upper thresholds must have different values");
     int flip = 0;
     if (lower > upper) { const double t = lower; lower = upper; upper = t; flip = 1; }
+    TfProfScope ps(TFK_SEEDS_GLUE, 8.0 * (double)n, (hipStream_t)stream);
     if (tf_vec4_ok({field, out}, {}))
         hipLaunchKernelGGL(k_linearise4, dim3((unsigned)(((n + 3) / 4 + 255) / 256)), dim3(256), 0, (hipStream_t)stream, field, n,
                            (float)lower, (float)upper, flip, out);
@@ -268,6 +269,7 @@
 extern "C" int tf_apply_lut(const int32_t *labels, int64_t n, const int32_t *lut, int n_lut, int32_t *out, void *stream)
 {
     TF_REQUIRE(labels && lut && out && n > 0 && n_lut > 0, "tf_apply_lut: bad arguments");
+    TfProfScope ps(TFK_SEEDS_GLUE, 8.0 * (double)n, (hipStream_t)stream);
     hipLaunchKernelGGL(k_apply_lut, dim3((unsigned)((n + 255) / 256)), dim3(256), 0, (hipStream_t)stream, labels, n, lut, n_lut, out);
     TF_CHECK_LAUNCH();
     return TF_OK;
@@ -299,6 +301,7 @@
 extern "C" int tf_apply_lut_keep_nonpositive(const int32_t *labels, int64_t n, const int32_t *lut, int n_lut, int32_t *out, void *stream)
 {
     TF_REQUIRE(labels && lut && out && n > 0 && n_lut > 0, "tf_apply_lut_keep_nonpositive: bad arguments");
+    TfProfScope ps(TFK_SEEDS_GLUE, 8.0 * (double)n, (hipStream_t)stream);
     if (tf_vec4_ok({labels, out}, {}))
         hipLaunchKernelGGL(k_apply_lut_keep4, dim3((unsigned)(((n + 3) / 4 + 255) / 256)), dim3(256), 0, (hipStream_t)stream, labels, n, lut, n_lut, out);
     else
@@ -364,6 +367,7 @@
 extern "C" int tf_field_masks(const float *field, int64_t n, uint8_t *ge1, uint8_t *le0_or_nan, uint8_t *isnan_out, void *stream)
 {
     TF_REQUIRE(field && ge1 && le0_or_nan && isnan_out && n > 0, "tf_field_masks: bad arguments");
+    TfProfScope ps(TFK_SEEDS_GLUE, 7.0 * (double)n, (hipStream_t)stream);
     if (tf_vec4_ok({field}, {ge1, le0_or_nan, isnan_out}))
         hipLaunchKernelGGL(k_field_masks4, dim3((unsigned)(((n + 3) / 4 + 255) / 256)), dim3(256), 0, (hipStream_t)stream, field, n, ge1, le0_or_nan, isnan_out);
     else
@@ -374,6 +378,7 @@
 extern "C" int tf_merge_seeds(const int32_t *comp, const uint8_t *bg, const uint8_t *isnan_in, int64_t n, int32_t *seeds, void *stream)
 {
     TF_REQUIRE(comp && bg && isnan_in && seeds && n > 0, "tf_merge_seeds: bad arguments");
+    TfProfScope ps(TFK_SEEDS_GLUE, 10.0 * (double)n, (hipStream_t)stream);
     if (tf_vec4_ok({comp, seeds}, {bg, isnan_in}))
         hipLaunchKernelGGL(k_merge_seeds4, dim3((unsigned)(((n + 3) / 4 + 255) / 256)), dim3(256), 0, (hipStream_t)stream, comp, bg, isnan_in, n, seeds);
     else
@@ -428,8 +433,7 @@
     const int64_t plane = (int64_t)H * W, p = t * plane + (int64_t)y * W + x;
     const bool on = inside && in[p] != 0;
     const unsigned long long m = __ballot(on);
-    if (!inside) return;
-    if (!on) { parent[p] = -1; return; }
+    if (!inside || !on) return;
     const int lane = threadIdx.x;
     const unsigned long long zeros_below = ~m & ((1ull << lane) - 1ull);
     const int head = zeros_below ? 64 - __clzll((long long)zeros_below) : 0;
@@ -461,14 +465,39 @@
 }
 
 __global__ void __launch_bounds__(256)
-k_ccl_flatten(int64_t n, int *__restrict__ parent, uint8_t *__restrict__ isroot) {
-    const int64_t i = (int64_t)blockIdx.x * blockDim.x + threadIdx.x;
-    if (i >= n) return;
-    const int p = parent[i];
-    if (p < 0) { isroot[i] = 0; return; }
+k_ccl_flatten(const uint8_t *__restrict__ in, int64_t n, int *__restrict__ parent, uint8_t *__restrict__ isroot) {
+    const int64_t i = (int64_t)blockIdx.x * blockDim.x + threadIdx.x;
+    if (i >= n) return;
+    if (!in[i]) { isroot[i] = 0; return; }
     const int r = ccl_find(parent, (int)i);
     parent[i] = r;
     isroot[i] = r == (int)i;
+}
+__global__ void __launch_bounds__(256)
+k_ccl_flatten4(const uint8_t *__restrict__ in, int64_t n, int *__restrict__ parent, uint8_t *__restrict__ isroot) {
+    const int64_t i = ((int64_t)blockIdx.x * blockDim.x + threadIdx.x) * 4;
+    if (i >= n) return;
+    if (i + 3 < n) {
+        const uint32_t m = *(const uint32_t *)(in + i);
+        uint32_t out = 0;
+        if (m) {
+#pragma unroll
+            for (int j = 0; j < 4; j++) {
+                if (!((m >> (8 * j)) & 0xffu)) continue;
+                const int r = ccl_find(parent, (int)i + j);
+                parent[i + j] = r;
+                out |= (uint32_t)(r == (int)i + j) << (8 * j);
+            }
+        }
+        *(uint32_t *)(isroot + i) = out;
+    } else {
+        for (int64_t j = i; j < n; j++) {
+            if (!in[j]) { isroot[j] = 0; continue; }
+            const int r = ccl_find(parent, (int)j);
+            parent[j] = r;
+            isroot[j] = r == (int)j;
+        }
+    }
 }
 
 __global__ void __launch_bounds__(256)
@@ -499,22 +528,27 @@
 }
 
 __global__ void __launch_bounds__(256)
-k_ccl_number(int64_t n, const int *__restrict__ parent, const int *__restrict__ rank, int32_t *__restrict__ labels) {
-    const int64_t i = (int64_t)blockIdx.x * blockDim.x + threadIdx.x;
-    if (i >= n) return;
-    const int r = parent[i];
-    labels[i] = r < 0 ? 0 : rank[r] + 1;
-}
-__global__ void __launch_bounds__(256)
-k_ccl_number4(int64_t n, const int *__restrict__ parent, const int *__restrict__ rank, int32_t *__restrict__ labels) {
+k_ccl_number(const uint8_t *__restrict__ in, int64_t n, const int *__restrict__ parent, const int *__restrict__ rank, int32_t *__restrict__ labels) {
+    const int64_t i = (int64_t)blockIdx.x * blockDim.x + threadIdx.x;
+    if (i >= n) return;
+    labels[i] = in[i] ? rank[parent[i]] + 1 : 0;
+}
+__global__ void __launch_bounds__(256)
+k_ccl_number4(const uint8_t *__restrict__ in, int64_t n, const int *__restrict__ parent, const int *__restrict__ rank, int32_t *__restrict__ labels) {
     const int64_t i = ((int64_t)blockIdx.x * blockDim.x + threadIdx.x) * 4;
     if (i >= n) return;
     if (i + 3 < n) {
-        const int4 r = *(const int4 *)(parent + i);
-        const int a = rank[r.x < 0 ? 0 : r.x], b = rank[r.y < 0 ? 0 : r.y], c = rank[r.z < 0 ? 0 : r.z], d = rank[r.w < 0 ? 0 : r.w];
-        *(int4 *)(labels + i) = make_int4(r.x < 0 ? 0 : a + 1, r.y < 0 ? 0 : b + 1, r.z < 0 ? 0 : c + 1, r.w < 0 ? 0 : d + 1);
+        const uint32_t m = *(const uint32_t *)(in + i);
+        int4 out = make_int4(0, 0, 0, 0);
+        if (m) {
+            const int4 r = *(const int4 *)(parent + i);
+            const bool f0 = m & 0xffu, f1 = m & 0xff00u, f2 = m & 0xff0000u, f3 = m & 0xff000000u;
+            const int a = rank[f0 ? r.x : 0], b = rank[f1 ? r.y : 0], c = rank[f2 ? r.z : 0], d = rank[f3 ? r.w : 0];
+            out = make_int4(f0 ? a + 1 : 0, f1 ? b + 1 : 0, f2 ? c + 1 : 0, f3 ? d + 1 : 0);
+        }
+        *(int4 *)(labels + i) = out;
     } else {
-        for (int64_t j = i; j < n; j++) { const int r = parent[j]; labels[j] = r < 0 ? 0 : rank[r] + 1; }
+        for (int64_t j = i; j < n; j++) labels[j] = in[j] ? rank[parent[j]] + 1 : 0;
     }
 }
 
@@ -558,6 +592,8 @@
     for (int i = 0; i < tp.n; i++) runs = runs || (tp.dt[i] == 0 && tp.dy[i] == 0 && tp.dx[i] == 1);
     static const bool no_runs_env = getenv("TF_CCL_NO_RUNS") != nullptr;
     if (no_runs_env) runs = false;
+    {
+    TfProfScope ps(TFK_LABEL_CCL, 5.0 * (double)n, s);
     if (runs) hipLaunchKernelGGL(k_ccl_init_runs, grid, block, 0, s, in, T, (int)H, (int)W, parent);
     else if (tf_vec4_ok({parent}, {in})) hipLaunchKernelGGL(k_ccl_init4, dim3((unsigned)(((n + 3) / 4 + 255) / 256)), dim3(256), 0, s, in, n, parent);
     else hipLaunchKernelGGL(k_ccl_init, dim3(nb), dim3(256), 0, s, in, n, parent);
@@ -567,14 +603,16 @@
             if (tp.dx[j] == 0 && tp.dt[j] == tp.dt[i] && tp.dy[j] == tp.dy[i]) sibling |= 1u << i;
     if (tp.n && runs) hipLaunchKernelGGL(k_ccl_union<true>, grid, block, 0, s, in, T, (int)H, (int)W, tp, sibling, parent);
     else if (tp.n) hipLaunchKernelGGL(k_ccl_union<false>, grid, block, 0, s, in, T, (int)H, (int)W, tp, sibling, parent);
-    hipLaunchKernelGGL(k_ccl_flatten, dim3(nb), dim3(256), 0, s, n, parent, isroot);
+    if (tf_vec4_ok({parent}, {in, isroot})) hipLaunchKernelGGL(k_ccl_flatten4, dim3((unsigned)(((n + 3) / 4 + 255) / 256)), dim3(256), 0, s, in, n, parent, isroot);
+    else hipLaunchKernelGGL(k_ccl_flatten, dim3(nb), dim3(256), 0, s, in, n, parent, isroot);
     TF_CHECK_LAUNCH();
     const unsigned nb4 = (unsigned)((nblk + 3) / 4);
     hipLaunchKernelGGL(k_ccl_count_roots, dim3(nb4), dim3(256), 0, s, n, (const uint8_t *)isroot, block_count);
     TF_CHECK_HIP(tf_exclusive_sum(scan_tmp, scan_bytes, (const int *)block_count, block_base, (size_t)nblk, s));
     hipLaunchKernelGGL(k_ccl_rank_roots, dim3(nb4), dim3(256), 0, s, n, (const uint8_t *)isroot, (const int *)block_base, rank);
-    if (tf_vec4_ok({parent, labels}, {})) hipLaunchKernelGGL(k_ccl_number4, dim3((unsigned)(((n + 3) / 4 + 255) / 256)), dim3(256), 0, s, n, parent, rank, labels);
-    else hipLaunchKernelGGL(k_ccl_number, dim3(nb), dim3(256), 0, s, n, parent, rank, labels);
+    if (tf_vec4_ok({parent, labels}, {in})) hipLaunchKernelGGL(k_ccl_number4, dim3((unsigned)(((n + 3) / 4 + 255) / 256)), dim3(256), 0, s, in, n, parent, rank, labels);
+    else hipLaunchKernelGGL(k_ccl_number, dim3(nb), dim3(256), 0, s, in, n, parent, rank, labels);
+    }
     TF_CHECK_LAUNCH();
     int last_base = 0, last_count = 0;
     TF_CHECK_HIP(hipMemcpyAsync(&last_base, block_base + nblk - 1, sizeof(int), hipMemcpyDeviceToHost, s));
diff --git a/tobac_flow_amd/csrc/tf_common.h b/tobac_flow_amd/csrc/tf_common.h
--- a/tobac_flow_amd/csrc/tf_common.h
+++ b/tobac_flow_amd/csrc/tf_common.h
@@ -67,6 +67,9 @@
     TFK_TO8BIT = 0, TFK_FB_BLUR, TFK_FB_RESIZE, TFK_FB_POLYEXP, TFK_FB_MATRICES, TFK_FB_BLUR_SOLVE, TFK_FB_ITER,
     TFK_SMOOTH, TFK_CONVOLVE, TFK_SOBEL, TFK_WS_SETUP, TFK_WS_RELAX, TFK_WS_LABELS, TFK_VR_PREPARE, TFK_VR_SYSTEM, TFK_VR_SOR,
     TFK_MORPH,
+    TFK_WS_EXPORT,
+    TFK_LABEL_CCL,
+    TFK_SEEDS_GLUE,
     TFK_COUNT
 };
 extern bool g_tf_prof_on;
diff --git a/tobac_flow_amd/csrc/watershed.hip b/tobac_flow_amd/csrc/watershed.hip
--- a/tobac_flow_amd/csrc/watershed.hip
+++ b/tobac_flow_amd/csrc/watershed.hip
@@ -177,14 +177,19 @@
 
 __global__ void __launch_bounds__(256)
 k_ws_cid_tiled(const uint8_t *__restrict__ cls, const uint8_t *__restrict__ flag, const int *__restrict__ scan, WsGeom g,
-               int *__restrict__ cid)
+               int *__restrict__ cid, u64 *__restrict__ pix)
 {
     const int x = blockIdx.x * 64 + threadIdx.x, y = blockIdx.y * 4 + threadIdx.y;
     const int64_t t = blockIdx.z;
     if (x >= g.W || y >= g.H) return;
     const int64_t p = t * g.plane + (int64_t)y * g.W + x, k = ws_vpos(g, t, y, x);
     int c = -1;
-    if (flag[k]) c = cls[p] == 1 ? scan[k] : -2 - scan[k];
+    if (flag[k]) {
+        const int id = scan[k];
+        const bool marker = cls[p] != 1;
+        c = marker ? -2 - id : id;
+        pix[id] = (u64)p | (marker ? WS_MARKER_BIT : 0ull);
+    }
     cid[p] = c;
 }
 
@@ -202,7 +207,7 @@
 }
 __global__ void __launch_bounds__(256)
 k_ws_cid_tiles(const uint8_t *__restrict__ cls, const uint8_t *__restrict__ flag, const long long *__restrict__ base, int64_t n_tiles,
-               WsGeom g, int *__restrict__ cid)
+               WsGeom g, int *__restrict__ cid, u64 *__restrict__ pix)
 {
     const int64_t b = (int64_t)blockIdx.x * 4 + (threadIdx.x >> 6);
     if (b >= n_tiles) return;
@@ -223,7 +228,13 @@
 #pragma unroll
     for (int j = 0; j < 4; j++) {
         c[j] = -1;
-        if (f[j]) { const int id = id0 + run; c[j] = cls[p0 + j] == 1 ? id : -2 - id; run++; }
+        if (f[j]) {
+            const int id = id0 + run;
+            const bool marker = cls[p0 + j] != 1;
+            c[j] = marker ? -2 - id : id;
+            pix[id] = (u64)(p0 + j) | (marker ? WS_MARKER_BIT : 0ull);
+            run++;
+        }
     }
     if (x0 + 3 < g.W && (((uintptr_t)(cid + p0)) & 15) == 0) *(int4 *)(cid + p0) = make_int4(c[0], c[1], c[2], c[3]);
     else {
@@ -235,35 +246,38 @@
 
 __global__ void __launch_bounds__(256)
 k_ws_cid(const uint8_t *__restrict__ cls, const uint8_t *__restrict__ flag, const int *__restrict__ scan, int64_t n,
-         int *__restrict__ cid)
+         int *__restrict__ cid, u64 *__restrict__ pix)
 {
     const int64_t i = (int64_t)blockIdx.x * blockDim.x + threadIdx.x;
     if (i >= n) return;
     int c = -1;
-    if (flag[i]) c = cls[i] == 1 ? scan[i] : -2 - scan[i];
+    if (flag[i]) {
+        const int id = scan[i];
+        const bool marker = cls[i] != 1;
+        c = marker ? -2 - id : id;
+        pix[id] = (u64)i | (marker ? WS_MARKER_BIT : 0ull);
+    }
     cid[i] = c;
 }
 
 template <int NN>
 __global__ void __launch_bounds__(256)
 k_ws_compact(const float *__restrict__ field, const float *__restrict__ fwd, const float *__restrict__ bwd,
-             const int *__restrict__ cid, WsGeom g, u64 *__restrict__ pix, unsigned *__restrict__ val,
+             const int *__restrict__ cid, WsGeom g, int64_t R, const u64 *__restrict__ pix, unsigned *__restrict__ val,
              int *__restrict__ nbr, u64 *__restrict__ KM, int *__restrict__ nan_flag)
 {
-    const int x = blockIdx.x * 64 + threadIdx.x, y = blockIdx.y * 4 + threadIdx.y;
-    const int64_t t = blockIdx.z;
-    if (x >= g.W || y >= g.H) return;
-    const int64_t p = t * g.plane + (int64_t)y * g.W + x;
-    const int c = cid[p];
-    if (c == -1) return;
-    const bool marker = c < 0;
-    const int64_t id = marker ? -2 - c : c;
+    const int64_t id = (int64_t)blockIdx.x * blockDim.x + threadIdx.x;
+    if (id >= R) return;
+    const u64 px = pix[id];
+    const bool marker = (px & WS_MARKER_BIT) != 0ull;
+    const int64_t p = (int64_t)(px & ~WS_MARKER_BIT);
+    const int64_t t = p / g.plane;
+    const int r = (int)(p - t * g.plane), y = r / g.W, x = r - y * g.W;
     const float2 fw = ((const float2 *)fwd)[p], bw = ((const float2 *)bwd)[p];
     const int fx = ws_round_flow(fw.x), fy = ws_round_flow(fw.y), bx = ws_round_flow(bw.x), by = ws_round_flow(bw.y);
     const float fv = field[p];
     if (fv != fv) *nan_flag = 1;
     const unsigned v = ws_ordkey(fv);
-    pix[id] = (u64)p | (marker ? WS_MARKER_BIT : 0ull);
     val[id] = v;
     if (NN > 0) {
         int cn[NN > 0 ? NN : 1];
@@ -332,20 +346,18 @@
 }
 
 __global__ void __launch_bounds__(256)
-k_wsr_compact(const float *__restrict__ image, const int *__restrict__ cid, WsRavel g, u64 *__restrict__ pix,
+k_wsr_compact(const float *__restrict__ image, const int *__restrict__ cid, WsRavel g, int64_t R, const u64 *__restrict__ pix,
               unsigned *__restrict__ val, int *__restrict__ nbr, u64 *__restrict__ KM, int *__restrict__ nan_flag)
 {
-    const int64_t p = (int64_t)blockIdx.x * blockDim.x + threadIdx.x;
-    if (p >= g.n) return;
-    const int c = cid[p];
-    if (c == -1) return;
-    const bool marker = c < 0;
-    const int64_t id = marker ? -2 - c : c;
+    const int64_t id = (int64_t)blockIdx.x * blockDim.x + threadIdx.x;
+    if (id >= R) return;
+    const u64 px = pix[id];
+    const bool marker = (px & WS_MARKER_BIT) != 0ull;
+    const int64_t p = (int64_t)(px & ~WS_MARKER_BIT);
     const int fo = g.foff[p], bo = g.boff[p];
     const float fv = image[p];
     if (fv != fv) *nan_flag = 1;
     const unsigned v = ws_ordkey(fv);
-    pix[id] = (u64)p | (marker ? WS_MARKER_BIT : 0ull);
     val[id] = v;
     for (int i = 0; i < g.n_nbr; i++) {
         const int64_t n = wsr_neighbour(g, p, fo, bo, i);
@@ -698,11 +710,11 @@
 }
 
 __global__ void __launch_bounds__(256)
-k_ws_seed_counts(const uint8_t *__restrict__ cls, const float *__restrict__ field, int64_t n, unsigned vmax,
+k_ws_seed_counts(const uint8_t *__restrict__ cls, const float *__restrict__ field, int64_t n, unsigned vmax, int64_t blk0,
                  int *__restrict__ n_seed, int *__restrict__ n_small, int *__restrict__ any_below)
 {
     __shared__ int part[2][4];
-    const int64_t i = (int64_t)blockIdx.x * 256 + threadIdx.x;
+    const int64_t blk = blk0 + blockIdx.x, i = blk * 256 + threadIdx.x;
     const bool sd = i < n && cls[i] == 2;
     const unsigned key = sd ? ws_ordkey(field[i]) : 0u;
     const bool sm = sd && key <= vmax;
@@ -711,17 +723,17 @@
     if ((threadIdx.x & 63) == 0) { part[0][threadIdx.x >> 6] = __popcll(ms); part[1][threadIdx.x >> 6] = __popcll(mm); }
     __syncthreads();
     if (threadIdx.x == 0) {
-        n_seed[blockIdx.x] = part[0][0] + part[0][1] + part[0][2] + part[0][3];
-        n_small[blockIdx.x] = part[1][0] + part[1][1] + part[1][2] + part[1][3];
-    }
-}
-__global__ void __launch_bounds__(256)
-k_ws_small_list(const uint8_t *__restrict__ cls, const int *__restrict__ cid, const float *__restrict__ field, int64_t n, unsigned vmax,
+        n_seed[blk] = part[0][0] + part[0][1] + part[0][2] + part[0][3];
+        n_small[blk] = part[1][0] + part[1][1] + part[1][2] + part[1][3];
+    }
+}
+__global__ void __launch_bounds__(256)
+k_ws_small_list(const uint8_t *__restrict__ cls, const int *__restrict__ cid, const float *__restrict__ field, int64_t n, unsigned vmax, int64_t blk0,
                 const long long *__restrict__ base_seed, const long long *__restrict__ base_small, const int *__restrict__ subid,
                 long long *__restrict__ out_k, unsigned *__restrict__ out_val, int *__restrict__ out_id)
 {
     __shared__ int part[2][4];
-    const int64_t i = (int64_t)blockIdx.x * 256 + threadIdx.x;
+    const int64_t blk = blk0 + blockIdx.x, i = blk * 256 + threadIdx.x;
     unsigned key = 0;
     const bool sd = i < n && cls[i] == 2;
     bool sm = false;
@@ -732,21 +744,22 @@
     __syncthreads();
     if (!sm) return;
     const unsigned long long below = (1ull << lane) - 1ull;
-    long long k = base_seed[blockIdx.x] + __popcll(ms & below), slot = base_small[blockIdx.x] + __popcll(mm & below);
+    long long k = base_seed[blk] + __popcll(ms & below), slot = base_small[blk] + __popcll(mm & below);
     for (int w = 0; w < wave; w++) { k += part[0][w]; slot += part[1][w]; }
     const int c = cid[i];
     const int id = c <= -2 ? -2 - c : -1;
     out_k[slot] = k; out_val[slot] = key; out_id[slot] = (id >= 0 && subid) ? subid[id] : id;
 }
 __global__ void __launch_bounds__(256)
-k_ws_seed_list(const uint8_t *__restrict__ cls, const int *__restrict__ cid, const float *__restrict__ field, int64_t n,
+k_ws_seed_list(const uint8_t *__restrict__ cls, const int *__restrict__ cid, const float *__restrict__ field, int64_t n, int64_t blk0,
                const long long *__restrict__ base_seed, int64_t c0, int64_t cap, const int *__restrict__ subid, unsigned vmax,
                u64 *__restrict__ out_entry)
 {
     __shared__ int part[4];
-    const long long b0 = base_seed[blockIdx.x];
+    const int64_t blk = blk0 + blockIdx.x;
+    const long long b0 = base_seed[blk];
     if (b0 >= c0 + cap || b0 + 256 <= c0) return;
-    const int64_t i = (int64_t)blockIdx.x * 256 + threadIdx.x;
+    const int64_t i = blk * 256 + threadIdx.x;
     const bool sd = i < n && cls[i] == 2;
     const unsigned long long ms = __ballot(sd);
     const int lane = threadIdx.x & 63, wave = threadIdx.x >> 6;
@@ -792,25 +805,27 @@
 }
 __global__ void __launch_bounds__(256)
 k_ws_code_counts(const uint8_t *__restrict__ cls, const int *__restrict__ cid, const float *__restrict__ field, int64_t n, unsigned vmax, u64 D,
-                 int *__restrict__ n_exc)
+                 int64_t blk0, int *__restrict__ n_exc)
 {
     __shared__ int part[4];
-    const WsSeedCode r = ws_seed_code(cls, cid, field, (int64_t)blockIdx.x * 256 + threadIdx.x, n, vmax, D);
+    const int64_t blk = blk0 + blockIdx.x;
+    const WsSeedCode r = ws_seed_code(cls, cid, field, blk * 256 + threadIdx.x, n, vmax, D);
     const unsigned long long m = __ballot(r.x);
     if ((threadIdx.x & 63) == 0) part[threadIdx.x >> 6] = __popcll(m);
     __syncthreads();
-    if (threadIdx.x == 0) n_exc[blockIdx.x] = part[0] + part[1] + part[2] + part[3];
+    if (threadIdx.x == 0) n_exc[blk] = part[0] + part[1] + part[2] + part[3];
 }
 __global__ void __launch_bounds__(256)
 k_ws_seed_codes(const uint8_t *__restrict__ cls, const int *__restrict__ cid, const float *__restrict__ field, int64_t n, unsigned vmax, u64 D,
-                const long long *__restrict__ base_seed, const long long *__restrict__ base_exc, const int *__restrict__ subid,
+                int64_t blk0, const long long *__restrict__ base_seed, const long long *__restrict__ base_exc, const int *__restrict__ subid,
                 int write_bits, unsigned *__restrict__ bits_d, unsigned *__restrict__ bits_l, int64_t c0, int64_t cap, u64 *__restrict__ exc)
 {
     __shared__ int part_s[4], part_x[4];
     __shared__ unsigned lb_d[9], lb_l[9];
-    if (!write_bits) { const long long b0 = base_exc[blockIdx.x]; if (b0 >= c0 + cap || b0 + 256 <= c0) return; }
+    const int64_t blk = blk0 + blockIdx.x;
+    if (!write_bits) { const long long b0 = base_exc[blk]; if (b0 >= c0 + cap || b0 + 256 <= c0) return; }
     if (threadIdx.x < 9) { lb_d[threadIdx.x] = 0u; lb_l[threadIdx.x] = 0u; }
-    const WsSeedCode r = ws_seed_code(cls, cid, field, (int64_t)blockIdx.x * 256 + threadIdx.x, n, vmax, D);
+    const WsSeedCode r = ws_seed_code(cls, cid, field, blk * 256 + threadIdx.x, n, vmax, D);
     const unsigned long long ms = __ballot(r.seed), mx = __ballot(r.x);
     const int lane = threadIdx.x & 63, wave = threadIdx.x >> 6;
     if (lane == 0) { part_s[wave] = __popcll(ms); part_x[wave] = __popcll(mx); }
@@ -826,7 +841,7 @@
             const int t = threadIdx.x % 9;
             const unsigned *lb = threadIdx.x < 9 ? lb_d : lb_l;
             unsigned *bits = threadIdx.x < 9 ? bits_d : bits_l;
-            const long long kb = base_seed[blockIdx.x];
+            const long long kb = base_seed[blk];
             const int sh = (int)(kb & 31);
             const unsigned lo = t < 8 ? lb[t] : 0u, hi = t > 0 ? lb[t - 1] : 0u;
             const unsigned word = sh ? ((lo << sh) | (hi >> (32 - sh))) : lo;
@@ -834,11 +849,204 @@
         }
     }
     if (r.x) {
-        const long long slot = base_exc[blockIdx.x] + xl - c0;
+        const long long slot = base_exc[blk] + xl - c0;
         if (slot >= 0 && slot < cap) {
             int id = r.id;
             if (id >= 0 && subid) id = subid[id];
             exc[slot] = ((u64)r.key << 32) | 0x80000000ull | (u64)(unsigned)(id + 1);
+        }
+    }
+}
+struct WsLane16 { unsigned seed; float f[16]; };
+__device__ __forceinline__ void ws_lane16_load(const uint8_t *__restrict__ cls, const float *__restrict__ field, int64_t i0, bool f16, WsLane16 &L)
+{
+    const uint4 c = *(const uint4 *)(cls + i0);
+    const uint32_t w[4] = {c.x, c.y, c.z, c.w};
+    L.seed = 0u;
+#pragma unroll
+    for (int q = 0; q < 4; q++) {
+        const uint32_t m = (w[q] >> 1) & 0x01010101u;
+        const unsigned b = (m | (m >> 7) | (m >> 14) | (m >> 21)) & 0xfu;
+        L.seed |= b << (4 * q);
+        float4 v = make_float4(0.0f, 0.0f, 0.0f, 0.0f);
+        if (b) {
+            if (f16) v = *(const float4 *)(field + i0 + 4 * q);
+            else { v.x = field[i0 + 4 * q]; v.y = field[i0 + 4 * q + 1]; v.z = field[i0 + 4 * q + 2]; v.w = field[i0 + 4 * q + 3]; }
+        }
+        L.f[4 * q] = v.x; L.f[4 * q + 1] = v.y; L.f[4 * q + 2] = v.z; L.f[4 * q + 3] = v.w;
+    }
+}
+__device__ __forceinline__ void ws_lane16_cid(const int *__restrict__ cid, int64_t i0, unsigned want, int (&c)[16])
+{
+#pragma unroll
+    for (int q = 0; q < 4; q++) {
+        int4 v = make_int4(-1, -1, -1, -1);
+        if ((want >> (4 * q)) & 0xfu) v = *(const int4 *)(cid + i0 + 4 * q);
+        c[4 * q] = v.x; c[4 * q + 1] = v.y; c[4 * q + 2] = v.z; c[4 * q + 3] = v.w;
+    }
+}
+__device__ __forceinline__ int ws_sum16(int v) {
+#pragma unroll
+    for (int o = 1; o < 16; o <<= 1) v += __shfl_xor(v, o, 16);
+    return v;
+}
+__device__ __forceinline__ int ws_excl16(int v) {
+    const int l = threadIdx.x & 15;
+    int inc = v;
+#pragma unroll
+    for (int o = 1; o < 16; o <<= 1) { const int u = __shfl_up(inc, o, 16); if (l >= o) inc += u; }
+    return inc - v;
+}
+__device__ __forceinline__ unsigned ws_lane16_small(const WsLane16 &L, unsigned vmax, bool *below)
+{
+    unsigned sm = 0u; bool bl = false;
+#pragma unroll
+    for (int j = 0; j < 16; j++) {
+        const unsigned key = ws_ordkey(L.f[j]);
+        const bool sd = (L.seed >> j) & 1u;
+        sm |= (unsigned)(sd && key <= vmax) << j;
+        bl = bl || (sd && key < vmax);
+    }
+    if (below) *below = bl;
+    return sm;
+}
+#define WS_FOR_GROUPS16(g, nblk) for (int64_t g = (int64_t)blockIdx.x * 256 + threadIdx.x; g < (nblk) * 16; g += (int64_t)gridDim.x * 256)
+static unsigned ws_grid16(int64_t nblk) { const int64_t c = (nblk + 15) / 16; return (unsigned)(c < 8192 ? (c > 0 ? c : 1) : 8192); }
+
+__global__ void __launch_bounds__(256)
+k_ws_seed_counts16(const uint8_t *__restrict__ cls, const float *__restrict__ field, int64_t nblk, unsigned vmax, int f16,
+                   int *__restrict__ n_seed, int *__restrict__ n_small, int *__restrict__ any_below)
+{
+    WS_FOR_GROUPS16(g, nblk) {
+        WsLane16 L;
+        ws_lane16_load(cls, field, g * 16, f16 != 0, L);
+        bool below;
+        const unsigned sm = ws_lane16_small(L, vmax, &below);
+        if (below) *any_below = 1;
+        const int tot = ws_sum16(__popc(L.seed) | (__popc(sm) << 16));
+        if ((threadIdx.x & 15) == 0) { n_seed[g >> 4] = tot & 0xffff; n_small[g >> 4] = tot >> 16; }
+    }
+}
+__global__ void __launch_bounds__(256)
+k_ws_small_list16(const uint8_t *__restrict__ cls, const int *__restrict__ cid, const float *__restrict__ field, int64_t nblk, unsigned vmax, int f16,
+                  const long long *__restrict__ base_seed, const long long *__restrict__ base_small, const int *__restrict__ subid,
+                  long long *__restrict__ out_k, unsigned *__restrict__ out_val, int *__restrict__ out_id)
+{
+    WS_FOR_GROUPS16(g, nblk) {
+        WsLane16 L;
+        ws_lane16_load(cls, field, g * 16, f16 != 0, L);
+        const unsigned sm = ws_lane16_small(L, vmax, nullptr);
+        const int pre = ws_excl16(__popc(L.seed) | (__popc(sm) << 16));
+        if (!sm) continue;
+        int c[16];
+        ws_lane16_cid(cid, g * 16, sm, c);
+        const long long k0 = base_seed[g >> 4] + (pre & 0xffff), s0 = base_small[g >> 4] + (pre >> 16);
+#pragma unroll
+        for (int j = 0; j < 16; j++) {
+            if (!((sm >> j) & 1u)) continue;
+            const unsigned lower = (1u << j) - 1u;
+            const long long slot = s0 + __popc(sm & lower);
+            const int id = c[j] <= -2 ? -2 - c[j] : -1;
+            out_k[slot] = k0 + __popc(L.seed & lower); out_val[slot] = ws_ordkey(L.f[j]); out_id[slot] = (id >= 0 && subid) ? subid[id] : id;
+        }
+    }
+}
+__global__ void __launch_bounds__(256)
+k_ws_seed_list16(const uint8_t *__restrict__ cls, const int *__restrict__ cid, const float *__restrict__ field, int64_t nblk, int f16,
+                 const long long *__restrict__ base_seed, int64_t c0, int64_t cap, const int *__restrict__ subid, unsigned vmax,
+                 u64 *__restrict__ out_entry)
+{
+    WS_FOR_GROUPS16(g, nblk) {
+        const long long b0 = base_seed[g >> 4];
+        if (b0 >= c0 + cap || b0 + 256 <= c0) continue;
+        WsLane16 L;
+        ws_lane16_load(cls, field, g * 16, f16 != 0, L);
+        const int pre = ws_excl16(__popc(L.seed));
+        if (!L.seed) continue;
+        int c[16];
+        ws_lane16_cid(cid, g * 16, L.seed, c);
+#pragma unroll
+        for (int j = 0; j < 16; j++) {
+            if (!((L.seed >> j) & 1u)) continue;
+            const long long k = b0 + pre + __popc(L.seed & ((1u << j) - 1u)) - c0;
+            if (k < 0 || k >= cap) continue;
+            int id = c[j] <= -2 ? -2 - c[j] : -1;
+            const unsigned v = ws_ordkey(L.f[j]);
+            if (id >= 0 && subid && v <= vmax) id = subid[id];
+            out_entry[k] = v > vmax ? WS_INF : (((u64)v << 32) | 0x80000000ull | (u64)(unsigned)(id + 1));
+        }
+    }
+}
+struct WsCodes16 { unsigned d, l, x; };
+__device__ __forceinline__ WsCodes16 ws_lane16_codes(const WsLane16 &L, const int (&c)[16], unsigned vmax, u64 D)
+{
+    WsCodes16 r; r.d = r.l = r.x = 0u;
+#pragma unroll
+    for (int j = 0; j < 16; j++) {
+        if (!((L.seed >> j) & 1u)) continue;
+        const unsigned key = ws_ordkey(L.f[j]);
+        const int id = c[j] <= -2 ? -2 - c[j] : -1;
+        const bool l = key > vmax, d = !l && id < 0 && D != 0ull && key == (unsigned)(D >> 32);
+        r.l |= (unsigned)l << j; r.d |= (unsigned)d << j; r.x |= (unsigned)(!l && !d) << j;
+    }
+    return r;
+}
+__global__ void __launch_bounds__(256)
+k_ws_code_counts16(const uint8_t *__restrict__ cls, const int *__restrict__ cid, const float *__restrict__ field, int64_t nblk, unsigned vmax, u64 D,
+                   int f16, int *__restrict__ n_exc)
+{
+    WS_FOR_GROUPS16(g, nblk) {
+        WsLane16 L;
+        ws_lane16_load(cls, field, g * 16, f16 != 0, L);
+        int c[16];
+        ws_lane16_cid(cid, g * 16, L.seed, c);
+        const WsCodes16 r = ws_lane16_codes(L, c, vmax, D);
+        const int tot = ws_sum16(__popc(r.x));
+        if ((threadIdx.x & 15) == 0) n_exc[g >> 4] = tot;
+    }
+}
+__device__ __forceinline__ void ws_or_bits(unsigned *__restrict__ bits, long long pos, unsigned str)
+{
+    if (!str) return;
+    const int sh = (int)(pos & 31);
+    const unsigned lo = str << sh, hi = sh ? str >> (32 - sh) : 0u;
+    if (lo) atomicOr(&bits[pos >> 5], lo);
+    if (hi) atomicOr(&bits[(pos >> 5) + 1], hi);
+}
+__global__ void __launch_bounds__(256)
+k_ws_seed_codes16(const uint8_t *__restrict__ cls, const int *__restrict__ cid, const float *__restrict__ field, int64_t nblk, unsigned vmax, u64 D,
+                  int f16, const long long *__restrict__ base_seed, const long long *__restrict__ base_exc, const int *__restrict__ subid,
+                  int write_bits, unsigned *__restrict__ bits_d, unsigned *__restrict__ bits_l, int64_t c0, int64_t cap, u64 *__restrict__ exc)
+{
+    WS_FOR_GROUPS16(g, nblk) {
+        const long long bx = base_exc[g >> 4];
+        if (!write_bits && (bx >= c0 + cap || bx + 256 <= c0)) continue;
+        WsLane16 L;
+        ws_lane16_load(cls, field, g * 16, f16 != 0, L);
+        int c[16];
+        ws_lane16_cid(cid, g * 16, L.seed, c);
+        const WsCodes16 r = ws_lane16_codes(L, c, vmax, D);
+        const int pre = ws_excl16(__popc(L.seed) | (__popc(r.x) << 16));
+        if (!L.seed) continue;
+        if (write_bits) {
+            unsigned sd = 0u, sl = 0u; int n = 0;
+#pragma unroll
+            for (int j = 0; j < 16; j++) {
+                if (!((L.seed >> j) & 1u)) continue;
+                sd |= ((r.d >> j) & 1u) << n; sl |= ((r.l >> j) & 1u) << n; n++;
+            }
+            const long long pos = base_seed[g >> 4] + (pre & 0xffff);
+            ws_or_bits(bits_d, pos, sd);
+            ws_or_bits(bits_l, pos, sl);
+        }
+#pragma unroll
+        for (int j = 0; j < 16; j++) {
+            if (!((r.x >> j) & 1u)) continue;
+            const long long slot = bx + (pre >> 16) + __popc(r.x & ((1u << j) - 1u)) - c0;
+            if (slot < 0 || slot >= cap) continue;
+            int id = c[j] <= -2 ? -2 - c[j] : -1;
+            if (id >= 0 && subid) id = subid[id];
+            exc[slot] = ((u64)ws_ordkey(L.f[j]) << 32) | 0x80000000ull | (u64)(unsigned)(id + 1);
         }
     }
 }
@@ -1206,8 +1414,22 @@
     TF_REQUIRE(need <= j->scan_bytes, "tf_watershed: scan scratch too small for the seed numbering");
     int *d_any = j->d_flags + WS_BATCH + 6;
     TF_CHECK_HIP(hipMemsetAsync(d_any, 0, 2 * sizeof(int), s));
-    hipLaunchKernelGGL(k_ws_seed_counts, dim3((unsigned)nb256), dim3(256), 0, s, (const uint8_t *)j->cls, j->field, N, h_vmax, n_seed, n_small, d_any);
+    const int64_t nb16 = j->raveled ? 0 : N / 256, nb_tail = nb256 - nb16;
+    const int f16 = (uintptr_t)j->field % 16 == 0;
+    const double export_bytes = (double)N;
+    {
+    TfProfScope ps(TFK_WS_EXPORT, export_bytes, s);
+    if (nb16) hipLaunchKernelGGL(k_ws_seed_counts16, dim3(ws_grid16(nb16)), dim3(256), 0, s, (const uint8_t *)j->cls, j->field, nb16, h_vmax, f16, n_seed, n_small, d_any);
+    if (nb_tail) hipLaunchKernelGGL(k_ws_seed_counts, dim3((unsigned)nb_tail), dim3(256), 0, s, (const uint8_t *)j->cls, j->field, N, h_vmax, nb16, n_seed, n_small, d_any);
+    }
     TF_CHECK_LAUNCH();
+    auto small_list = [&](const int *sub, long long *out_k, unsigned *out_val, int *out_id) {
+        TfProfScope ps(TFK_WS_EXPORT, export_bytes, s);
+        if (nb16) hipLaunchKernelGGL(k_ws_small_list16, dim3(ws_grid16(nb16)), dim3(256), 0, s, (const uint8_t *)j->cls, (const int *)j->cid, j->field, nb16, h_vmax, f16,
+                                     (const long long *)base_seed, (const long long *)base_small, sub, out_k, out_val, out_id);
+        if (nb_tail) hipLaunchKernelGGL(k_ws_small_list, dim3((unsigned)nb_tail), dim3(256), 0, s, (const uint8_t *)j->cls, (const int *)j->cid, j->field, N, h_vmax, nb16,
+                                        (const long long *)base_seed, (const long long *)base_small, sub, out_k, out_val, out_id);
+    };
     size_t tb = j->scan_bytes;
     TF_CHECK_HIP(tf_exclusive_sum(j->scan_tmp, tb, WsCountIter(n_seed, WsIntToLL()), base_seed, (size_t)nb256, s));
     tb = j->scan_bytes;
@@ -1241,8 +1463,7 @@
                     h_any[0], h_any[1], (long long)S, (long long)R, tie_room, tie_need);
         if (!force_host && !force_dense && !h_any[0] && !h_any[1] && S > 0 && S <= R && S < 0x3fffffffll && tie_need <= tie_room) {
             long long *stg_k = (long long *)c.Rt; unsigned *stg_val = (unsigned *)c.Llo; int *stg_id = c.Lhi;
-            hipLaunchKernelGGL(k_ws_small_list, dim3((unsigned)nb256), dim3(256), 0, s, (const uint8_t *)j->cls, (const int *)j->cid, j->field, N, h_vmax,
-                               (const long long *)base_seed, (const long long *)base_small, (const int *)nullptr, stg_k, stg_val, stg_id);
+            small_list(nullptr, stg_k, stg_val, stg_id);
             TF_CHECK_LAUNCH();
             long long k_max = 0;
             TF_CHECK_HIP(hipMemcpyAsync(&k_max, stg_k + S - 1, sizeof(long long), hipMemcpyDeviceToHost, s));
@@ -1321,8 +1542,7 @@
     const int *subid_or_null = j->identity ? nullptr : subid;
     if (j->sparse) {
         long long *stg_k = (long long *)c.Rt; unsigned *stg_val = (unsigned *)c.Llo; int *stg_id = c.Lhi;
-        hipLaunchKernelGGL(k_ws_small_list, dim3((unsigned)nb256), dim3(256), 0, s, (const uint8_t *)j->cls, (const int *)j->cid, j->field, N, h_vmax,
-                           (const long long *)base_seed, (const long long *)base_small, subid_or_null, stg_k, stg_val, stg_id);
+        small_list(subid_or_null, stg_k, stg_val, stg_id);
         TF_CHECK_LAUNCH();
         if (ws_to_host(j->hb_sk.p, stg_k, (size_t)j->S * sizeof(long long), s) || ws_to_host(j->hb_sval.p, stg_val, (size_t)j->S * sizeof(unsigned), s) ||
             ws_to_host(j->hb_sid.p, stg_id, (size_t)j->S * sizeof(int), s)) return TF_EHIP;
@@ -1347,7 +1567,11 @@
             }
             j->code_d = D;
             int *n_exc = n_small; long long *base_exc = base_small;
-            hipLaunchKernelGGL(k_ws_code_counts, dim3((unsigned)nb256), dim3(256), 0, s, (const uint8_t *)j->cls, (const int *)j->cid, j->field, N, h_vmax, D, n_exc);
+            {
+            TfProfScope ps(TFK_WS_EXPORT, export_bytes, s);
+            if (nb16) hipLaunchKernelGGL(k_ws_code_counts16, dim3(ws_grid16(nb16)), dim3(256), 0, s, (const uint8_t *)j->cls, (const int *)j->cid, j->field, nb16, h_vmax, D, f16, n_exc);
+            if (nb_tail) hipLaunchKernelGGL(k_ws_code_counts, dim3((unsigned)nb_tail), dim3(256), 0, s, (const uint8_t *)j->cls, (const int *)j->cid, j->field, N, h_vmax, D, nb16, n_exc);
+            }
             TF_CHECK_LAUNCH();
             tb = j->scan_bytes;
             TF_CHECK_HIP(tf_exclusive_sum(j->scan_tmp, tb, WsCountIter(n_exc, WsIntToLL()), base_exc, (size_t)nb256, s));
@@ -1368,8 +1592,10 @@
             for (int64_t c0 = 0; first || c0 < E; c0 += cap, first = false) {
                 const int64_t cnt = E - c0 < cap ? E - c0 : cap;
                 u64 *stg = (u64 *)j->Q.q[1];
-                hipLaunchKernelGGL(k_ws_seed_codes, dim3((unsigned)nb256), dim3(256), 0, s, (const uint8_t *)j->cls, (const int *)j->cid, j->field, N, h_vmax, D,
-                                   (const long long *)base_seed, (const long long *)base_exc, subid_or_null, first ? 1 : 0, d_bits, d_bits + W, c0, cap, stg);
+                if (nb16) hipLaunchKernelGGL(k_ws_seed_codes16, dim3(ws_grid16(nb16)), dim3(256), 0, s, (const uint8_t *)j->cls, (const int *)j->cid, j->field, nb16, h_vmax, D, f16,
+                                             (const long long *)base_seed, (const long long *)base_exc, subid_or_null, first ? 1 : 0, d_bits, d_bits + W, c0, cap, stg);
+                if (nb_tail) hipLaunchKernelGGL(k_ws_seed_codes, dim3((unsigned)nb_tail), dim3(256), 0, s, (const uint8_t *)j->cls, (const int *)j->cid, j->field, N, h_vmax, D, nb16,
+                                                (const long long *)base_seed, (const long long *)base_exc, subid_or_null, first ? 1 : 0, d_bits, d_bits + W, c0, cap, stg);
                 TF_CHECK_LAUNCH();
                 if (cnt > 0 && ws_to_host((u64 *)j->hb_sid.p + c0, stg, (size_t)cnt * sizeof(u64), s)) return TF_EHIP;
                 if (first && ws_to_host(j->hb_sval.p, d_bits, (size_t)2 * W * sizeof(unsigned), s)) return TF_EHIP;
@@ -1383,8 +1609,10 @@
             for (int64_t c0 = 0; c0 < j->M; c0 += cap, turn ^= 1) {
                 const int64_t cnt = j->M - c0 < cap ? j->M - c0 : cap;
                 u64 *stg = (u64 *)j->Q.q[turn];
-                hipLaunchKernelGGL(k_ws_seed_list, dim3((unsigned)nb256), dim3(256), 0, s, (const uint8_t *)j->cls, (const int *)j->cid, j->field, N,
-                                   (const long long *)base_seed, c0, cap, subid_or_null, h_vmax, stg);
+                if (nb16) hipLaunchKernelGGL(k_ws_seed_list16, dim3(ws_grid16(nb16)), dim3(256), 0, s, (const uint8_t *)j->cls, (const int *)j->cid, j->field, nb16, f16,
+                                             (const long long *)base_seed, c0, cap, subid_or_null, h_vmax, stg);
+                if (nb_tail) hipLaunchKernelGGL(k_ws_seed_list, dim3((unsigned)nb_tail), dim3(256), 0, s, (const uint8_t *)j->cls, (const int *)j->cid, j->field, N, nb16,
+                                                (const long long *)base_seed, c0, cap, subid_or_null, h_vmax, stg);
                 TF_CHECK_LAUNCH();
                 if (ws_to_host((u64 *)j->hb_sk.p + c0, stg, (size_t)cnt * sizeof(u64), s)) return TF_EHIP;
                 if (turn) TF_CHECK_HIP(hipStreamSynchronize(s));
@@ -1581,15 +1809,18 @@
         tf_set_error("tf_watershed: workspace too small for %lld relevant pixels", (long long)R);
         return TF_ENOMEM;
     }
-    if (rv) hipLaunchKernelGGL(k_ws_cid, dim3(nb1), dim3(256), 0, s, cls, flag, scan, N, cid);
-    else if (tiles) hipLaunchKernelGGL(k_ws_cid_tiles, dim3((unsigned)((NV / 256 + 3) / 4)), dim3(256), 0, s, (const uint8_t *)cls, (const uint8_t *)flag,
-                                       (const long long *)((long long *)scan + NV / 256), NV / 256, g, cid);
-    else hipLaunchKernelGGL(k_ws_cid_tiled, grid, block, 0, s, (const uint8_t *)cls, (const uint8_t *)flag, (const int *)scan, g, cid);
-    TF_CHECK_LAUNCH();
     WsC &c = j->c; memset(&c, 0, sizeof(c));
     c.R = R; c.n_nbr = n_nbr;
     j->org = nullptr; j->rank_dev = nullptr;
     j->depth = 0;
+    auto launch_cid = [&](u64 *pix) {
+        TfProfScope ps(TFK_WS_SETUP, 0.0, s);
+        if (rv) hipLaunchKernelGGL(k_ws_cid, dim3(nb1), dim3(256), 0, s, cls, flag, scan, N, cid, pix);
+        else if (tiles) hipLaunchKernelGGL(k_ws_cid_tiles, dim3((unsigned)((NV / 256 + 3) / 4)), dim3(256), 0, s, (const uint8_t *)cls, (const uint8_t *)flag,
+                                           (const long long *)((long long *)scan + NV / 256), NV / 256, g, cid, pix);
+        else hipLaunchKernelGGL(k_ws_cid_tiled, grid, block, 0, s, (const uint8_t *)cls, (const uint8_t *)flag, (const int *)scan, g, cid, pix);
+    };
+    if (R == 0) { launch_cid(nullptr); TF_CHECK_LAUNCH(); }
     if (R > 0) {
         u64 *pix = ar.take<u64>(R); unsigned *val = ar.take<unsigned>(R); int *nbr = ar.take<int>(R * n_nbr);
         c.pix = pix; c.val = val; c.nbr = nbr;
@@ -1606,15 +1837,18 @@
         j->subid = ar.take<int>(R);
         Q.cnt = d_flags; Q.h_cnt = j->h_cnt; Q.processed = &st[7];
         if (!ar.ok()) { tf_set_error("tf_watershed: workspace too small"); return TF_ENOMEM; }
+        launch_cid(pix);
+        TF_CHECK_LAUNCH();
         int *d_nan = d_flags + WS_BATCH + 4;
         TF_CHECK_HIP(hipMemsetAsync(d_nan, 0, sizeof(int), s));
         {
             TfProfScope ps(TFK_WS_SETUP, 0.0, s);
-            if (rv) hipLaunchKernelGGL(k_wsr_compact, dim3(nb1), dim3(256), 0, s, field, (const int *)cid, *rv, pix, val, nbr, c.KM, d_nan);
-            else if (n_nbr == 6) hipLaunchKernelGGL(k_ws_compact<6>, grid, block, 0, s, field, fwd, bwd, cid, g, pix, val, nbr, c.KM, d_nan);
-            else if (n_nbr == 18) hipLaunchKernelGGL(k_ws_compact<18>, grid, block, 0, s, field, fwd, bwd, cid, g, pix, val, nbr, c.KM, d_nan);
-            else if (n_nbr == 26) hipLaunchKernelGGL(k_ws_compact<26>, grid, block, 0, s, field, fwd, bwd, cid, g, pix, val, nbr, c.KM, d_nan);
-            else hipLaunchKernelGGL(k_ws_compact<0>, grid, block, 0, s, field, fwd, bwd, cid, g, pix, val, nbr, c.KM, d_nan);
+            const dim3 gridR((unsigned)((R + 255) / 256));
+            if (rv) hipLaunchKernelGGL(k_wsr_compact, gridR, dim3(256), 0, s, field, (const int *)cid, *rv, R, (const u64 *)pix, val, nbr, c.KM, d_nan);
+            else if (n_nbr == 6) hipLaunchKernelGGL(k_ws_compact<6>, gridR, dim3(256), 0, s, field, fwd, bwd, cid, g, R, (const u64 *)pix, val, nbr, c.KM, d_nan);
+            else if (n_nbr == 18) hipLaunchKernelGGL(k_ws_compact<18>, gridR, dim3(256), 0, s, field, fwd, bwd, cid, g, R, (const u64 *)pix, val, nbr, c.KM, d_nan);
+            else if (n_nbr == 26) hipLaunchKernelGGL(k_ws_compact<26>, gridR, dim3(256), 0, s, field, fwd, bwd, cid, g, R, (const u64 *)pix, val, nbr, c.KM, d_nan);
+            else hipLaunchKernelGGL(k_ws_compact<0>, gridR, dim3(256), 0, s, field, fwd, bwd, cid, g, R, (const u64 *)pix, val, nbr, c.KM, d_nan);
         }
         TF_CHECK_LAUNCH();
         {
```

Measured after the change: 1024, median of 5. No clear change (+0.2%).
